# cmavro/GNN-RAG

Hardware: AMD Instinct MI355X
Metric: kg_edges_aggregated_per_sec (higher is better)
Workload: dtype f32

## Files before the change

### gnn-rag_amd/_lib.py

```python
from __future__ import annotations

import ctypes as C
import os

PKG = os.path.dirname(os.path.abspath(__file__))
LIB_PATH = os.path.join(PKG, "lib", "libgnnrag_hip.so")

c_i32p = C.POINTER(C.c_int32)
c_f32p = C.POINTER(C.c_float)


class CsrStruct(C.Structure):
    _fields_ = [
        ("B", C.c_int32), ("N", C.c_int32), ("R1", C.c_int32), ("heavy_deg", C.c_int32),
        ("F", C.c_int64),
        ("row_ptr", C.c_void_p * 2), ("edge", C.c_void_p * 2), ("perm", C.c_void_p * 2),
        ("w_gnn", C.c_void_p * 2), ("w_rel", C.c_void_p * 2),
        ("heavy", C.c_void_p * 2), ("chunk_off", C.c_void_p * 2),
        ("n_heavy", C.c_void_p), ("n_chunks", C.c_void_p),
        ("heavy_cap", C.c_int32), ("max_chunks", C.c_int32),
        ("big_cnt", C.c_void_p), ("big_nodes", C.c_void_p),
        ("big_deg", C.c_int32), ("hub_sorted", C.c_int32),
        ("edge_l", C.c_void_p * 2), ("rel_off", C.c_void_p), ("rel_rows", C.c_void_p),
        ("rel_total", C.c_int32), ("rel_max", C.c_int32),
        ("edge_m", C.c_void_p), ("m_from", C.c_void_p), ("m_dst", C.c_void_p),
        ("hub_q_off", C.c_void_p * 2), ("hub_wbase", C.c_void_p * 2),
    ]


class RelorderStruct(C.Structure):
    _fields_ = [("F", C.c_int64), ("rel_total", C.c_int32), ("n_chunks", C.c_int32),
                ("ht", C.c_void_p), ("perm", C.c_void_p), ("w", C.c_void_p), ("row_ptr", C.c_void_p),
                ("chunk_ptr", C.c_void_p)]


class UGraphStruct(C.Structure):
    _fields_ = [("B", C.c_int32), ("N", C.c_int32), ("F", C.c_int64), ("cap", C.c_int64),
                ("u_ptr", C.c_void_p), ("u_adj", C.c_void_p)]


class DenseFormStruct(C.Structure):
    _fields_ = [(n, C.c_int32) for n in ("family", "block_family", "launches", "epi", "nt", "mt", "v4", "math", "nw",
                                          "v4out", "n0", "nc", "has_add", "kguard")]


class LayerParams(C.Structure):
    _fields_ = [("W_rel", C.c_void_p), ("b_rel", C.c_void_p), ("pos_fwd", C.c_void_p), ("pos_inv", C.c_void_p),
                ("W_e2e", C.c_void_p), ("b_e2e", C.c_void_p)]


class BertLayer(C.Structure):
    _fields_ = [(n, C.c_void_p) for n in ("W_qkv", "b_qkv", "W_o", "b_o", "ln1_g", "ln1_b", "W_i", "b_i", "W_f", "b_f",
                                          "ln2_g", "ln2_b")]


_VP = C.c_void_p
SIGNATURES = {
    "gnnrag_csr_bytes": (C.c_size_t, [C.c_int64, C.c_int32, C.c_int32, C.c_int32, C.c_int, C.c_int]),
    "gnnrag_csr_scratch_bytes": (C.c_size_t, [C.c_int64, C.c_int32, C.c_int32, C.c_int32]),
    "gnnrag_csr_build": (C.c_int, [_VP, _VP, _VP, _VP, _VP, C.c_int64, C.c_int32, C.c_int32, C.c_int32,
                                   _VP, C.c_size_t, _VP, C.c_size_t, C.POINTER(CsrStruct), _VP]),
    "gnnrag_csr_build_counts": (C.c_int, [_VP, _VP, _VP, _VP, _VP, C.c_int64, C.c_int32, C.c_int32, C.c_int32, C.c_int32,
                                          C.c_int32, _VP, C.c_size_t, _VP, C.c_size_t, C.POINTER(CsrStruct), _VP]),
    "gnnrag_csr_status": (C.c_int, [C.POINTER(CsrStruct), _VP]),
    "gnnrag_csr_concat": (C.c_int, [C.POINTER(C.POINTER(CsrStruct)), C.c_int32, C.c_int32, C.c_int32, _VP, C.c_size_t,
                                    C.POINTER(CsrStruct), _VP]),
    "gnnrag_narrow_tuple": (C.c_int, [_VP, _VP, _VP, C.c_int64, _VP, C.c_int32]),
    "gnnrag_csr_permute_weight": (C.c_int, [C.POINTER(CsrStruct), _VP, C.c_int, _VP, _VP, _VP]),
    "gnnrag_linear": (C.c_int, [_VP, C.c_int64, C.c_int32, _VP, _VP, _VP, C.c_int64, C.c_int, _VP,
                                C.c_int32, C.c_int32, _VP]),
    "gnnrag_linear_pair": (C.c_int, [_VP, _VP, C.c_int64, C.c_int32, _VP, _VP, _VP, _VP, C.c_int64, _VP, _VP,
                                     C.c_int32, C.c_int32, _VP]),
    "gnnrag_aggregate_workspace_bytes": (C.c_size_t, [C.POINTER(CsrStruct), C.c_int32, C.c_int32]),
    "gnnrag_aggregate": (C.c_int, [C.POINTER(CsrStruct), _VP, _VP, _VP, _VP, _VP, C.c_int32, C.c_int32,
                                   _VP, C.c_size_t, _VP]),
    "gnnrag_aggregate_fused": (C.c_int, [C.POINTER(CsrStruct), _VP, _VP, _VP, C.c_int32, _VP, C.c_size_t, _VP]),
    "gnnrag_aggregate_fused_variant": (C.c_int, [C.POINTER(CsrStruct), C.c_int32]),
    "gnnrag_aggregate_fused_hub_form": (C.c_int, [C.POINTER(CsrStruct), C.c_int32, _VP, C.c_size_t, _VP, _VP]),
    "gnnrag_relorder_bytes": (C.c_size_t, [C.POINTER(CsrStruct), C.c_int]),
    "gnnrag_relorder_scratch_bytes": (C.c_size_t, [C.POINTER(CsrStruct)]),
    "gnnrag_relorder_build": (C.c_int, [C.POINTER(CsrStruct), _VP, _VP, _VP, _VP, _VP, C.c_size_t, _VP, C.c_size_t,
                                        C.POINTER(RelorderStruct), _VP]),
    "gnnrag_backward_workspace_bytes": (C.c_size_t, [C.POINTER(CsrStruct), C.POINTER(RelorderStruct), C.c_int32,
                                                     C.c_int32]),
    "gnnrag_aggregate_fused_backward": (C.c_int, [C.POINTER(CsrStruct), C.POINTER(RelorderStruct), _VP, _VP, _VP, _VP, _VP,
                                                 C.c_int32, _VP, C.c_size_t, _VP]),
    "gnnrag_aggregate_backward": (C.c_int, [C.POINTER(CsrStruct), C.POINTER(RelorderStruct), _VP, _VP, _VP, _VP, _VP,
                                            _VP, _VP, _VP, _VP, C.c_int32, C.c_int32, _VP, C.c_size_t, _VP]),
    "gnnrag_typelayer_backward": (C.c_int, [C.POINTER(CsrStruct), C.POINTER(RelorderStruct), _VP, _VP, C.c_int, _VP,
                                            C.c_int32, _VP, C.c_size_t, _VP]),
    "gnnrag_lstm_workspace_bytes": (C.c_size_t, [C.c_int32, C.c_int32]),
    "gnnrag_lstm_forward": (C.c_int, [_VP] * 10 + [C.c_int32] * 4 + [_VP, C.c_size_t, _VP]),
    "gnnrag_lstm_reserve_bytes": (C.c_size_t, [C.c_int32] * 3),
    "gnnrag_lstm_forward_train": (C.c_int, [_VP] * 10 + [C.c_int32] * 4 + [_VP, C.c_size_t, _VP, C.c_size_t, _VP]),
    "gnnrag_lstm_backward_workspace_bytes": (C.c_size_t, [C.c_int32] * 4),
    "gnnrag_lstm_backward": (C.c_int, [_VP] * 7 + [C.c_size_t] + [_VP] * 9 + [C.c_int32] * 4 + [_VP, C.c_size_t, _VP]),
    "gnnrag_seed_retrieve": (C.c_int, [_VP, _VP, _VP, C.c_int32, C.c_int32, C.c_int32, _VP]),
    "gnnrag_query_reform": (C.c_int, [_VP, _VP, _VP, C.c_int64, _VP, _VP, _VP, C.c_int32, C.c_int32, C.c_int32, _VP]),
    "gnnrag_topp_candidates": (C.c_int, [_VP, _VP, C.c_int32, C.c_int32, C.c_double, C.c_double, _VP, _VP, _VP]),
    "gnnrag_topp_workspace_bytes": (C.c_size_t, [C.c_int32, C.c_int32]),
    "gnnrag_topp_candidates_ws": (C.c_int, [_VP, _VP, C.c_int32, C.c_int32, C.c_double, C.c_double, _VP, _VP, _VP,
                                            C.c_size_t, _VP]),
    "gnnrag_relation_tables": (C.c_int, [C.POINTER(CsrStruct), _VP, _VP, _VP, _VP, _VP, C.c_int32, C.c_int32,
                                         C.c_int32, _VP]),
    "gnnrag_update_score_fused": (C.c_int, [_VP, _VP, _VP, _VP, _VP, _VP, _VP, _VP, _VP, C.c_int64, C.c_int32,
                                            C.c_int32, C.c_int32, _VP]),
    "gnnrag_update_score": (C.c_int, [_VP, _VP, _VP, _VP, _VP, _VP, _VP, _VP, _VP, C.c_int64, C.c_int32,
                                      C.c_int32, C.c_int32, _VP]),
    "gnnrag_dense_form": (C.c_int, [C.c_int32, C.c_int64, C.c_int32, C.c_int32, C.c_int32, C.c_int32, C.c_int64,
                                    C.c_int32, C.c_int32, C.POINTER(DenseFormStruct)]),
    "gnnrag_masked_softmax": (C.c_int, [_VP, _VP, C.c_int32, C.c_int32, _VP]),
    "gnnrag_typelayer": (C.c_int, [C.POINTER(CsrStruct), _VP, C.c_int, _VP, C.c_int32, _VP, C.c_size_t, _VP]),
    "gnnrag_layer_workspace_bytes": (C.c_size_t, [C.POINTER(CsrStruct), C.c_int32, C.c_int32]),
    "gnnrag_stack_workspace_bytes": (C.c_size_t, [C.POINTER(CsrStruct), C.c_int32, C.c_int32, C.c_int32]),
    "gnnrag_rel_transform": (C.c_int, [_VP, _VP, C.c_int64, C.c_int32, C.c_int32, C.POINTER(LayerParams), C.c_int32, _VP,
                                      _VP, _VP]),
    "gnnrag_gemm_tn_workspace_bytes": (C.c_size_t, [C.c_int64, C.c_int32, C.c_int32]),
    "gnnrag_gemm_tn": (C.c_int, [_VP, _VP, C.c_int64, C.c_int32, C.c_int32, _VP, _VP, C.c_size_t, _VP]),
    "gnnrag_rel_planes_bytes": (C.c_size_t, [C.c_int64, C.c_int32, C.c_int32]),
    "gnnrag_relation_tables_planes": (C.c_int, [C.POINTER(CsrStruct), _VP, _VP, _VP, _VP, C.c_int32, C.c_int32, _VP]),
    "gnnrag_rel_packed_bytes": (C.c_size_t, [C.c_int64, C.c_int32, C.c_int32]),
    "gnnrag_rel_transform_packed": (C.c_int, [_VP, _VP, C.c_int64, C.c_int32, C.c_int32, C.POINTER(LayerParams), C.c_int32,
                                             _VP, _VP, _VP]),
    "gnnrag_relation_tables_packed": (C.c_int, [C.POINTER(CsrStruct), _VP, _VP, _VP, _VP, C.c_int32, C.c_int32, C.c_int32,
                                               _VP]),
    "gnnrag_reason_layer": (C.c_int, [C.POINTER(CsrStruct)] + [_VP] * 9 + [C.c_int32] + [_VP] * 8 +
                            [_VP, C.c_size_t, C.c_int32, C.c_int32, C.c_int32, C.c_int32, _VP]),
    "gnnrag_reason_stack": (C.c_int, [C.POINTER(CsrStruct), C.c_int32, C.POINTER(LayerParams)] + [_VP] * 5 +
                            [C.c_int32] + [_VP] * 6 + [_VP, C.c_size_t, C.c_int32, C.c_int32, C.c_int32, C.c_int32, _VP]),
    "gnnrag_reason_stack_capture": (C.c_int, [C.POINTER(CsrStruct), C.c_int32, C.POINTER(LayerParams)] + [_VP] * 5 +
                                    [C.c_int32] + [_VP] * 6 + [_VP, C.c_size_t, C.c_int32, C.c_int32, C.c_int32,
                                                               C.c_int32, _VP, C.POINTER(C.c_void_p)]),
    "gnnrag_graph_launch": (C.c_int, [_VP, _VP]),
    "gnnrag_graph_destroy": (C.c_int, [_VP]),
    "gnnrag_frontier_workspace_bytes": (C.c_size_t, [C.POINTER(CsrStruct)]),
    "gnnrag_frontier_supported": (C.c_int, [C.POINTER(CsrStruct), C.c_int32]),
    "gnnrag_frontier_build": (C.c_int, [C.POINTER(CsrStruct), _VP, _VP, C.c_size_t, _VP]),
    "gnnrag_relation_tables_frontier": (C.c_int, [C.POINTER(CsrStruct), _VP, _VP, _VP, _VP, _VP, _VP, C.c_int32,
                                                  C.c_int32, _VP]),
    "gnnrag_aggregate_fused_frontier": (C.c_int, [C.POINTER(CsrStruct), _VP, _VP, _VP, _VP, C.c_int32, _VP]),
    "gnnrag_frontier_read": (C.c_int, [C.POINTER(CsrStruct), _VP, _VP, _VP, _VP]),
    "gnnrag_instructions": (C.c_int, [_VP] * 4 + [C.POINTER(C.c_void_p)] * 2 + [_VP] * 4 + [C.c_int32] * 4 + [_VP] * 3),
    "gnnrag_instructions_reserve_bytes": (C.c_size_t, [C.c_int32] * 4),
    "gnnrag_instructions_train": (C.c_int, [_VP] * 4 + [C.POINTER(C.c_void_p)] * 2 + [_VP] * 7 + [C.c_int32] * 4 +
                                  [_VP] * 3 + [C.c_size_t, _VP]),
    "gnnrag_instructions_backward_workspace_bytes": (C.c_size_t, [C.c_int32] * 4),
    "gnnrag_instructions_backward": (C.c_int, [_VP] * 3 + [C.POINTER(C.c_void_p)] + [_VP] * 8 + [C.c_size_t] + [_VP] * 5 +
                                     [C.POINTER(C.c_void_p)] * 2 + [_VP] * 4 + [C.c_int32] * 4 + [_VP, C.c_size_t, _VP]),
    "gnnrag_query_reform_reserve_bytes": (C.c_size_t, [C.c_int32] * 3),
    "gnnrag_query_reform_train": (C.c_int, [C.POINTER(C.c_void_p), _VP, _VP, C.c_int64] + [C.POINTER(C.c_void_p)] * 2 +
                                  [_VP, _VP, C.c_size_t] + [C.c_int32] * 4 + [_VP]),
    "gnnrag_query_reform_backward_workspace_bytes": (C.c_size_t, [C.c_int32] * 4),
    "gnnrag_query_reform_backward": (C.c_int, [C.POINTER(C.c_void_p), _VP] + [C.POINTER(C.c_void_p)] * 2 +
                                     [_VP, C.c_size_t] + [C.POINTER(C.c_void_p)] * 4 + [_VP] + [C.c_int32] * 4 +
                                     [_VP, C.c_size_t, _VP]),
    "gnnrag_layer_tail_train": (C.c_int, [_VP] * 3 + [C.c_float] + [_VP] * 3 + [C.c_int32] * 3 + [_VP] * 4),
    "gnnrag_layer_tail_backward_workspace_bytes": (C.c_size_t, [C.c_int32] * 3),
    "gnnrag_layer_tail_backward": (C.c_int, [_VP] * 3 + [C.c_float] + [_VP] * 3 + [C.c_int32] * 3 + [_VP] * 4 +
                                   [C.c_size_t, _VP]),
    "gnnrag_kl_loss_workspace_bytes": (C.c_size_t, [C.c_int32]),
    "gnnrag_kl_loss_train": (C.c_int, [_VP] * 3 + [C.c_int32] * 2 + [_VP] * 3 + [C.c_size_t, _VP]),
    "gnnrag_kl_loss_backward": (C.c_int, [_VP] * 5 + [C.c_int32] * 2 + [_VP] * 2),
    "gnnrag_train_metrics": (C.c_int, [_VP] * 4 + [C.c_int64, C.c_double] + [C.c_int32] * 2 + [_VP] * 5),
    "gnnrag_bert_workspace_bytes": (C.c_size_t, [C.c_int32] * 4),
    "gnnrag_bert_attention": (C.c_int, [_VP] + [C.c_int32] * 4 + [_VP, _VP]),
    "gnnrag_bert_encode": (C.c_int, [_VP, _VP, C.c_int32, _VP, C.c_int32, _VP, _VP, _VP, C.c_float, C.c_int32,
                                     C.POINTER(BertLayer)] + [C.c_int32] * 5 + [_VP, _VP, C.c_size_t, C.c_int32, _VP]),
    "gnnrag_bert_attention_bias": (C.c_int, [_VP] + [C.c_int32] * 4 + [_VP, _VP, _VP]),
    "gnnrag_bert_encode_ex": (C.c_int, [_VP, _VP, C.c_int32, _VP, C.c_int32, _VP, C.c_int32, _VP, _VP, _VP, C.c_float,
                                        C.c_int32, C.POINTER(BertLayer)] + [C.c_int32] * 5 +
                              [_VP, _VP, C.c_size_t, C.c_int32, _VP]),
    "gnnrag_bert_keep_hidden_bytes": (C.c_size_t, [C.c_int32] * 4),
    "gnnrag_bert_keep_att_bytes": (C.c_size_t, [C.c_int32] * 4),
    "gnnrag_bert_attention_drop": (C.c_int, [_VP] + [C.c_int32] * 4 + [_VP, _VP, C.c_float, _VP, _VP]),
    "gnnrag_bert_encode_train": (C.c_int, [_VP, _VP, C.c_int32, _VP, C.c_int32, _VP, C.c_int32, _VP, _VP, _VP, C.c_float,
                                           C.c_int32, C.POINTER(BertLayer)] + [C.c_int32] * 5 +
                                 [_VP, C.c_float, _VP, C.c_float, _VP, _VP, C.c_size_t, C.c_int32, _VP]),
    "gnnrag_rel_text_workspace_bytes": (C.c_size_t, [C.c_int64] + [C.c_int32] * 4),
    "gnnrag_rel_text_pool": (C.c_int, [_VP] * 6 + [C.c_int64] + [C.c_int32] * 3 + [_VP] * 5 + [C.c_size_t, _VP]),
    "gnnrag_rel_text_backward_workspace_bytes": (C.c_size_t, [C.c_int64] + [C.c_int32] * 4),
    "gnnrag_rel_text_pool_backward": (C.c_int, [_VP] * 8 + [C.c_int64] + [C.c_int32] * 3 + [_VP] * 4 + [C.c_size_t, _VP]),
    "gnnrag_ugraph_bytes": (C.c_size_t, [C.c_int64, C.c_int32, C.c_int32]),
    "gnnrag_ugraph_scratch_bytes": (C.c_size_t, [C.c_int64, C.c_int32, C.c_int32]),
    "gnnrag_ugraph_build": (C.c_int, [C.POINTER(CsrStruct), _VP, C.c_size_t, _VP, C.c_size_t, C.POINTER(UGraphStruct),
                                      _VP]),
    "gnnrag_paths_workspace_bytes": (C.c_size_t, [C.c_int32, C.c_int32, C.c_int32, C.c_int32]),
    "gnnrag_paths_out_bytes": (C.c_size_t, [C.c_int32] * 5),
    "gnnrag_shortest_paths": (C.c_int, [C.POINTER(UGraphStruct), _VP, _VP, _VP, C.c_int32, C.c_int32, C.c_int32, C.c_int32,
                                        _VP, _VP, _VP, _VP, _VP, _VP, C.c_size_t, _VP]),
    "gnnrag_rule_paths_workspace_bytes": (C.c_size_t, [C.c_int64] + [C.c_int32] * 4),
    "gnnrag_rule_paths_out_bytes": (C.c_size_t, [C.c_int32] * 5),
    "gnnrag_rule_paths": (C.c_int, [C.POINTER(UGraphStruct), _VP, _VP, _VP, _VP, C.c_int32, C.c_int32, C.c_int32, C.c_int32,
                                    _VP, _VP, _VP, _VP, _VP, _VP, C.c_size_t, _VP]),
    "gnnrag_stream_copy": (C.c_int, [_VP, _VP, C.c_int64, _VP]),
    "gnnrag_abi_version": (C.c_int, []),
    "gnnrag_error_string": (C.c_char_p, [C.c_int]),
}

ABI_VERSION = 16
PATH_AUTO, PATH_UNFUSED, PATH_FUSED = 0, 1, 2
PATH_ONLY_FWD, PATH_ONLY_INV = 0x10, 0x20
PATH_SEED_PRIOR = 0x40
PATH_REUSE_PROJ = 0x80
E_TUPLE = -4
_lib = None


class GnnragError(RuntimeError):
    pass


def load():
    global _lib
    if _lib is not None:
        return _lib
    path = os.environ.get("GNNRAG_LIB", LIB_PATH)
    if not os.path.exists(path):
        raise GnnragError(
            "HIP extension %s is not built. Run `python -c 'import __graft_entry__ as g; g.build()'` "
            "(hipcc --offload-arch=gfx950). There is no CPU fallback." % path)
    lib = C.CDLL(path)
    for name, (res, args) in SIGNATURES.items():
        fn = getattr(lib, name)
        fn.restype = res
        fn.argtypes = args
    if lib.gnnrag_abi_version() != ABI_VERSION:
        raise GnnragError("ABI mismatch: library %d, binding %d" % (lib.gnnrag_abi_version(), ABI_VERSION))
    _lib = lib
    return lib


def check(code: int, what: str = ""):
    if code != 0:
        msg = load().gnnrag_error_string(code)
        err = GnnragError("%s failed (%d): %s" % (what or "gnnrag call", code,
                                                  msg.decode() if msg else "?"))
        err.code = code
        raise err
```

### gnn-rag_amd/csrc/dense_internal.h

```cpp
#pragma once
#include "gnnrag_common.h"

namespace gnnrag {

int tables_vq_launch_z(const gnnrag_csr* csr, const void* planes, const float* ins, const float* W, float* P, int32_t D,
                       int32_t I, int32_t only_dir, float* zero, int64_t zero_n, hipStream_t stream, bool packed);
size_t tables_vq_packed_bytes(int64_t R1);

int update_score_fused_rows(const float* h, const float* nbr, const uint8_t* add_flag, const float* W, const float* b,
                            const float* w_s, const float* b_s, const float* mask, float* h_out, float* score,
                            int64_t BN, int32_t D, int32_t I, int32_t math, hipStream_t stream, bool score_zeroed);
int update_b3_launch_f(const float* h, const float* nbr, const uint8_t* add_flag, const float* W, const float* b,
                       const float* w_s, const float* b_s, const float* mask, float* h_out, float* score, int64_t BN,
                       int32_t D, int32_t ldw, hipStream_t stream, bool score_zeroed);

bool update_rows_supported(const float* h, const float* nbr, const float* W, const float* h_out, int64_t BN, int32_t D,
                           int32_t I, int32_t math);
bool update_b3_shape_ok(int64_t BN, int32_t D, int32_t ldw);
int tables_small_launch(const gnnrag_csr* csr, const float* T_fwd, const float* T_inv, const float* ins, const float* W,
                        float* P, int32_t D, int32_t I, hipStream_t stream);

int frontier_build_z(const gnnrag_csr* csr, const float* dist, void* fws, size_t fws_bytes, float* zero_a,
                     int64_t zero_na, float* zero_b, int64_t zero_nb, hipStream_t stream);
const uint8_t* frontier_row_flags(const gnnrag_csr* csr, const void* fws);

int update_score_fused_z(const float* h, const float* nbr, const float* W, const float* b, const float* w_s,
                         const float* b_s, const float* mask, float* h_out, float* score, int64_t BN, int32_t D,
                         int32_t I, int32_t math, hipStream_t stream, bool score_zeroed);

bool rel_transform_accepts(const float* relfeat_fwd, const float* relfeat_inv, int64_t R1, int32_t D, int32_t L,
                           const gnnrag_layer_params* layers, int32_t pos_rows, const float* T_out, const void* planes_out);
int rel_transform_launch(const float* relfeat_fwd, const float* relfeat_inv, int64_t R1, int32_t D, int32_t L,
                         const gnnrag_layer_params* layers, int32_t pos_rows, float* T_out, void* planes_out,
                         void* packed_out, gnnrag_stream_t stream);

}
```

### gnn-rag_amd/csrc/frontier.hip

```cpp
#include "dense_internal.h"

namespace gnnrag {

constexpr int kFrThreads = 1024;
constexpr int kFrSeedCap = 2048;
constexpr int kFrAltSeeds = 32;

struct FrontierWs {
  size_t counts, row_flag, rows, tflag, trows, seeds, seedinfo, total;
};

static FrontierWs frontier_ws(const gnnrag_csr* csr) {
  FrontierWs w;
  Carve cv;
  const size_t BN = (size_t)csr->B * csr->N;
  const size_t RT = (size_t)(csr->rel_total > 0 ? csr->rel_total : 1);
  w.counts = cv.take((size_t)2 * csr->B * sizeof(int32_t));
  w.row_flag = cv.take(BN + 64);
  w.rows = cv.take(BN * sizeof(int32_t));
  w.tflag = cv.take(RT + 64);
  w.trows = cv.take(RT * sizeof(int32_t));
  w.seeds = cv.take((size_t)csr->B * kFrAltSeeds * sizeof(int32_t));
  w.seedinfo = cv.take((size_t)2 * csr->B * sizeof(int32_t));
  w.total = cv.off;
  return w;
}

__global__ __launch_bounds__(kFrThreads) void k_frontier_build(
    const float* __restrict__ dist, const int32_t* __restrict__ rp0, const int32_t* __restrict__ rp1,
    const int2* __restrict__ el0, const int2* __restrict__ el1, const int32_t* __restrict__ rel_off, int N,
    uint8_t* __restrict__ row_flag, int32_t* __restrict__ rows, uint8_t* __restrict__ tflag,
    int32_t* __restrict__ trows, int32_t* __restrict__ counts, int32_t* __restrict__ seeds,
    int32_t* __restrict__ seedinfo, float* __restrict__ zero_a, long long zero_na, float* __restrict__ zero_b,
    long long zero_nb) {
  __shared__ int s_seed[kFrSeedCap];
  __shared__ int s_ns, s_wsum[kFrThreads / 64];
  const int g = blockIdx.x, tid = threadIdx.x, lane = tid & 63, wave = tid >> 6;
  const int roff = rel_off[g], Rg = rel_off[g + 1] - roff;
  const size_t n0 = (size_t)g * N;
  for (long long i = (long long)blockIdx.x * kFrThreads + tid; i < zero_na; i += (long long)gridDim.x * kFrThreads) zero_a[i] = 0.f;
  for (long long i = (long long)blockIdx.x * kFrThreads + tid; i < zero_nb; i += (long long)gridDim.x * kFrThreads) zero_b[i] = 0.f;
  if (tid == 0) s_ns = 0;
  if (g == (int)gridDim.x - 1 && tid < 64) row_flag[(size_t)gridDim.x * N + tid] = 0;
  for (int i = tid; i < N; i += kFrThreads) row_flag[n0 + i] = 0;
  for (int i = tid; i < Rg; i += kFrThreads) tflag[roff + i] = 0;
  __syncthreads();
  for (int i = tid; i < N; i += kFrThreads) {
    if (dist[n0 + i] != 0.f) {
      const int k = atomicAdd(&s_ns, 1);
      if (k < kFrSeedCap) s_seed[k] = (int)n0 + i;
    }
  }
  __syncthreads();
  const int ns = s_ns;
  if (tid == 0) {
    int cnt = -1, facts = 0;
    if (ns <= kFrAltSeeds) {
      cnt = ns;
      for (int i = 1; i < ns; ++i) {
        const int v = s_seed[i];
        int j = i - 1;
        for (; j >= 0 && s_seed[j] > v; --j) s_seed[j + 1] = s_seed[j];
        s_seed[j + 1] = v;
      }
      for (int i = 0; i < ns; ++i) {
        const int sn = s_seed[i];
        seeds[g * kFrAltSeeds + i] = sn;
        facts += (rp0[sn + 1] - rp0[sn]) + (rp1[sn + 1] - rp1[sn]);
      }
    }
    seedinfo[2 * g] = cnt;
    seedinfo[2 * g + 1] = facts;
  }
  __syncthreads();
  if (ns > kFrSeedCap) {
    for (int i = tid; i < N; i += kFrThreads) row_flag[n0 + i] = 1;
    for (int i = tid; i < Rg; i += kFrThreads) tflag[roff + i] = 1;
  } else {
    for (int k = 0; k < ns; ++k) {
      const int s = s_seed[k];
#pragma unroll
      for (int dd = 0; dd < 2; ++dd) {
        const int32_t* rp = dd ? rp1 : rp0;
        const int2* el = dd ? el1 : el0;
        const int beg = rp[s], end = rp[s + 1];
        for (int j = beg + tid; j < end; j += kFrThreads) {
          const int2 e = el[j];
          row_flag[e.x] = 1;
          tflag[roff + e.y] = 1;
        }
      }
    }
  }
  __syncthreads();
  auto compact = [&](const uint8_t* flag, int n, int first, int32_t* list, int32_t* count_out) {
    int base = 0;
    for (int c0 = 0; c0 < n; c0 += kFrThreads) {
      const int i = c0 + tid;
      const bool on = i < n && flag[i] != 0;
      const unsigned long long m = __ballot(on);
      if (lane == 0) s_wsum[wave] = __popcll(m);
      __syncthreads();
      int off = base, tot = 0;
      for (int w = 0; w < kFrThreads / 64; ++w) {
        const int c = s_wsum[w];
        if (w < wave) off += c;
        tot += c;
      }
      if (on) list[off + __popcll(m & ((1ull << lane) - 1))] = first + i;
      base += tot;
      __syncthreads();
    }
    if (tid == 0) *count_out = base;
  };
  compact(row_flag + n0, N, (int)n0, rows + n0, counts + 2 * g);
  compact(tflag + roff, Rg, roff, trows + roff, counts + 2 * g + 1);
}

struct TabFrArgs {
  const float* T[2];
  const float* ins;
  const float* W;
  const int2* rel_rows;
  const int32_t* rel_off;
  const int32_t* list;
  const int32_t* counts;
  float* P;
  int32_t D, I, rel_total, B;
  int32_t dense;
};

__global__ __launch_bounds__(256) void k_tables_frontier(TabFrArgs a, int tiles_per_q) {
  __shared__ __attribute__((aligned(16))) float s_part[3][4][64][4];
  const int lane = threadIdx.x & 63, wave = threadIdx.x >> 6;
  const int fr = lane & 15, fg = lane >> 4;
  const int D = a.D, K = a.I * D, ldw = (2 * a.I + 1) * D;
  const int ncg = (D + 63) >> 6;
  const f32x4 zero4 = {0.f, 0.f, 0.f, 0.f};
  const int nitem = a.dense ? ((a.rel_total + 15) >> 4) * 2 * ncg : a.B * 2 * ncg;
  for (int item = blockIdx.x; item < nitem; item += gridDim.x)
  for (int tile = a.dense ? item / (2 * ncg) : 0; tile < (a.dense ? item / (2 * ncg) + 1 : tiles_per_q); ++tile) {
    int r = a.dense ? item % (2 * ncg) : item;
    const int cg = r % ncg; r /= ncg;
    const int d = r & 1; r >>= 1;
    const int g = a.dense ? 0 : r;
    const int cnt = a.dense ? a.rel_total : a.counts[2 * g + 1];
    if (tile * 16 >= cnt) break;
    const int32_t* list = a.dense ? nullptr : a.list + a.rel_off[g];
    const int c0 = cg * 64;
    const int m = tile * 16 + fr;
    const int prow = a.dense ? (m < cnt ? m : cnt - 1) : list[m < cnt ? m : cnt - 1];
    const int2 br = a.rel_rows[prow];
    const float* trow = a.T[d] + (size_t)br.y * D;
    const float* qrow = a.ins + (size_t)br.x * a.I * D;
    const float* wrow[4];
#pragma unroll
    for (int nt = 0; nt < 4; ++nt) wrow[nt] = a.W + (size_t)min(c0 + nt * 16 + fr, D - 1) * ldw + (size_t)(1 + d) * D;
    f32x4 acc[4] = {zero4, zero4, zero4, zero4};
    const int nkg = (K + 15) >> 4;
    for (int kg0 = wave; kg0 < nkg; kg0 += 16) {
      f32x4 av[4], bv[4][4];
#pragma unroll
      for (int u = 0; u < 4; ++u) {
        const int k = (kg0 + 4 * u) * 16 + fg * 4;
        av[u] = zero4;
#pragma unroll
        for (int nt = 0; nt < 4; ++nt) bv[u][nt] = zero4;
        if (k < K) {
          const int i = k / D, kk = k - i * D;
          const f32x4 t = *reinterpret_cast<const f32x4*>(trow + kk);
          const f32x4 q = *reinterpret_cast<const f32x4*>(qrow + (size_t)i * D + kk);
          av[u] = __builtin_elementwise_max(t * q, zero4);
#pragma unroll
          for (int nt = 0; nt < 4; ++nt) bv[u][nt] = *reinterpret_cast<const f32x4*>(wrow[nt] + (size_t)2 * i * D + kk);
        }
      }
#pragma unroll
      for (int u = 0; u < 4; ++u)
#pragma unroll
        for (int nt = 0; nt < 4; ++nt)
#pragma unroll
          for (int e = 0; e < 4; ++e) acc[nt] = __builtin_amdgcn_mfma_f32_16x16x4f32(av[u][e], bv[u][nt][e], acc[nt], 0, 0, 0);
    }
    if (wave > 0) {
#pragma unroll
      for (int nt = 0; nt < 4; ++nt) *reinterpret_cast<f32x4*>(&s_part[wave - 1][nt][lane][0]) = acc[nt];
    }
    __syncthreads();
    if (wave == 0) {
#pragma unroll
      for (int nt = 0; nt < 4; ++nt) {
        const f32x4 v = ((acc[nt] + *reinterpret_cast<const f32x4*>(&s_part[0][nt][lane][0])) +
                         *reinterpret_cast<const f32x4*>(&s_part[1][nt][lane][0])) +
                        *reinterpret_cast<const f32x4*>(&s_part[2][nt][lane][0]);
        const int col = c0 + nt * 16 + fr;
#pragma unroll
        for (int rr = 0; rr < 4; ++rr) {
          const int mm = tile * 16 + fg * 4 + rr;
          if (mm < cnt && col < D) a.P[((size_t)d * a.rel_total + (a.dense ? mm : list[mm])) * D + col] = v[rr];
        }
      }
    }
    __syncthreads();
  }
}

struct WalkFrArgs {
  const int32_t* rp0;
  const int32_t* rp1;
  const int2* edge_m;
  const int32_t* m_from;
  const float* w0;
  const float* w1;
  const float* dist;
  const float* P;
  const int32_t* rel_off;
  const int32_t* rows;
  const int32_t* counts;
  float* out;
  const int32_t* seeds;
  const int32_t* seedinfo;
  int64_t F;
  int32_t N, D, rel_total, B;
};

constexpr int kWfThreads = 256;
constexpr int kWfPer = 8;
constexpr int kWfCap = kWfThreads * kWfPer;
constexpr int kWfAltMin = 4096;

__global__ __launch_bounds__(kWfThreads) void k_walk_frontier(WalkFrArgs a, int per_q) {
  __shared__ int2 s_live[kWfCap];
  __shared__ int s_wsum[kWfPer * 4];
  __shared__ __attribute__((aligned(16))) float s_red[3][256];
  const int tid = threadIdx.x, lane = tid & 63, wave = tid >> 6;
  const int D = a.D;
  const int g = blockIdx.x / per_q;
  const int cnt = a.counts[2 * g];
  const int roff = a.rel_off[g], Rg = a.rel_off[g + 1] - roff;
  const int col = 4 * lane;
  const bool cok = col < D;
  const f32x4 zero4 = {0.f, 0.f, 0.f, 0.f};
  for (int it = blockIdx.x % per_q; it < cnt; it += per_q) {
    const int n = a.rows[(size_t)g * a.N + it];
    const int beg = a.rp0[n] + a.rp1[n], end = a.rp0[n + 1] + a.rp1[n + 1];
    f32x4 acc = zero4;
    bool split = false;
    const int nseed = a.seedinfo[2 * g];
    const bool alt = nseed > 0 && end - beg > kWfAltMin && a.seedinfo[2 * g + 1] <= ((end - beg) >> 2);
    if (alt && wave == 0) {
      for (int si = 0; si < nseed; ++si) {
        const int sn = a.seeds[g * kFrAltSeeds + si];
        const float ps = a.dist[sn];
        const int sb = a.rp0[sn] + a.rp1[sn], se = a.rp0[sn + 1] + a.rp1[sn + 1];
        for (int c0 = sb; c0 < se; c0 += 64) {
          const int j = c0 + lane;
          const int2 e = j < se ? a.edge_m[j] : make_int2(-1, 0);
          float p = 0.f;
          if (e.x == n) {
            p = ps;
            if (a.w0) {
              const int f = a.m_from[j];
              p *= f < a.F ? a.w0[f] : a.w1[f - a.F];
            }
          }
          unsigned long long m = __ballot(p != 0.f);
          while (m) {
            const int l = __builtin_ctzll(m);
            m &= m - 1;
            const float pl = __int_as_float(__builtin_amdgcn_readlane(__float_as_int(p), l));
            const int rm = __builtin_amdgcn_readlane(e.y, l);
            const int dq = rm > Rg ? 1 : 0;
            const int rl = dq ? rm - (Rg + 1) : rm;
            if (cok) acc += pl * *reinterpret_cast<const f32x4*>(a.P + ((size_t)(1 - dq) * a.rel_total + roff + rl) * D + col);
          }
        }
      }
    }
    for (int c0 = beg; c0 < (alt ? beg : end); c0 += kWfCap) {
      int2 e[kWfPer];
      float p[kWfPer];
#pragma unroll
      for (int u = 0; u < kWfPer; ++u) {
        const int j = c0 + u * kWfThreads + tid;
        e[u] = j < end ? a.edge_m[j] : make_int2(0, 0);
      }
#pragma unroll
      for (int u = 0; u < kWfPer; ++u) {
        const int j = c0 + u * kWfThreads + tid;
        p[u] = 0.f;
        if (j < end) {
          p[u] = a.dist[e[u].x];
          if (a.w0) {
            const int f = a.m_from[j];
            p[u] *= f < a.F ? a.w0[f] : a.w1[f - a.F];
          }
        }
      }
      unsigned long long mk[kWfPer];
#pragma unroll
      for (int u = 0; u < kWfPer; ++u) {
        mk[u] = __ballot(p[u] != 0.f);
        if (lane == 0) s_wsum[u * 4 + wave] = __popcll(mk[u]);
      }
      __syncthreads();
      int nl = 0;
#pragma unroll
      for (int u = 0; u < kWfPer; ++u) {
        int off = nl;
#pragma unroll
        for (int w = 0; w < 4; ++w) {
          const int t = s_wsum[u * 4 + w];
          if (w < wave) off += t;
          nl += t;
        }
        if (p[u] != 0.f) {
          const int rm = e[u].y;
          const int d = rm > Rg ? 1 : 0;
          const int rl = d ? rm - (Rg + 1) : rm;
          s_live[off + __popcll(mk[u] & ((1ull << lane) - 1))] = make_int2(__float_as_int(p[u]), d * a.rel_total + roff + rl);
        }
      }
      __syncthreads();
      if (nl <= 32 && !split) {
        if (wave == 0 && cok) {
          for (int k = 0; k < nl; ++k) {
            const int2 lv = s_live[k];
            const f32x4 t = *reinterpret_cast<const f32x4*>(a.P + (size_t)lv.y * D + col);
            acc += __int_as_float(lv.x) * t;
          }
        }
      } else {
        split = true;
        if (cok) {
          for (int k = wave; k < nl; k += 4) {
            const int2 lv = s_live[k];
            const f32x4 t = *reinterpret_cast<const f32x4*>(a.P + (size_t)lv.y * D + col);
            acc += __int_as_float(lv.x) * t;
          }
        }
      }
      __syncthreads();
    }
    if (split) {
      if (wave > 0) *reinterpret_cast<f32x4*>(&s_red[wave - 1][col]) = acc;
      __syncthreads();
      if (wave == 0)
        acc = ((acc + *reinterpret_cast<const f32x4*>(&s_red[0][col])) + *reinterpret_cast<const f32x4*>(&s_red[1][col])) +
              *reinterpret_cast<const f32x4*>(&s_red[2][col]);
      __syncthreads();
    }
    if (wave == 0 && cok) *reinterpret_cast<f32x4*>(a.out + (size_t)n * D + col) = acc;
  }
}

}

using namespace gnnrag;

extern "C" size_t gnnrag_frontier_workspace_bytes(const gnnrag_csr* csr) {
  if (!csr) return 0;
  return frontier_ws(csr).total;
}

extern "C" int gnnrag_frontier_supported(const gnnrag_csr* csr, int32_t D) {
  return csr && csr->edge_m && csr->m_from && D > 0 && D % 4 == 0 && D <= 256 ? 1 : 0;
}

int gnnrag::frontier_build_z(const gnnrag_csr* csr, const float* dist, void* fws, size_t fws_bytes, float* zero_a,
                             int64_t zero_na, float* zero_b, int64_t zero_nb, hipStream_t stream) {
  if (!csr || !dist || !fws) return GNNRAG_E_BADARG;
  const FrontierWs w = frontier_ws(csr);
  if (fws_bytes < w.total) return GNNRAG_E_WORKSPACE;
  char* base = (char*)fws;
  hipLaunchKernelGGL(k_frontier_build, dim3(csr->B), dim3(kFrThreads), 0, stream, dist, csr->row_ptr[0], csr->row_ptr[1],
                     (const int2*)csr->edge_l[0], (const int2*)csr->edge_l[1], csr->rel_off, csr->N,
                     (uint8_t*)(base + w.row_flag), (int32_t*)(base + w.rows), (uint8_t*)(base + w.tflag),
                     (int32_t*)(base + w.trows), (int32_t*)(base + w.counts), (int32_t*)(base + w.seeds),
                     (int32_t*)(base + w.seedinfo), zero_a, (long long)zero_na, zero_b,
                     (long long)zero_nb);
  GNNRAG_LAUNCH_CHECK();
  return 0;
}

extern "C" int gnnrag_frontier_build(const gnnrag_csr* csr, const float* dist, void* fws, size_t fws_bytes,
                                     gnnrag_stream_t stream) {
  return frontier_build_z(csr, dist, fws, fws_bytes, nullptr, 0, nullptr, 0, (hipStream_t)stream);
}

const uint8_t* gnnrag::frontier_row_flags(const gnnrag_csr* csr, const void* fws) {
  return (const uint8_t*)fws + frontier_ws(csr).row_flag;
}

extern "C" int gnnrag_relation_tables_frontier(const gnnrag_csr* csr, const void* fws, const float* T_fwd,
                                               const float* T_inv, const float* ins, const float* W, float* P,
                                               int32_t D, int32_t I, gnnrag_stream_t stream) {
  if (!csr || !fws || !T_fwd || !T_inv || !ins || !W || !P || I <= 0) return GNNRAG_E_BADARG;
  if (!gnnrag_frontier_supported(csr, D) || !aligned16(T_fwd, T_inv, ins, W, P)) return GNNRAG_E_UNSUPPORTED;
  if (csr->rel_total == 0) return 0;
  const FrontierWs w = frontier_ws(csr);
  const char* base = (const char*)fws;
  TabFrArgs a;
  a.T[0] = T_fwd; a.T[1] = T_inv; a.ins = ins; a.W = W;
  a.rel_rows = (const int2*)csr->rel_rows;
  a.rel_off = csr->rel_off;
  a.list = (const int32_t*)(base + w.trows);
  a.counts = (const int32_t*)(base + w.counts);
  a.P = P; a.D = D; a.I = I; a.rel_total = csr->rel_total; a.B = csr->B; a.dense = 0;
  const int tiles_per_q = (csr->rel_max + 15) / 16;
  const int64_t nitem = (int64_t)csr->B * 2 * ((D + 63) / 64);
  hipLaunchKernelGGL(k_tables_frontier, dim3((unsigned)(nitem < 4096 ? nitem : 4096)), dim3(256), 0, (hipStream_t)stream, a,
                     tiles_per_q);
  GNNRAG_LAUNCH_CHECK();
  return 0;
}

extern "C" int gnnrag_aggregate_fused_frontier(const gnnrag_csr* csr, const void* fws, const float* dist,
                                               const float* P, float* out, int32_t D, gnnrag_stream_t stream) {
  if (!csr || !fws || !dist || !P || !out) return GNNRAG_E_BADARG;
  if (!gnnrag_frontier_supported(csr, D) || !aligned16(P, out) || csr->N <= 0) return GNNRAG_E_UNSUPPORTED;
  const FrontierWs w = frontier_ws(csr);
  const char* base = (const char*)fws;
  WalkFrArgs a;
  a.rp0 = csr->row_ptr[0]; a.rp1 = csr->row_ptr[1];
  a.edge_m = (const int2*)csr->edge_m; a.m_from = csr->m_from;
  a.w0 = csr->w_gnn[0]; a.w1 = csr->w_gnn[1];
  a.dist = dist; a.P = P; a.rel_off = csr->rel_off;
  a.rows = (const int32_t*)(base + w.rows);
  a.counts = (const int32_t*)(base + w.counts);
  a.seeds = (const int32_t*)(base + w.seeds);
  a.seedinfo = (const int32_t*)(base + w.seedinfo);
  a.out = out; a.F = csr->F; a.N = csr->N; a.D = D; a.rel_total = csr->rel_total; a.B = csr->B;
  int per_q = 1024 / csr->B;
  if (per_q < 4) per_q = 4;
  if (per_q > 256) per_q = 256;
  if (per_q > csr->N) per_q = csr->N;
  hipLaunchKernelGGL(k_walk_frontier, dim3((unsigned)(csr->B * per_q)), dim3(kWfThreads), 0, (hipStream_t)stream, a, per_q);
  GNNRAG_LAUNCH_CHECK();
  return 0;
}

extern "C" int gnnrag_frontier_read(const gnnrag_csr* csr, const void* fws, int32_t* counts2, uint8_t* row_flag_host,
                                    gnnrag_stream_t stream) {
  if (!csr || !fws || !counts2) return GNNRAG_E_BADARG;
  const FrontierWs w = frontier_ws(csr);
  const char* base = (const char*)fws;
  int32_t* per_q = new int32_t[(size_t)2 * csr->B];
  hipError_t e = hipMemcpyAsync(per_q, base + w.counts, (size_t)2 * csr->B * sizeof(int32_t), hipMemcpyDeviceToHost,
                                (hipStream_t)stream);
  if (e == hipSuccess && row_flag_host)
    e = hipMemcpyAsync(row_flag_host, base + w.row_flag, (size_t)csr->B * csr->N, hipMemcpyDeviceToHost, (hipStream_t)stream);
  if (e == hipSuccess) e = hipStreamSynchronize((hipStream_t)stream);
  counts2[0] = counts2[1] = 0;
  for (int g = 0; g < csr->B; ++g) {
    counts2[0] += per_q[2 * g];
    counts2[1] += per_q[2 * g + 1];
  }
  delete[] per_q;
  return e == hipSuccess ? 0 : (int)e;
}

int gnnrag::tables_small_launch(const gnnrag_csr* csr, const float* T_fwd, const float* T_inv, const float* ins,
                                const float* W, float* P, int32_t D, int32_t I, hipStream_t stream) {
  if (D % 4 || D > 256 || csr->rel_total <= 0) return GNNRAG_E_UNSUPPORTED;
  if (2.0 * 2 * csr->rel_total * (double)I * D * D > 1.5e8) return GNNRAG_E_UNSUPPORTED;
  if (!aligned16(T_fwd, T_inv, ins, W)) return GNNRAG_E_UNSUPPORTED;
  TabFrArgs a;
  a.T[0] = T_fwd; a.T[1] = T_inv; a.ins = ins; a.W = W;
  a.rel_rows = (const int2*)csr->rel_rows;
  a.rel_off = csr->rel_off;
  a.list = nullptr; a.counts = nullptr;
  a.P = P; a.D = D; a.I = I; a.rel_total = csr->rel_total; a.B = csr->B; a.dense = 1;
  const int nitem = ((csr->rel_total + 15) / 16) * 2 * ((D + 63) / 64);
  hipLaunchKernelGGL(k_tables_frontier, dim3(nitem), dim3(256), 0, stream, a, 0);
  GNNRAG_LAUNCH_CHECK();
  return 0;
}
```

### gnn-rag_amd/csrc/rel_transform.hip

```cpp
#include "gnnrag_common.h"
#include "dense_internal.h"

namespace gnnrag {

constexpr int kRtMaxL = 8;
constexpr int kRtUnroll = 7;

struct RelTArgs {
  const float* A[2];
  const float* W[kRtMaxL];
  const float* b[kRtMaxL];
  const float* add[kRtMaxL][2];
  float* C;
  unsigned short* planes;
  unsigned char* packed;
  int M, K, N, add_rows;
};

constexpr int kPlaneHalf = 224;
constexpr int kPlaneRow = 2 * kPlaneHalf;
constexpr int kPackPlaneB = kPlaneHalf * 2;
constexpr int kPackIdxB = 3 * kPackPlaneB;
constexpr int kPackRowB = kPackIdxB + 64;

template <int TPW>
__global__ __launch_bounds__(256) void k_rel_transform(RelTArgs g) {
  extern __shared__ __attribute__((aligned(16))) float Wf[];
  const int tid = threadIdx.x, lane = tid & 63, wave = tid >> 6;
  const int fr = lane & 15, fg = lane >> 4;
  const int j = blockIdx.z >> 1, d = blockIdx.z & 1;
  const int colg = blockIdx.y * 64;
  const int K = g.K;
  const int nch = (K + 15) >> 4;
  const f32x4 zero4 = {0.f, 0.f, 0.f, 0.f};
  const bool compute = colg < g.N;
  if (compute) {
    const int total = 64 * nch * 4;
    for (int x = tid; x < total; x += 256) {
      const int col = x / (nch * 4), kq = x - col * (nch * 4);
      f32x4 v = zero4;
      if (colg + col < g.N && 4 * kq < K) v = *reinterpret_cast<const f32x4*>(g.W[j] + (size_t)(colg + col) * K + 4 * kq);
      const int c = kq >> 2, fgq = kq & 3, a = col & 3, frq = col >> 2;
      *reinterpret_cast<f32x4*>(Wf + ((size_t)((c * 4 + a) * 64 + fgq * 16 + frq)) * 4) = v;
    }
  }
  __syncthreads();
  const int c4 = colg + 4 * fr;
  const bool in_T = c4 < g.N;
  const bool in_pad = !in_T && c4 < kPlaneHalf;
  f32x4 bias = zero4;
  if (in_T && g.b[j]) bias = *reinterpret_cast<const f32x4*>(g.b[j] + c4);
  const float* __restrict__ addp = g.add[j][d];
  float* __restrict__ cp = g.C + ((size_t)(2 * j + d) * g.M) * g.N;
  unsigned short* pp = g.planes ? g.planes + ((size_t)(2 * j + d) * 3 * g.M) * kPlaneRow : nullptr;
  unsigned char* pk = g.packed ? g.packed + ((size_t)(2 * j + d) * g.M) * kPackRowB : nullptr;

#pragma unroll 1
  for (int t = 0; t < TPW; ++t) {
    const int row0 = (blockIdx.x * TPW + t) * 64 + wave * 16;
    if (row0 >= g.M) break;
    f32x4 acc[4][2];
#pragma unroll
    for (int a = 0; a < 4; ++a) acc[a][0] = acc[a][1] = zero4;
    if (compute) {
      const float* __restrict__ ap = g.A[d] + (size_t)min(row0 + fr, g.M - 1) * K;
      for (int c0 = 0; c0 < nch; c0 += kRtUnroll) {
        f32x4 av[kRtUnroll];
#pragma unroll
        for (int u = 0; u < kRtUnroll; ++u)
          av[u] = *reinterpret_cast<const f32x4*>(ap + min(16 * (c0 + u) + 4 * fg, K - 4));
#pragma unroll
        for (int u = 0; u < kRtUnroll; ++u) {
          const int c = min(c0 + u, nch - 1);
          const bool live = 16 * (c0 + u) + 4 * fg < K;
          const f32x4 x = live ? av[u] : zero4;
          f32x4 wv[4];
#pragma unroll
          for (int a = 0; a < 4; ++a) wv[a] = *reinterpret_cast<const f32x4*>(Wf + ((size_t)((c * 4 + a) * 64 + lane)) * 4);
#pragma unroll
          for (int e = 0; e < 4; ++e)
#pragma unroll
            for (int a = 0; a < 4; ++a)
              acc[a][e & 1] = __builtin_amdgcn_mfma_f32_16x16x4f32(x[e], wv[a][e], acc[a][e & 1], 0, 0, 0);
        }
      }
    }
    if (!in_T && !(pp && in_pad) && !pk) continue;
#pragma unroll
    for (int r = 0; r < 4; ++r) {
      const int row = row0 + 4 * fg + r;
      if (row >= g.M) continue;
      f32x4 v = zero4;
      if (in_T) {
#pragma unroll
        for (int a = 0; a < 4; ++a) v[a] = acc[a][0][r] + acc[a][1][r];
        v += bias;
        if (addp && row < g.add_rows) v += *reinterpret_cast<const f32x4*>(addp + (size_t)row * g.N + c4);
        *reinterpret_cast<f32x4*>(cp + (size_t)row * g.N + c4) = v;
      }
      if (pp) {
#pragma unroll
        for (int half = 0; half < 2; ++half) {
          const Split3 sp = split3(__builtin_elementwise_max(half ? -v : v, zero4));
          const size_t e = (size_t)row * kPlaneRow + half * kPlaneHalf + c4;
          *reinterpret_cast<uint2*>(pp + e) = sp.hi;
          *reinterpret_cast<uint2*>(pp + (size_t)g.M * kPlaneRow + e) = sp.mid;
          *reinterpret_cast<uint2*>(pp + (size_t)2 * g.M * kPlaneRow + e) = sp.lo;
        }
      }
      if (pk) {
        unsigned char* rowp = pk + (size_t)row * kPackRowB;
        if (c4 < kPlaneHalf) {
          const Split3 sp = split3(__builtin_elementwise_abs(v));
          *reinterpret_cast<uint2*>(rowp + 2 * c4) = sp.hi;
          *reinterpret_cast<uint2*>(rowp + kPackPlaneB + 2 * c4) = sp.mid;
          *reinterpret_cast<uint2*>(rowp + 2 * kPackPlaneB + 2 * c4) = sp.lo;
        }
        const int q = c4 >> 2;
        const unsigned ix = 0x88u | (unsigned)(v[0] < 0.f) | (unsigned)(v[1] < 0.f) << 2 | (unsigned)(v[2] < 0.f) << 4 |
                            (unsigned)(v[3] < 0.f) << 6;
        rowp[kPackIdxB + ((q & 7) >> 1) * 16 + (q >> 3) * 2 + (q & 1)] = (unsigned char)(c4 < kPlaneHalf ? ix : 0u);
      }
    }
  }
}

}

using namespace gnnrag;

extern "C" size_t gnnrag_rel_planes_bytes(int64_t R1, int32_t D, int32_t L) {
  if (R1 <= 0 || D <= 0 || D > kPlaneHalf || L <= 0) return 0;
  return (size_t)L * 2 * 3 * R1 * kPlaneRow * sizeof(unsigned short);
}

bool gnnrag::rel_transform_accepts(const float* relfeat_fwd, const float* relfeat_inv, int64_t R1, int32_t D, int32_t L,
                                   const gnnrag_layer_params* layers, int32_t pos_rows, const float* T_out,
                                   const void* planes_out) {
  if (D <= 0 || (D & 3)) return false;
  if (planes_out && D > kPlaneHalf) return false;
  if (R1 >= ((int64_t)1 << 31) / D) return false;
  uintptr_t align = (uintptr_t)relfeat_fwd | (uintptr_t)relfeat_inv | (uintptr_t)T_out | (uintptr_t)planes_out;
  for (int j = 0; j < L; ++j) {
    align |= (uintptr_t)layers[j].W_rel | (uintptr_t)layers[j].b_rel;
    if (pos_rows > 0) align |= (uintptr_t)layers[j].pos_fwd | (uintptr_t)layers[j].pos_inv;
  }
  if (align & 15) return false;
  return (size_t)64 * ((D + 15) / 16) * 16 * sizeof(float) <= 160 * 1024;
}

extern "C" size_t gnnrag_rel_packed_bytes(int64_t R1, int32_t D, int32_t L) {
  if (R1 <= 0 || D <= 0 || D > kPlaneHalf || L <= 0) return 0;
  return (size_t)L * 2 * R1 * kPackRowB;
}

int gnnrag::rel_transform_launch(const float* relfeat_fwd, const float* relfeat_inv, int64_t R1, int32_t D, int32_t L,
                                 const gnnrag_layer_params* layers, int32_t pos_rows, float* T_out, void* planes_out,
                                 void* packed_out, gnnrag_stream_t stream) {
  if (planes_out && packed_out) return GNNRAG_E_BADARG;
  void* const side_out = planes_out ? planes_out : packed_out;
  if (!relfeat_fwd || !relfeat_inv || !layers || !T_out || R1 < 0 || D <= 0 || L <= 0 || pos_rows < 0)
    return GNNRAG_E_BADARG;
  for (int j = 0; j < L; ++j) {
    if (!layers[j].W_rel) return GNNRAG_E_BADARG;
    if ((layers[j].pos_fwd == nullptr) != (layers[j].pos_inv == nullptr)) return GNNRAG_E_BADARG;
  }
  if (!gnnrag::rel_transform_accepts(relfeat_fwd, relfeat_inv, R1, D, L, layers, pos_rows, T_out, side_out))
    return GNNRAG_E_UNSUPPORTED;
  if (R1 == 0) return 0;
  for (int j0 = 0; j0 < L; j0 += kRtMaxL) {
    const int n = L - j0 < kRtMaxL ? L - j0 : kRtMaxL;
    RelTArgs g;
    memset(&g, 0, sizeof(g));
    g.A[0] = relfeat_fwd;
    g.A[1] = relfeat_inv;
    for (int j = 0; j < n; ++j) {
      const gnnrag_layer_params& p = layers[j0 + j];
      g.W[j] = p.W_rel;
      g.b[j] = p.b_rel;
      g.add[j][0] = pos_rows > 0 ? p.pos_fwd : nullptr;
      g.add[j][1] = pos_rows > 0 ? p.pos_inv : nullptr;
    }
    g.C = T_out + (size_t)j0 * 2 * R1 * D;
    g.planes = planes_out ? (unsigned short*)planes_out + (size_t)j0 * 2 * 3 * R1 * kPlaneRow : nullptr;
    g.packed = packed_out ? (unsigned char*)packed_out + (size_t)j0 * 2 * R1 * kPackRowB : nullptr;
    g.M = (int)R1; g.K = D; g.N = D;
    g.add_rows = (int)(pos_rows < R1 ? pos_rows : R1);
    const unsigned gy = (unsigned)(((side_out ? kPlaneHalf : D) + 63) / 64), gz = (unsigned)(2 * n);
    const size_t lds = (size_t)64 * ((D + 15) / 16) * 16 * sizeof(float);
    static DeviceMask cap1, cap4;
    if (R1 > 2048) {
      if (lds > 64 * 1024) { const int rc = raise_lds_cap(k_rel_transform<4>, cap4); if (rc) return rc; }
      hipLaunchKernelGGL(k_rel_transform<4>, dim3((unsigned)((R1 + 255) / 256), gy, gz), dim3(256), lds,
                         (hipStream_t)stream, g);
    } else {
      if (lds > 64 * 1024) { const int rc = raise_lds_cap(k_rel_transform<1>, cap1); if (rc) return rc; }
      hipLaunchKernelGGL(k_rel_transform<1>, dim3((unsigned)((R1 + 63) / 64), gy, gz), dim3(256), lds,
                         (hipStream_t)stream, g);
    }
    GNNRAG_LAUNCH_CHECK();
  }
  return 0;
}

extern "C" int gnnrag_rel_transform(const float* relfeat_fwd, const float* relfeat_inv, int64_t R1, int32_t D,
                                    int32_t L, const gnnrag_layer_params* layers, int32_t pos_rows, float* T_out,
                                    void* planes_out, gnnrag_stream_t stream) {
  return gnnrag::rel_transform_launch(relfeat_fwd, relfeat_inv, R1, D, L, layers, pos_rows, T_out, planes_out, nullptr, stream);
}

extern "C" int gnnrag_rel_transform_packed(const float* relfeat_fwd, const float* relfeat_inv, int64_t R1, int32_t D,
                                           int32_t L, const gnnrag_layer_params* layers, int32_t pos_rows, float* T_out,
                                           void* packed_out, gnnrag_stream_t stream) {
  if (!packed_out) return GNNRAG_E_BADARG;
  return gnnrag::rel_transform_launch(relfeat_fwd, relfeat_inv, R1, D, L, layers, pos_rows, T_out, nullptr, packed_out, stream);
}
```

### gnn-rag_amd/csrc/softmax_layer.hip

```cpp
#include "gnnrag_common.h"
#include "dense_internal.h"

namespace gnnrag {

template <int ITEMS>
__global__ __launch_bounds__(1024) void k_masked_softmax(const float* __restrict__ score,
                                                         float* __restrict__ dist, int N) {
  __shared__ float red[16];
  __shared__ float bcast;
  const float* s = score + (size_t)blockIdx.x * N;
  float* o = dist + (size_t)blockIdx.x * N;
  const int lane = threadIdx.x & 63, wave = threadIdx.x >> 6;
  float v[ITEMS > 0 ? ITEMS : 1];

  float m = -INFINITY;
  if constexpr (ITEMS > 0) {
#pragma unroll
    for (int k = 0; k < ITEMS; ++k) {
      const int i = threadIdx.x + k * 1024;
      v[k] = i < N ? s[i] : -INFINITY;
      m = fmaxf(m, v[k]);
    }
  } else {
    for (int i = threadIdx.x; i < N; i += 1024) m = fmaxf(m, s[i]);
  }
#pragma unroll
  for (int off = 32; off > 0; off >>= 1) m = fmaxf(m, __shfl_xor(m, off, 64));
  if (lane == 0) red[wave] = m;
  __syncthreads();
  if (threadIdx.x == 0) {
    float mm = red[0];
    for (int w = 1; w < 16; ++w) mm = fmaxf(mm, red[w]);
    bcast = mm;
  }
  __syncthreads();
  m = bcast;
  __syncthreads();

  float sum = 0.f;
  if constexpr (ITEMS > 0) {
#pragma unroll
    for (int k = 0; k < ITEMS; ++k) {
      v[k] = expf(v[k] - m);
      sum += v[k];
    }
  } else {
    for (int i = threadIdx.x; i < N; i += 1024) sum += expf(s[i] - m);
  }
  sum = wave_sum(sum);
  if (lane == 0) red[wave] = sum;
  __syncthreads();
  if (threadIdx.x == 0) {
    float t = 0.f;
    for (int w = 0; w < 16; ++w) t += red[w];
    bcast = t;
  }
  __syncthreads();
  const float total = bcast;
  if constexpr (ITEMS > 0) {
#pragma unroll
    for (int k = 0; k < ITEMS; ++k) {
      const int i = threadIdx.x + k * 1024;
      if (i < N) o[i] = v[k] / total;
    }
  } else {
    for (int i = threadIdx.x; i < N; i += 1024) o[i] = expf(s[i] - m) / total;
  }
}

template <int ITEMS>
__global__ __launch_bounds__(1024) void k_softmax_pairs(const float* __restrict__ score, float* __restrict__ dist, int N,
                                                        const int32_t* __restrict__ rp0, const int32_t* __restrict__ rp1,
                                                        const int2* __restrict__ em, const int32_t* __restrict__ from,
                                                        const float* __restrict__ w0, const float* __restrict__ w1,
                                                        int64_t F, int2* __restrict__ pr) {
  extern __shared__ float s_dist[];
  __shared__ float red[16];
  __shared__ float bcast;
  const int g = blockIdx.x, part = blockIdx.y, nparts = gridDim.y;
  const float* s = score + (size_t)g * N;
  float* o = dist + (size_t)g * N;
  const int lane = threadIdx.x & 63, wave = threadIdx.x >> 6;
  float v[ITEMS];
  float m = -INFINITY;
#pragma unroll
  for (int k = 0; k < ITEMS; ++k) {
    const int i = threadIdx.x + k * 1024;
    v[k] = i < N ? s[i] : -INFINITY;
    m = fmaxf(m, v[k]);
  }
  m = wave_max(m);
  if (lane == 0) red[wave] = m;
  __syncthreads();
  if (threadIdx.x == 0) {
    float mm = red[0];
    for (int w = 1; w < 16; ++w) mm = fmaxf(mm, red[w]);
    bcast = mm;
  }
  __syncthreads();
  m = bcast;
  __syncthreads();
  float sum = 0.f;
#pragma unroll
  for (int k = 0; k < ITEMS; ++k) {
    v[k] = expf(v[k] - m);
    sum += v[k];
  }
  sum = wave_sum(sum);
  if (lane == 0) red[wave] = sum;
  __syncthreads();
  if (threadIdx.x == 0) {
    float t = 0.f;
    for (int w = 0; w < 16; ++w) t += red[w];
    bcast = t;
  }
  __syncthreads();
  const float total = bcast;
#pragma unroll
  for (int k = 0; k < ITEMS; ++k) {
    const int i = threadIdx.x + k * 1024;
    if (i < N) {
      const float d = v[k] / total;
      s_dist[i] = d;
      if (part == 0) o[i] = d;
    }
  }
  __syncthreads();
  const int64_t n0 = (int64_t)g * N;
  const int64_t beg = (int64_t)rp0[n0] + rp1[n0], end = (int64_t)rp0[n0 + N] + rp1[n0 + N];
  const int64_t lo = beg + (end - beg) * part / nparts, hi = beg + (end - beg) * (part + 1) / nparts;
  typedef int i32x2 __attribute__((ext_vector_type(2)));
  for (int64_t j = lo + threadIdx.x; j < hi; j += 1024) {
    const i32x2 e = __builtin_nontemporal_load(reinterpret_cast<const i32x2*>(em) + j);
    const unsigned s = (unsigned)(e.x - (int)n0);
    float p = s < (unsigned)N ? s_dist[s] : 0.f;
    if (w0) {
      const int f = from[j];
      p *= f < F ? w0[f] : w1[f - F];
    }
    pr[j] = make_int2(__float_as_int(p), e.y);
  }
}

__global__ __launch_bounds__(256) void k_stream_copy(const f32x4* __restrict__ src, f32x4* __restrict__ dst,
                                                     int64_t n4) {
  const int64_t stride = (int64_t)gridDim.x * 1024;
  for (int64_t base = (int64_t)blockIdx.x * 1024; base < n4; base += stride) {
    f32x4 v[4];
#pragma unroll
    for (int u = 0; u < 4; ++u) {
      const int64_t i = base + u * 256 + threadIdx.x;
      if (i < n4) v[u] = __builtin_nontemporal_load(src + i);
    }
#pragma unroll
    for (int u = 0; u < 4; ++u) {
      const int64_t i = base + u * 256 + threadIdx.x;
      if (i < n4) __builtin_nontemporal_store(v[u], dst + i);
    }
  }
}

struct LayerWs { size_t T_fwd, T_inv, planes, agg, P, nbr, partial, partial_bytes, fws, fws_bytes, total; };

static bool fused_is_cheaper(int64_t B, int64_t N, int64_t rel_total, int64_t D, int64_t I) {
  const double unfused = (double)B * N * (2 * I + 1) * D * D;
  const double fused = 2.0 * rel_total * I * D * D + (double)B * N * D * D;
  return fused < 0.8 * unfused;
}

static bool path_ok(int32_t path) {
  const int base = path & 0xf, flags = path & ~0xf & ~GNNRAG_PATH_SEED_PRIOR & ~GNNRAG_PATH_REUSE_PROJ;
  if (base < GNNRAG_PATH_AUTO || base > GNNRAG_PATH_FUSED) return false;
  return flags == 0 || flags == GNNRAG_PATH_ONLY_FWD || flags == GNNRAG_PATH_ONLY_INV;
}

static LayerWs layer_ws(const gnnrag_csr* csr, int32_t D, int32_t I) {
  LayerWs w;
  Carve cv;
  const size_t BN = (size_t)csr->B * csr->N;
  w.T_fwd = cv.take((size_t)2 * csr->R1 * D * sizeof(float));
  w.T_inv = w.T_fwd + (size_t)csr->R1 * D * sizeof(float);
  w.planes = cv.take(tables_vq_shape_ok(D, I) ? tables_vq_planes_bytes(csr->R1) : 0);
  const size_t a_bytes = BN * 2 * I * D * sizeof(float);
  const size_t p_bytes = align_up((size_t)2 * (csr->rel_total > 0 ? csr->rel_total : 1) * D * sizeof(float), 256);
  const size_t n_bytes = (BN + 1) * D * sizeof(float);
  const size_t big = cv.take(a_bytes > p_bytes + n_bytes ? a_bytes : p_bytes + n_bytes);
  w.agg = big;
  w.P = big;
  w.nbr = big + p_bytes;
  w.partial_bytes = gnnrag_aggregate_workspace_bytes(csr, D, I);
  w.partial = cv.take(w.partial_bytes);
  w.fws_bytes = gnnrag_frontier_workspace_bytes(csr);
  w.fws = cv.take(w.fws_bytes);
  w.total = cv.off;
  return w;
}

static bool planes_wanted(const gnnrag_csr* csr, int32_t D, int32_t I, int32_t path, int32_t math) {
  const bool fused = (path & 0xf) == GNNRAG_PATH_FUSED ||
                     ((path & 0xf) == GNNRAG_PATH_AUTO && fused_is_cheaper(csr->B, csr->N, csr->rel_total, D, I));
  return fused && math != GNNRAG_MATH_FP32 && tables_vq_shape_ok(D, I) && csr->rel_total >= 1024;
}

}

using namespace gnnrag;

extern "C" int gnnrag_masked_softmax(const float* score, float* dist, int32_t B, int32_t N,
                                     gnnrag_stream_t stream) {
  if (!score || !dist || B <= 0 || N <= 0) return GNNRAG_E_BADARG;
  if (N <= 2048) hipLaunchKernelGGL(k_masked_softmax<2>, dim3(B), dim3(1024), 0, (hipStream_t)stream, score, dist, N);
  else if (N <= 8192) hipLaunchKernelGGL(k_masked_softmax<8>, dim3(B), dim3(1024), 0, (hipStream_t)stream, score, dist, N);
  else hipLaunchKernelGGL(k_masked_softmax<0>, dim3(B), dim3(1024), 0, (hipStream_t)stream, score, dist, N);
  GNNRAG_LAUNCH_CHECK();
  return 0;
}

extern "C" int gnnrag_stream_copy(const float* src, float* dst, int64_t n, gnnrag_stream_t stream) {
  if (!src || !dst || n < 0 || (n & 3)) return GNNRAG_E_BADARG;
  if (n == 0) return 0;
  hipLaunchKernelGGL(k_stream_copy, dim3(256 * 16), dim3(256), 0, (hipStream_t)stream, (const f32x4*)src,
                     (f32x4*)dst, n / 4);
  GNNRAG_LAUNCH_CHECK();
  return 0;
}

extern "C" size_t gnnrag_layer_workspace_bytes(const gnnrag_csr* csr, int32_t D, int32_t I) {
  if (!csr || D <= 0 || I <= 0) return 0;
  return layer_ws(csr, D, I).total;
}

static int finish_softmax(const gnnrag_csr* csr, const LayerWs& w, char* base, const float* score, float* dist_out, int32_t D,
                          bool want_pairs, bool* pairs_done, gnnrag_stream_t stream) {
  if (pairs_done) *pairs_done = false;
  const char* env = getenv("GNNRAG_SOFTMAX_PAIRS");
  const bool enabled = !(env && env[0] == '0');
  if (want_pairs && pairs_done && enabled && csr->N <= 8192 && csr->edge_m) {
    PriorPairsTarget t;
    const int rc = prior_pairs_target(csr, D, base + w.partial, w.partial_bytes, &t);
    if (rc) return rc;
    if (t.ok) {
      int parts = (512 + csr->B - 1) / csr->B;
      parts = parts < 1 ? 1 : parts > 8 ? 8 : parts;
      const size_t lds = (size_t)csr->N * sizeof(float);
      if (csr->N <= 2048)
        hipLaunchKernelGGL(k_softmax_pairs<2>, dim3(csr->B, parts), dim3(1024), lds, (hipStream_t)stream, score, dist_out,
                           csr->N, csr->row_ptr[0], csr->row_ptr[1], t.edge_m, t.m_from, t.w0, t.w1, t.F, t.pairs);
      else
        hipLaunchKernelGGL(k_softmax_pairs<8>, dim3(csr->B, parts), dim3(1024), lds, (hipStream_t)stream, score, dist_out,
                           csr->N, csr->row_ptr[0], csr->row_ptr[1], t.edge_m, t.m_from, t.w0, t.w1, t.F, t.pairs);
      GNNRAG_LAUNCH_CHECK();
      *pairs_done = true;
      return 0;
    }
  }
  return gnnrag_masked_softmax(score, dist_out, csr->B, csr->N, stream);
}

static int layer_body(const gnnrag_csr* csr, const LayerWs& w, char* base, const float* h, const float* dist,
                      const float* ins, const float* T_fwd, const float* T_inv, const void* planes, const float* W_e2e,
                      const float* b_e2e, const float* w_score, const float* b_score, const float* mask,
                      float* h_out, float* score_out, float* dist_out, int32_t D, int32_t I, int32_t path,
                      int32_t math, gnnrag_stream_t stream, bool pairs_ready = false, bool* pairs_for_next = nullptr) {
  if (pairs_for_next) *pairs_for_next = false;
  const int64_t BN = (int64_t)csr->B * csr->N;
  int rc;
  const int only = (path & GNNRAG_PATH_ONLY_FWD) ? 0 : (path & GNNRAG_PATH_ONLY_INV) ? 1 : -1;
  const bool seed_prior = (path & GNNRAG_PATH_SEED_PRIOR) != 0;
  path &= 0xf;
  if (path == GNNRAG_PATH_AUTO)
    path = fused_is_cheaper(csr->B, csr->N, csr->rel_total, D, I) ? GNNRAG_PATH_FUSED : GNNRAG_PATH_UNFUSED;
  if (path == GNNRAG_PATH_FUSED) {
    float* P = (float*)(base + w.P);
    float* nbr = (float*)(base + w.nbr);
    const bool one_dir = only >= 0 && gnnrag_aggregate_fused_variant(csr, D) != GNNRAG_WALK_L2_GATHER;
    const bool fr_aligned = aligned16(ins, W_e2e, T_fwd, T_inv, P, nbr, dist) && csr->N > 0;
    const bool frontier_form = seed_prior && only < 0 && fr_aligned && gnnrag_frontier_supported(csr, D) && csr->rel_total > 0;
    if (frontier_form) {
      void* fws = base + w.fws;
      const bool gated = update_rows_supported(h, nbr, W_e2e, h_out, BN, D, I, math);
      if (!gated) GNNRAG_HIP(hipMemsetAsync(nbr, 0, (size_t)BN * D * sizeof(float), (hipStream_t)stream));
      rc = frontier_build_z(csr, dist, fws, w.fws_bytes, score_out, BN, nbr + (size_t)BN * D, D, (hipStream_t)stream);
      if (rc) return rc;
      rc = gnnrag_relation_tables_frontier(csr, fws, T_fwd, T_inv, ins, W_e2e, P, D, I, stream);
      if (rc) return rc;
      rc = gnnrag_aggregate_fused_frontier(csr, fws, dist, P, nbr, D, stream);
      if (rc) return rc;
      rc = update_score_fused_rows(h, nbr, gated ? frontier_row_flags(csr, fws) : nullptr, W_e2e, b_e2e, w_score, b_score,
                                   mask, h_out, score_out, BN, D, I, math, (hipStream_t)stream, true);
      if (rc) return rc;
      return finish_softmax(csr, w, base, score_out, dist_out, D, only < 0, pairs_for_next, stream);
    }
    rc = GNNRAG_E_UNSUPPORTED;
    bool score_zeroed = false;
    if (planes && math != GNNRAG_MATH_FP32 && csr->rel_total > 0) {
      rc = tables_vq_launch_z(csr, planes, ins, W_e2e, P, D, I, one_dir ? only : -1, score_out, BN, (hipStream_t)stream, true);
      score_zeroed = rc == 0;
    }
    if (rc == GNNRAG_E_UNSUPPORTED) rc = gnnrag_relation_tables(csr, T_fwd, T_inv, ins, W_e2e, P, D, I, math, stream);
    if (rc) return rc;
    rc = aggregate_fused_dirs(csr, dist, P, nbr, D, one_dir ? 2 - only : 0, base + w.partial, w.partial_bytes,
                              (hipStream_t)stream, pairs_ready && !one_dir);
    if (rc) return rc;
    rc = update_score_fused_z(h, nbr, W_e2e, b_e2e, w_score, b_score, mask, h_out, score_out, BN, D, I, math,
                              (hipStream_t)stream, score_zeroed);
    if (rc) return rc;
    return finish_softmax(csr, w, base, score_out, dist_out, D, only < 0, pairs_for_next, stream);
  } else {
    float* agg = (float*)(base + w.agg);
    rc = gnnrag_aggregate(csr, dist, ins, T_fwd, T_inv, agg, D, I, base + w.partial, w.partial_bytes, stream);
    if (rc) return rc;
    rc = gnnrag_update_score(h, agg, W_e2e, b_e2e, w_score, b_score, mask, h_out, score_out, BN, D, I, math,
                             stream);
    if (rc) return rc;
  }
  return gnnrag_masked_softmax(score_out, dist_out, csr->B, csr->N, stream);
}

static int rel_projections(const gnnrag_csr* csr, int32_t n, const gnnrag_layer_params* layers,
                           const float* relfeat_fwd, const float* relfeat_inv, int32_t pos_rows, float* T,
                           void* planes, bool* planes_written, int32_t D, int32_t math, gnnrag_stream_t stream) {
  *planes_written = false;
  if ((D & 3) == 0) {
    const int rc = rel_transform_launch(relfeat_fwd, relfeat_inv, csr->R1, D, n, layers, pos_rows, T, nullptr, planes, stream);
    if (rc == 0) *planes_written = planes != nullptr;
    if (rc != GNNRAG_E_UNSUPPORTED) return rc;
  }
  const size_t RD = (size_t)csr->R1 * D;
  for (int j = 0; j < n; ++j) {
    const gnnrag_layer_params& p = layers[j];
    const int rc = gnnrag_linear_pair(relfeat_fwd, relfeat_inv, csr->R1, D, p.W_rel, p.b_rel, p.pos_fwd, p.pos_inv,
                                      p.pos_fwd ? pos_rows : 0, T + 2 * j * RD, T + (2 * j + 1) * RD, D, math, stream);
    if (rc) return rc;
  }
  return 0;
}

extern "C" size_t gnnrag_stack_workspace_bytes(const gnnrag_csr* csr, int32_t L, int32_t D, int32_t I) {
  if (!csr || L <= 0 || D <= 0 || I <= 0) return 0;
  return layer_ws(csr, D, I).total + align_up((size_t)L * 2 * csr->R1 * D * sizeof(float), 256) +
         align_up(tables_vq_shape_ok(D, I) ? (size_t)L * tables_vq_planes_bytes(csr->R1) : 0, 256);
}

extern "C" int gnnrag_reason_layer(const gnnrag_csr* csr, const float* h, const float* dist, const float* ins,
                                   const float* relfeat_fwd, const float* relfeat_inv, const float* W_rel,
                                   const float* b_rel, const float* pos_fwd, const float* pos_inv,
                                   int32_t pos_rows, const float* W_e2e, const float* b_e2e,
                                   const float* w_score, const float* b_score, const float* mask,
                                   float* h_out, float* score_out, float* dist_out, void* workspace,
                                   size_t workspace_bytes, int32_t D, int32_t I, int32_t path, int32_t math,
                                   gnnrag_stream_t stream) {
  if (!csr || !h || !dist || !ins || !relfeat_fwd || !relfeat_inv || !W_rel || !b_rel || !W_e2e || !b_e2e ||
      !w_score || !b_score || !mask || !h_out || !score_out || !dist_out || !workspace || D <= 0 || I <= 0)
    return GNNRAG_E_BADARG;
  if (!path_ok(path)) return GNNRAG_E_BADARG;
  const LayerWs w = layer_ws(csr, D, I);
  if (workspace_bytes < w.total) return GNNRAG_E_WORKSPACE;
  char* base = (char*)workspace;
  float* T_fwd = (float*)(base + w.T_fwd);
  float* T_inv = (float*)(base + w.T_inv);
  const gnnrag_layer_params p = {W_rel, b_rel, pos_fwd, pos_inv, W_e2e, b_e2e};
  void* planes = planes_wanted(csr, D, I, path, math) ? (void*)(base + w.planes) : nullptr;
  bool planes_written = false;
  const int rc = rel_projections(csr, 1, &p, relfeat_fwd, relfeat_inv, pos_rows, T_fwd, planes, &planes_written, D, math,
                                 stream);
  if (rc) return rc;
  if (!planes_written) planes = nullptr;
  return layer_body(csr, w, base, h, dist, ins, T_fwd, T_inv, planes, W_e2e, b_e2e, w_score, b_score, mask, h_out, score_out,
                    dist_out, D, I, path, math, stream);
}

extern "C" int gnnrag_reason_stack(const gnnrag_csr* csr, int32_t L, const gnnrag_layer_params* layers,
                                   const float* h0, const float* dist0, const float* ins,
                                   const float* relfeat_fwd, const float* relfeat_inv, int32_t pos_rows,
                                   const float* w_score, const float* b_score, const float* mask, float* h_out,
                                   float* score_out, float* dist_out, void* workspace, size_t workspace_bytes,
                                   int32_t D, int32_t I, int32_t path, int32_t math, gnnrag_stream_t stream) {
  if (!csr || L <= 0 || !layers || !h0 || !dist0 || !ins || !relfeat_fwd || !relfeat_inv || !w_score || !b_score ||
      !mask || !h_out || !score_out || !dist_out || !workspace || D <= 0 || I <= 0)
    return GNNRAG_E_BADARG;
  if (!path_ok(path)) return GNNRAG_E_BADARG;
  for (int j = 0; j < L; ++j)
    if (!layers[j].W_rel || !layers[j].b_rel || !layers[j].W_e2e || !layers[j].b_e2e) return GNNRAG_E_BADARG;
  const LayerWs w = layer_ws(csr, D, I);
  if (workspace_bytes < w.total) return GNNRAG_E_WORKSPACE;
  char* base = (char*)workspace;
  const size_t BN = (size_t)csr->B * csr->N;
  const size_t RD = (size_t)csr->R1 * D;
  const bool upfront = L > 1 && workspace_bytes >= gnnrag_stack_workspace_bytes(csr, L, D, I);
  float* T0 = (float*)(base + w.T_fwd);
  float* Tall = (float*)(base + w.total);
  const bool want_planes = planes_wanted(csr, D, I, path, math);
  const size_t plane_bytes = tables_vq_packed_bytes(csr->R1);
  char* planes_all = base + w.total + align_up((size_t)L * 2 * RD * sizeof(float), 256);
  bool planes_written = false;
  const bool reuse = upfront && (path & GNNRAG_PATH_REUSE_PROJ) != 0;
  path &= ~GNNRAG_PATH_REUSE_PROJ;
  if (reuse) {
    planes_written = want_planes && rel_transform_accepts(relfeat_fwd, relfeat_inv, csr->R1, D, L, layers, pos_rows, Tall,
                                                          planes_all);
  } else if (upfront) {
    const int rc = rel_projections(csr, L, layers, relfeat_fwd, relfeat_inv, pos_rows, Tall,
                                   want_planes ? planes_all : nullptr, &planes_written, D, math, stream);
    if (rc) return rc;
  }
  const float* h = h0;
  const float* dist = dist0;
  bool pairs_ready = false;
  for (int j = 0; j < L; ++j) {
    const gnnrag_layer_params& p = layers[j];
    float* hj = h_out + (size_t)j * BN * D;
    float* sj = score_out + (size_t)j * BN;
    float* dj = dist_out + (size_t)j * BN;
    float* T = upfront ? Tall + (size_t)j * 2 * RD : T0;
    void* planes = !want_planes ? nullptr : upfront ? (void*)(planes_all + (size_t)j * plane_bytes) : (void*)(base + w.planes);
    if (!upfront) {
      const int rc = rel_projections(csr, 1, &p, relfeat_fwd, relfeat_inv, pos_rows, T, planes, &planes_written, D, math,
                                     stream);
      if (rc) return rc;
    }
    if (!planes_written) planes = nullptr;
    bool pairs_next = false;
    const int rc = layer_body(csr, w, base, h, dist, ins, T, T + RD, planes, p.W_e2e, p.b_e2e, w_score, b_score, mask, hj, sj,
                              dj, D, I, j == 0 ? path : (path & ~GNNRAG_PATH_SEED_PRIOR), math, stream, pairs_ready,
                              j + 1 < L ? &pairs_next : nullptr);
    if (rc) return rc;
    pairs_ready = pairs_next;
    h = hj;
    dist = dj;
  }
  return 0;
}

struct gnnrag_graph {
  hipGraph_t graph;
  hipGraphExec_t exec;
};

extern "C" int gnnrag_reason_stack_capture(const gnnrag_csr* csr, int32_t L, const gnnrag_layer_params* layers,
                                           const float* h0, const float* dist0, const float* ins,
                                           const float* relfeat_fwd, const float* relfeat_inv, int32_t pos_rows,
                                           const float* w_score, const float* b_score, const float* mask,
                                           float* h_out, float* score_out, float* dist_out, void* workspace,
                                           size_t workspace_bytes, int32_t D, int32_t I, int32_t path, int32_t math,
                                           gnnrag_stream_t stream_, gnnrag_graph** out) {
  if (!out) return GNNRAG_E_BADARG;
  *out = nullptr;
  hipStream_t stream = (hipStream_t)stream_;
  GNNRAG_HIP(hipStreamBeginCapture(stream, hipStreamCaptureModeThreadLocal));
  const int rc = gnnrag_reason_stack(csr, L, layers, h0, dist0, ins, relfeat_fwd, relfeat_inv, pos_rows, w_score,
                                     b_score, mask, h_out, score_out, dist_out, workspace, workspace_bytes, D, I, path,
                                     math, stream);
  hipGraph_t graph = nullptr;
  const hipError_t e = hipStreamEndCapture(stream, &graph);
  if (rc) {
    if (graph) (void)hipGraphDestroy(graph);
    return rc;
  }
  if (e != hipSuccess) return (int)e;
  hipGraphExec_t exec = nullptr;
  const hipError_t e2 = hipGraphInstantiate(&exec, graph, nullptr, nullptr, 0);
  if (e2 != hipSuccess) {
    (void)hipGraphDestroy(graph);
    return (int)e2;
  }
  gnnrag_graph* g = new gnnrag_graph{graph, exec};
  *out = g;
  return 0;
}

extern "C" int gnnrag_graph_launch(gnnrag_graph* graph, gnnrag_stream_t stream) {
  if (!graph) return GNNRAG_E_BADARG;
  GNNRAG_HIP(hipGraphLaunch(graph->exec, (hipStream_t)stream));
  return 0;
}

extern "C" int gnnrag_graph_destroy(gnnrag_graph* graph) {
  if (!graph) return 0;
  (void)hipGraphExecDestroy(graph->exec);
  (void)hipGraphDestroy(graph->graph);
  delete graph;
  return 0;
}

extern "C" int gnnrag_abi_version(void) { return GNNRAG_ABI_VERSION; }

extern "C" const char* gnnrag_error_string(int code) {
  switch (code) {
    case 0: return "success";
    case GNNRAG_E_BADARG: return "gnnrag: bad argument (null pointer, negative or inconsistent size)";
    case GNNRAG_E_UNSUPPORTED: return "gnnrag: shape outside the compiled kernel set";
    case GNNRAG_E_WORKSPACE: return "gnnrag: caller-provided buffer too small";
    case GNNRAG_E_TUPLE:
      return "gnnrag: edge tuple out of range: node ids must lie in [0, B*N), relation ids in [0, R1), and a fact "
             "may not connect two questions";
  }
  if (code > 0) return hipGetErrorString((hipError_t)code);
  return "gnnrag: unknown error";
}
```

### gnn-rag_amd/ops.py

```python
from __future__ import annotations

import collections
import ctypes as C
import os
from typing import Optional

import numpy as np
import torch

from . import _lib


MATH_FP32, MATH_BF16X3, MATH_MIXED = 0, 1, 2
MATH_NAMES = {MATH_FP32: "fp32 (v_mfma_f32_16x16x4_f32, bit-exact fmaf chains)",
              MATH_BF16X3: "bf16x3 (exact 3-way bf16 split, 6 plane products on v_mfma_f32_16x16x32_bf16, fp32 accumulate)",
              MATH_MIXED: "mixed (per kernel the faster fp32-class form: bf16x3 - exact 3-way bf16 split, 6 plane products, "
                          "fp32 accumulate - for the relation tables and the self-block update, exact fp32 MFMA for the "
                          "small products)"}
_default_math = {"fp32": MATH_FP32, "bf16x3": MATH_BF16X3, "mixed": MATH_MIXED}[os.environ.get("GNNRAG_MATH", "mixed")]


def set_dense_math(mode: int) -> int:
    global _default_math
    if mode not in (MATH_FP32, MATH_BF16X3, MATH_MIXED):
# ... 274 lines not shown
            out["edge%d" % d] = self._view(self.c.edge[d], 2 * self.F, torch.int32).numpy().reshape(-1, 2)
            out["perm%d" % d] = self._view(self.c.perm[d], self.F, torch.int32).numpy()
        nh = self._view(self.c.n_heavy, 2, torch.int32).numpy()
        out["n_heavy"] = nh
        for d in (0, 1):
            out["heavy%d" % d] = self._view(self.c.heavy[d], int(min(nh[d], self.c.heavy_cap)), torch.int32).numpy()
            out["hub_q_off%d" % d] = self._view(self.c.hub_q_off[d], self.B + 1, torch.int32).numpy()
            out["hub_wbase%d" % d] = self._view(self.c.hub_wbase[d], self.B + 1, torch.int32).numpy()
        for key, t in self._w.items():
            if isinstance(key, str):
                out[key] = t.cpu().numpy()
        nc = self._view(self.c.n_chunks, 2, torch.int32).numpy()
        out["n_chunks"] = nc
        bc = self._view(self.c.big_cnt, self.B, torch.int32).numpy()
        bn = self._view(self.c.big_nodes, BN, torch.int32).numpy().reshape(self.B, self.N)
        out["big"] = [np.sort(bn[b, : bc[b]]) for b in range(self.B)]
        for d in (0, 1):
            out["edge_l%d" % d] = self._view(self.c.edge_l[d], 2 * self.F, torch.int32).numpy().reshape(-1, 2)
        out["rel_off"] = self._view(self.c.rel_off, self.B + 1, torch.int32).numpy()
        out["rel_rows"] = self._view(self.c.rel_rows, 2 * self.rel_total, torch.int32).numpy().reshape(-1, 2)
        out["edge_m"] = self._view(self.c.edge_m, 4 * self.F, torch.int32).numpy().reshape(-1, 2)
        out["m_from"] = self._view(self.c.m_from, 2 * self.F, torch.int32).numpy()
        out["m_dst"] = self._view(self.c.m_dst, 2 * self.F, torch.int32).numpy()
        return out

    def rel_rows(self) -> np.ndarray:
        return self._view(self.c.rel_rows, 2 * self.rel_total, torch.int32).numpy().reshape(-1, 2)


def linear(A: torch.Tensor, W: torch.Tensor, bias: Optional[torch.Tensor] = None,
           add: Optional[torch.Tensor] = None, relu: bool = False, math: Optional[int] = None) -> torch.Tensor:
    lib = _lib.load()
    A = _chk(A, "A")
    W = _chk(W, "W")
    M, K = A.shape
    Nout = W.shape[0]
    if W.shape[1] != K:
        raise ValueError("W is %s, A is %s" % (tuple(W.shape), tuple(A.shape)))
    bias = None if bias is None else _chk(bias, "bias", shape=(Nout,))
    add_rows = 0
    if add is not None:
        add = _chk(add, "add")
        if add.shape[1] != Nout:
            raise ValueError("add must have %d columns" % Nout)
        add_rows = add.shape[0]
    out = _buf((M, Nout), torch.float32, A.device, "linear: out")
    with torch.cuda.device(A.device):
        _lib.check(lib.gnnrag_linear(A.data_ptr(), M, K, W.data_ptr(), _ptr(bias), _ptr(add), add_rows,
                                     int(relu), out.data_ptr(), Nout, _math(math), _stream()), "gnnrag_linear")
    return out


def rel_transform(relfeat: torch.Tensor, relfeat_inv: torch.Tensor, layers, planes: bool = False, packed: bool = False):
    if planes and packed:
        raise ValueError("planes and packed are two forms of the same operand: ask for one")
    lib = _lib.load()
    relfeat = _chk(relfeat, "rel_features")
    R1, D = relfeat.shape
    relfeat_inv = _chk(relfeat_inv, "rel_features_inv", shape=(R1, D))
    L = len(layers)
    params = (_lib.LayerParams * max(L, 1))()
    keep, pos_rows = [], 0
    for j, (W, b, pos, pos_inv) in enumerate(layers):
        W = _chk(W, "rel_linear.weight", shape=(D, D))
        b = _chk(b, "rel_linear.bias", shape=(D,))
        keep += [W, b]
        params[j].W_rel, params[j].b_rel = W.data_ptr(), b.data_ptr()
        if pos is not None:
            pos = _chk(pos, "pos_emb.weight")
            pos_inv = _chk(pos_inv, "pos_emb_inv.weight", shape=tuple(pos.shape))
            if pos.shape[1] != D or (pos_rows and pos.shape[0] != pos_rows):
                raise ValueError("pos_emb must be [rows, D], the same size in every layer")
            pos_rows = pos.shape[0]
            keep += [pos, pos_inv]
            params[j].pos_fwd, params[j].pos_inv = pos.data_ptr(), pos_inv.data_ptr()
    out = _buf((L, 2, R1, D), torch.float32, relfeat.device, "rel_transform: out")
    pl = None
    if planes:
        nbytes = lib.gnnrag_rel_planes_bytes(R1, D, L)
        if nbytes == 0:
            raise _lib.GnnragError("relation planes need a hidden size <= 224")
        pl = _buf((L, 2, 3, R1, nbytes // (L * 6 * R1 * 2)), torch.int16, relfeat.device, "rel_transform: planes")
    if packed:
        nbytes = lib.gnnrag_rel_packed_bytes(R1, D, L)
        if nbytes == 0:
            raise _lib.GnnragError("the packed relation operand needs a hidden size <= 224")
        pl = _buf((L, 2, R1, nbytes // (L * 2 * R1)), torch.uint8, relfeat.device, "rel_transform: packed")
    with torch.cuda.device(relfeat.device):
        if packed:
            _lib.check(lib.gnnrag_rel_transform_packed(relfeat.data_ptr(), relfeat_inv.data_ptr(), R1, D, L, params,
                                                       pos_rows, out.data_ptr(), _ptr(pl), _stream()),
                       "gnnrag_rel_transform_packed")
        else:
            _lib.check(lib.gnnrag_rel_transform(relfeat.data_ptr(), relfeat_inv.data_ptr(), R1, D, L, params, pos_rows,
                                                out.data_ptr(), _ptr(pl), _stream()), "gnnrag_rel_transform")
    return (out, pl) if planes or packed else out


def relation_tables_planes(plan: "CsrPlan", planes: torch.Tensor, ins: torch.Tensor, W_e2e: torch.Tensor) -> torch.Tensor:
    lib = _lib.load()
    ins = _chk(ins, "relational_ins")
    B, I, D = ins.shape
    if (planes.dtype != torch.int16 or tuple(planes.shape[:3]) != (2, 3, plan.R1) or not planes.is_contiguous()
            or B != plan.B):
        raise ValueError("planes must be a contiguous [2, 3, R1, 448] int16 tensor of this plan's relation count")
    W_e2e = _chk(W_e2e, "e2e_linear.weight", shape=(D, (2 * I + 1) * D))
    _on_plan_device(plan, ins, "relational_ins")
    P = _buf((2, max(plan.rel_total, 1), D), torch.float32, ins.device, "relation_tables_planes: P")
    with torch.cuda.device(ins.device):
        _lib.check(lib.gnnrag_relation_tables_planes(C.byref(plan.c), planes.data_ptr(), ins.data_ptr(), W_e2e.data_ptr(),
                                                     P.data_ptr(), D, I, _stream()), "gnnrag_relation_tables_planes")
    return P[:, :plan.rel_total]


def relation_tables_packed(plan: "CsrPlan", packed: torch.Tensor, ins: torch.Tensor, W_e2e: torch.Tensor,
                           only_dir: int = -1) -> torch.Tensor:
    lib = _lib.load()
    ins = _chk(ins, "relational_ins")
    B, I, D = ins.shape
    if (packed.dtype != torch.uint8 or packed.dim() != 3 or tuple(packed.shape[:2]) != (2, plan.R1)
            or not packed.is_contiguous() or B != plan.B):
        raise ValueError("packed must be a contiguous [2, R1, 1408] uint8 tensor of this plan's relation count")
    if only_dir not in (-1, 0, 1):
        raise ValueError("only_dir is -1, 0 or 1")
    W_e2e = _chk(W_e2e, "e2e_linear.weight", shape=(D, (2 * I + 1) * D))
    _on_plan_device(plan, ins, "relational_ins")
    P = _buf((2, max(plan.rel_total, 1), D), torch.float32, ins.device, "relation_tables_packed: P")
    if only_dir >= 0:
        P.zero_()
    with torch.cuda.device(ins.device):
        _lib.check(lib.gnnrag_relation_tables_packed(C.byref(plan.c), packed.data_ptr(), ins.data_ptr(), W_e2e.data_ptr(),
                                                     P.data_ptr(), D, I, only_dir, _stream()), "gnnrag_relation_tables_packed")
    return P[:, :plan.rel_total]


def gemm_tn(A: torch.Tensor, B: torch.Tensor) -> torch.Tensor:
    lib = _lib.load()
    A = _chk(A, "A")
    B = _chk(B, "B")
    if A.dim() != 2 or B.dim() != 2 or A.shape[0] != B.shape[0]:
        raise ValueError("A is %s, B is %s" % (tuple(A.shape), tuple(B.shape)))
    M, N1 = A.shape
    N2 = B.shape[1]
    out = _buf((N1, N2), torch.float32, A.device, "gemm_tn: C")
    with torch.cuda.device(A.device):
        ws = _buf(max(lib.gnnrag_gemm_tn_workspace_bytes(M, N1, N2), 16), torch.uint8, A.device, "gemm_tn: workspace")
        _lib.check(lib.gnnrag_gemm_tn(A.data_ptr(), B.data_ptr(), M, N1, N2, out.data_ptr(), ws.data_ptr(), ws.numel(),
                                      _stream()), "gnnrag_gemm_tn")
    return out


def aggregate(plan: CsrPlan, dist: torch.Tensor, ins: torch.Tensor, T_fwd: torch.Tensor,
              T_inv: torch.Tensor) -> torch.Tensor:
    lib = _lib.load()
    B, N = plan.B, plan.N
    ins = _chk(ins, "ins")
    _, I, D = ins.shape
    dist = _chk(dist, "dist").reshape(-1)
    _on_plan_device(plan, dist, "dist")
    if dist.numel() != B * N or ins.shape[0] != B:
        raise ValueError("dist/ins do not match the plan (B=%d, N=%d)" % (B, N))
    T_fwd = _chk(T_fwd, "T_fwd", shape=(plan.R1, D))
    T_inv = _chk(T_inv, "T_inv", shape=(plan.R1, D))
    agg = _buf((B * N, 2 * I * D), torch.float32, dist.device, "aggregate: agg")
    ws = plan.walk_workspace(D, I)
    with torch.cuda.device(dist.device):
        _lib.check(lib.gnnrag_aggregate(C.byref(plan.c), dist.data_ptr(), ins.data_ptr(), T_fwd.data_ptr(),
                                        T_inv.data_ptr(), agg.data_ptr(), D, I, ws.data_ptr(), ws.numel(),
                                        _stream()), "gnnrag_aggregate")
    return agg


def relation_tables(plan: CsrPlan, T_fwd: torch.Tensor, T_inv: torch.Tensor, ins: torch.Tensor,
                    W_e2e: torch.Tensor, math: Optional[int] = None) -> torch.Tensor:
    lib = _lib.load()
    ins = _chk(ins, "ins")
    B, I, D = ins.shape
    if B != plan.B:
        raise ValueError("ins has %d questions, the plan %d" % (B, plan.B))
    T_fwd = _chk(T_fwd, "T_fwd", shape=(plan.R1, D))
    T_inv = _chk(T_inv, "T_inv", shape=(plan.R1, D))
    W_e2e = _chk(W_e2e, "e2e_linear.weight", shape=(D, (2 * I + 1) * D))
    P = _buf((2, plan.rel_total, D), torch.float32, ins.device, "relation_tables: P")
    with torch.cuda.device(ins.device):
        _lib.check(lib.gnnrag_relation_tables(C.byref(plan.c), T_fwd.data_ptr(), T_inv.data_ptr(), ins.data_ptr(),
                                              W_e2e.data_ptr(), P.data_ptr(), D, I, _math(math), _stream()),
                   "gnnrag_relation_tables")
    return P


WALK_L2_GATHER, WALK_LDS_16, WALK_LDS_32 = 0, 1, 2
WALK_KERNEL_NAMES = {WALK_L2_GATHER: "k_walk_light_q / k_walk_light<FUSED> + hub kernels (table rows gathered from L2)",
                     WALK_LDS_16: "k_fact_prior_merged + k_walk_slice<FUSED,1> (16-column table slices in LDS, merged rows)",
                     WALK_LDS_32: "k_fact_prior_merged + k_walk_slice<FUSED,2> (32-column table slices in LDS, merged rows)"}


def aggregate_fused_variant(plan: CsrPlan, D: int) -> int:
    v = _lib.load().gnnrag_aggregate_fused_variant(C.byref(plan.c), int(D))
    if v < 0:
        _lib.check(v, "gnnrag_aggregate_fused_variant")
    return v


DENSE_ENTRIES = {"linear": 0, "linear_pair": 1, "update_score": 2, "update_score_fused": 3}
DENSE_MISALIGNED_A, DENSE_MISALIGNED_W, DENSE_MISALIGNED_C, DENSE_MISALIGNED_ADD, DENSE_MISALIGNED_A1 = 1, 2, 4, 8, 16
(DENSE_NONE, DENSE_SKINNY, DENSE_KTILED, DENSE_WRES, DENSE_UPDATE_SKINNY, DENSE_UPDATE_B3,
 DENSE_WIDE) = range(7)
DENSE_KERNEL_NAMES = {DENSE_NONE: "nothing launched", DENSE_SKINNY: "k_gemm_skinny", DENSE_KTILED: "k_gemm_f32",
                      DENSE_WRES: "k_gemm_wres", DENSE_UPDATE_SKINNY: "k_update_skinny", DENSE_UPDATE_B3: "k_update_b3",
                      DENSE_WIDE: "EPI_LINEAR column blocks + k_score_rows"}
DenseForm = collections.namedtuple("DenseForm", [n for n, _ in _lib.DenseFormStruct._fields_])


def dense_form(entry: str, M: int, K: int, Nout: int, math: Optional[int] = None, add_rows: Optional[int] = None,
               misaligned: int = 0, block: int = 0) -> DenseForm:
    out = _lib.DenseFormStruct()
    _lib.check(_lib.load().gnnrag_dense_form(DENSE_ENTRIES[entry], int(M), int(K), int(Nout), _math(math),
                                             int(add_rows is not None), int(add_rows or 0), int(misaligned), int(block),
                                             C.byref(out)), "gnnrag_dense_form")
    return DenseForm(*(getattr(out, n) for n in DenseForm._fields))


HUB_FORM_NONE, HUB_FORM_DENSE, HUB_FORM_CHUNKED = 0, 1, 2


def aggregate_fused_hub_form(plan: CsrPlan, D: int, I: int = 1) -> dict:
    lib = _lib.load()
    ws = plan.walk_workspace(D, I)
    form = _buf(4, torch.int32, ws.device, "aggregate_fused_hub_form: form", 0)
    with torch.cuda.device(ws.device):
        _lib.check(lib.gnnrag_aggregate_fused_hub_form(C.byref(plan.c), int(D), ws.data_ptr(), ws.numel(), form.data_ptr(),
                                                       _stream()), "gnnrag_aggregate_fused_hub_form")
    f = form.cpu().tolist()
    return {"form": f[0], "hubs": (f[1], f[2]), "relation_ranges": f[3]}


def aggregate_fused(plan: CsrPlan, dist: torch.Tensor, P: torch.Tensor) -> torch.Tensor:
    lib = _lib.load()
    B, N = plan.B, plan.N
    P = _chk(P, "P")
    D = P.shape[-1]
    if tuple(P.shape) != (2, plan.rel_total, D):
        raise ValueError("P must be [2, plan.rel_total, D]")
    dist = _chk(dist, "dist").reshape(-1)
    _on_plan_device(plan, dist, "dist")
    out = _buf((B * N, D), torch.float32, dist.device, "aggregate_fused: out")
    ws = plan.walk_workspace(D, 1)
    with torch.cuda.device(dist.device):
        _lib.check(lib.gnnrag_aggregate_fused(C.byref(plan.c), dist.data_ptr(), P.data_ptr(), out.data_ptr(), D,
                                              ws.data_ptr(), ws.numel(), _stream()), "gnnrag_aggregate_fused")
    return out


class Frontier:

    def __init__(self, plan: CsrPlan, dist: torch.Tensor):
        lib = _lib.load()
        self.plan = plan
        dist = _chk(dist, "dist").reshape(-1)
        _on_plan_device(plan, dist, "dist")
        if dist.numel() != plan.B * plan.N:
            raise ValueError("dist does not match the plan")
        self.dist = dist
        nbytes = max(lib.gnnrag_frontier_workspace_bytes(C.byref(plan.c)), 256)
        self.ws = _buf(nbytes, torch.uint8, dist.device, "frontier_build: fws")
        with torch.cuda.device(dist.device):
            _lib.check(lib.gnnrag_frontier_build(C.byref(plan.c), dist.data_ptr(), self.ws.data_ptr(), self.ws.numel(),
                                                 _stream()), "gnnrag_frontier_build")

    def read(self):
        counts = (C.c_int32 * 2)()
        flags = np.zeros(self.plan.B * self.plan.N, dtype=np.uint8)
        with torch.cuda.device(self.dist.device):
            _lib.check(_lib.load().gnnrag_frontier_read(C.byref(self.plan.c), self.ws.data_ptr(), counts,
                                                        flags.ctypes.data, _stream()), "gnnrag_frontier_read")
        return int(counts[0]), int(counts[1]), flags

    def relation_tables(self, T_fwd, T_inv, ins, W_e2e, P: Optional[torch.Tensor] = None) -> torch.Tensor:
        ins = _chk(ins, "ins")
        B, I, D = ins.shape
        T_fwd = _chk(T_fwd, "T_fwd", shape=(self.plan.R1, D))
        T_inv = _chk(T_inv, "T_inv", shape=(self.plan.R1, D))
        W_e2e = _chk(W_e2e, "e2e_linear.weight", shape=(D, (2 * I + 1) * D))
        if P is None:
            P = _buf((2, max(self.plan.rel_total, 1), D), torch.float32, ins.device, "relation_tables_frontier: P", float("nan"))
        with torch.cuda.device(ins.device):
            _lib.check(_lib.load().gnnrag_relation_tables_frontier(
                C.byref(self.plan.c), self.ws.data_ptr(), T_fwd.data_ptr(), T_inv.data_ptr(), ins.data_ptr(),
                W_e2e.data_ptr(), P.data_ptr(), D, I, _stream()), "gnnrag_relation_tables_frontier")
        return P

    def aggregate(self, P: torch.Tensor, out: Optional[torch.Tensor] = None) -> torch.Tensor:
        P = _chk(P, "P")
        D = P.shape[-1]
        if out is None:
            out = _buf((self.plan.B * self.plan.N, D), torch.float32, P.device, "aggregate_fused_frontier: out", 0)
        with torch.cuda.device(P.device):
            _lib.check(_lib.load().gnnrag_aggregate_fused_frontier(
                C.byref(self.plan.c), self.ws.data_ptr(), self.dist.data_ptr(), P.data_ptr(), out.data_ptr(), D,
                _stream()), "gnnrag_aggregate_fused_frontier")
        return out


def update_score_fused(h, nbr, W, b, w_s, b_s, mask, I: int, math: Optional[int] = None):
    lib = _lib.load()
    h = _chk(h, "h")
    BN, D = h.shape
    nbr = _chk(nbr, "nbr", shape=(BN, D))
    W = _chk(W, "W", shape=(D, (2 * I + 1) * D))
    b = _chk(b, "b", shape=(D,))
    w_s = _chk(w_s, "w_s").reshape(-1)
    b_s = _chk(b_s, "b_s").reshape(-1)
    mask = _chk(mask, "mask").reshape(-1)
    h_out = _buf(h.shape, torch.float32, h.device, "update_score_fused: h_out")
    score = _buf(BN, torch.float32, h.device, "update_score_fused: score")
    with torch.cuda.device(h.device):
        _lib.check(lib.gnnrag_update_score_fused(h.data_ptr(), nbr.data_ptr(), W.data_ptr(), b.data_ptr(),
                                                 w_s.data_ptr(), b_s.data_ptr(), mask.data_ptr(), h_out.data_ptr(),
                                                 score.data_ptr(), BN, D, I, _math(math), _stream()),
                   "gnnrag_update_score_fused")
    return h_out, score


def update_score(h, agg, W, b, w_s, b_s, mask, I: int, math: Optional[int] = None):
    lib = _lib.load()
    h = _chk(h, "h")
    BN, D = h.shape
    agg = _chk(agg, "agg", shape=(BN, 2 * I * D))
    W = _chk(W, "W", shape=(D, (2 * I + 1) * D))
    b = _chk(b, "b", shape=(D,))
    w_s = _chk(w_s, "w_s").reshape(-1)
    b_s = _chk(b_s, "b_s").reshape(-1)
    mask = _chk(mask, "mask").reshape(-1)
    if w_s.numel() != D or b_s.numel() != 1 or mask.numel() != BN:
        raise ValueError("score_func / mask shapes do not match")
    h_out = _buf(h.shape, torch.float32, h.device, "update_score: h_out")
    score = _buf(BN, torch.float32, h.device, "update_score: score")
    with torch.cuda.device(h.device):
        _lib.check(lib.gnnrag_update_score(h.data_ptr(), agg.data_ptr(), W.data_ptr(), b.data_ptr(),
                                           w_s.data_ptr(), b_s.data_ptr(), mask.data_ptr(), h_out.data_ptr(),
                                           score.data_ptr(), BN, D, I, _math(math), _stream()), "gnnrag_update_score")
    return h_out, score


def masked_softmax(score: torch.Tensor, B: int, N: int) -> torch.Tensor:
    lib = _lib.load()
    score = _chk(score, "score")
    if score.numel() != B * N:
        raise ValueError("score has %d entries, expected %d" % (score.numel(), B * N))
    dist = _buf((B, N), torch.float32, score.device, "masked_softmax: dist")
    with torch.cuda.device(score.device):
        _lib.check(lib.gnnrag_masked_softmax(score.data_ptr(), dist.data_ptr(), B, N, _stream()),
                   "gnnrag_masked_softmax")
    return dist


def typelayer(plan: CsrPlan, T: torch.Tensor, use_w_rel: bool) -> torch.Tensor:
    lib = _lib.load()
    T = _chk(T, "T")
    _on_plan_device(plan, T, "T")
    D = T.shape[1]
    if T.shape[0] != plan.R1:
        raise ValueError("T has %d rows, plan has R1=%d" % (T.shape[0], plan.R1))
    h0 = _buf((plan.B * plan.N, D), torch.float32, T.device, "typelayer: h0")
    ws = plan.walk_workspace(D, 1)
    with torch.cuda.device(T.device):
        _lib.check(lib.gnnrag_typelayer(C.byref(plan.c), T.data_ptr(), int(use_w_rel), h0.data_ptr(), D,
                                        ws.data_ptr(), ws.numel(), _stream()), "gnnrag_typelayer")
    return h0


def aggregate_backward(plan: CsrPlan, dist, ins, T_fwd, T_inv, g_agg, gather: bool = True):
    lib = _lib.load()
    B, N = plan.B, plan.N
    ins = _chk(ins, "ins")
    _, I, D = ins.shape
    dist = _chk(dist, "dist").reshape(-1)
    T_fwd = _chk(T_fwd, "T_fwd", shape=(plan.R1, D))
    T_inv = _chk(T_inv, "T_inv", shape=(plan.R1, D))
    g_agg = _chk(g_agg, "g_agg", shape=(B * N, 2 * I * D))
    g_dist = _buf(B * N, torch.float32, dist.device, "aggregate_backward: g_dist")
    g_ins = _buf(ins.shape, torch.float32, ins.device, "aggregate_backward: g_ins")
    g_Tf = _buf(T_fwd.shape, torch.float32, T_fwd.device, "aggregate_backward: g_T_fwd")
    g_Ti = _buf(T_inv.shape, torch.float32, T_inv.device, "aggregate_backward: g_T_inv")
    ro = plan.relorder() if (gather and D % 4 == 0 and I <= 4) else None
    ws = plan.backward_workspace(D, I, ro)
    with torch.cuda.device(dist.device):
        _lib.check(lib.gnnrag_aggregate_backward(
            C.byref(plan.c), None if ro is None else C.byref(ro), dist.data_ptr(), ins.data_ptr(), T_fwd.data_ptr(),
            T_inv.data_ptr(), g_agg.data_ptr(),
            g_dist.data_ptr(), g_ins.data_ptr(), g_Tf.data_ptr(), g_Ti.data_ptr(), D, I, ws.data_ptr(), ws.numel(),
            _stream()), "gnnrag_aggregate_backward")
    return g_dist, g_ins, g_Tf, g_Ti


def aggregate_fused_backward(plan: CsrPlan, dist, P, g_nbr):
    lib = _lib.load()
    P = _chk(P, "P")
    D = P.shape[-1]
    if tuple(P.shape) != (2, plan.rel_total, D) or D % 4:
        raise ValueError("P must be [2, plan.rel_total, D] with D % 4 == 0")
    dist = _chk(dist, "dist").reshape(-1)
    g_nbr = _chk(g_nbr, "g_nbr", shape=(plan.B * plan.N, D))
    g_dist = _buf(plan.B * plan.N, torch.float32, dist.device, "aggregate_fused_backward: g_dist")
    g_P = _buf(P.shape, torch.float32, P.device, "aggregate_fused_backward: g_P", 0 if plan.rel_total == 0 else None)
    ro = plan.relorder()
    ws = plan.backward_workspace(D, 1, ro)
    with torch.cuda.device(dist.device):
        _lib.check(lib.gnnrag_aggregate_fused_backward(
            C.byref(plan.c), C.byref(ro), dist.data_ptr(), P.data_ptr(), g_nbr.data_ptr(), g_dist.data_ptr(),
            g_P.data_ptr(), D, ws.data_ptr(), ws.numel(), _stream()), "gnnrag_aggregate_fused_backward")
    return g_dist, g_P


def typelayer_backward(plan: CsrPlan, g_pre: torch.Tensor, use_w_rel: bool, gather: bool = True) -> torch.Tensor:
    lib = _lib.load()
    g_pre = _chk(g_pre, "g_pre")
    D = g_pre.shape[1]
    if g_pre.shape[0] != plan.B * plan.N:
        raise ValueError("g_pre has %d rows, the plan %d nodes" % (g_pre.shape[0], plan.B * plan.N))
    g_T = _buf((plan.R1, D), torch.float32, g_pre.device, "typelayer_backward: g_T")
    ro = plan.relorder() if (gather and D % 4 == 0) else None
    w_src = plan._w.get(("w_rel_src",)) if use_w_rel else None
    if use_w_rel and w_src is None:
        raise ValueError("use_w_rel needs attach_w_rel first")
    ws = plan.backward_workspace(D, 1, ro)
    with torch.cuda.device(g_pre.device):
        _lib.check(lib.gnnrag_typelayer_backward(C.byref(plan.c), None if ro is None else C.byref(ro), g_pre.data_ptr(),
                                                 _ptr(w_src), int(use_w_rel), g_T.data_ptr(), D, ws.data_ptr(),
                                                 ws.numel(), _stream()), "gnnrag_typelayer_backward")
    return g_T


class LayerWorkspace:

    def __init__(self):
        self.key = None
        self.buf = None

    def get(self, plan: "CsrPlan", D, I, device) -> torch.Tensor:
        nbytes = max(_lib.load().gnnrag_layer_workspace_bytes(C.byref(plan.c), D, I), 256)
        if self.key != str(device) or self.buf is None or self.buf.numel() < nbytes:
            self.buf = None
            self.buf = _buf(nbytes, torch.uint8, device, "reason_layer: workspace")
            self.key = str(device)
        return self.buf


def reason_layer(plan: CsrPlan, h, dist, ins, relfeat, relfeat_inv, W_rel, b_rel, W_e2e, b_e2e, w_score,
                 b_score, mask, pos=None, pos_inv=None, ws: Optional[LayerWorkspace] = None,
                 path: int = _lib.PATH_AUTO, math: Optional[int] = None):
    lib = _lib.load()
    B, N, R1 = plan.B, plan.N, plan.R1
    ins = _chk(ins, "ins")
    _, I, D = ins.shape
    h = _chk(h, "h").reshape(B * N, D)
    _on_plan_device(plan, h, "local_entity_emb")
    dist = _chk(dist, "dist").reshape(-1)
    mask = _chk(mask, "mask").reshape(-1)
    relfeat = _chk(relfeat, "rel_features", shape=(R1, D))
    relfeat_inv = _chk(relfeat_inv, "rel_features_inv", shape=(R1, D))
    W_rel = _chk(W_rel, "rel_linear.weight", shape=(D, D))
    b_rel = _chk(b_rel, "rel_linear.bias", shape=(D,))
    W_e2e = _chk(W_e2e, "e2e_linear.weight", shape=(D, (2 * I + 1) * D))
    b_e2e = _chk(b_e2e, "e2e_linear.bias", shape=(D,))
    w_score = _chk(w_score, "score_func.weight").reshape(-1)
    b_score = _chk(b_score, "score_func.bias").reshape(-1)
    if dist.numel() != B * N or mask.numel() != B * N or ins.shape[0] != B or w_score.numel() != D:
        raise ValueError("layer inputs do not match the plan (B=%d, N=%d, D=%d)" % (B, N, D))
    pos_rows = 0
    if pos is not None:
        pos = _chk(pos, "pos_emb.weight")
        pos_inv = _chk(pos_inv, "pos_emb_inv.weight", shape=tuple(pos.shape))
        pos_rows = pos.shape[0]
        if pos.shape[1] != D or pos_rows > R1:
            raise ValueError("pos_emb must be [<=R1, D]")
    ws = ws or LayerWorkspace()
    wbuf = ws.get(plan, D, I, h.device)
    h_out = _buf((B, N, D), torch.float32, h.device, "reason_layer: h_out")
    score = _buf((B, N), torch.float32, h.device, "reason_layer: score")
    dist_out = _buf((B, N), torch.float32, h.device, "reason_layer: dist_out")
    with torch.cuda.device(h.device):
        _lib.check(lib.gnnrag_reason_layer(
            C.byref(plan.c), h.data_ptr(), dist.data_ptr(), ins.data_ptr(), relfeat.data_ptr(),
            relfeat_inv.data_ptr(), W_rel.data_ptr(), b_rel.data_ptr(), _ptr(pos), _ptr(pos_inv), pos_rows,
            W_e2e.data_ptr(), b_e2e.data_ptr(), w_score.data_ptr(), b_score.data_ptr(), mask.data_ptr(),
            h_out.data_ptr(), score.data_ptr(), dist_out.data_ptr(), wbuf.data_ptr(), wbuf.numel(), D, I,
            int(path), _math(math), _stream()), "gnnrag_reason_layer")
    return h_out, score, dist_out


class LayerStack:

    def __init__(self, plan: CsrPlan, relfeat, relfeat_inv, layers, w_score, b_score, mask, I: int,
                 path: int = _lib.PATH_AUTO, math: Optional[int] = None):
        lib = _lib.load()
        B, N, R1 = plan.B, plan.N, plan.R1
        relfeat = _chk(relfeat, "rel_features")
        D = relfeat.shape[1]
        _on_plan_device(plan, relfeat, "rel_features")
        self.plan, self.B, self.N, self.D, self.I, self.L = plan, B, N, D, int(I), len(layers)
        self.path, self.math = int(path), _math(math)
        keep = [relfeat, _chk(relfeat_inv, "rel_features_inv", shape=(R1, D)),
                _chk(w_score, "score_func.weight").reshape(-1), _chk(b_score, "score_func.bias").reshape(-1),
                _chk(mask, "mask").reshape(-1)]
        if tuple(relfeat.shape) != (R1, D) or keep[2].numel() != D or keep[4].numel() != B * N:
            raise ValueError("layer stack inputs do not match the plan (B=%d, N=%d, R1=%d, D=%d)" % (B, N, R1, D))
        self._relfeat, self._relfeat_inv, self._ws, self._bs, self._mask = keep
        self._params = (_lib.LayerParams * self.L)()
        self.pos_rows = 0
        for j, (W_rel, b_rel, W_e2e, b_e2e, pos, pos_inv) in enumerate(layers):
            t = [_chk(W_rel, "rel_linear.weight", shape=(D, D)), _chk(b_rel, "rel_linear.bias", shape=(D,)),
                 _chk(W_e2e, "e2e_linear.weight", shape=(D, (2 * self.I + 1) * D)),
                 _chk(b_e2e, "e2e_linear.bias", shape=(D,))]
            if pos is not None:
                pos = _chk(pos, "pos_emb.weight")
                pos_inv = _chk(pos_inv, "pos_emb_inv.weight", shape=tuple(pos.shape))
                if pos.shape[1] != D or pos.shape[0] > R1 or (self.pos_rows and pos.shape[0] != self.pos_rows):
                    raise ValueError("pos_emb must be [<=R1, D], the same size in every layer")
                self.pos_rows = pos.shape[0]
                t += [pos, pos_inv]
            keep += t
            pr = self._params[j]
            pr.W_rel, pr.b_rel, pr.W_e2e, pr.b_e2e = (x.data_ptr() for x in t[:4])
            pr.pos_fwd, pr.pos_inv = (t[4].data_ptr(), t[5].data_ptr()) if pos is not None else (None, None)
        self._keep = keep
        self.device = relfeat.device
        nbytes = max(lib.gnnrag_stack_workspace_bytes(C.byref(plan.c), self.L, D, self.I), 256)
        self._ws_buf = _buf(nbytes, torch.uint8, self.device, "reason_stack: workspace")
        self._graph = self._graph_rest = None
        self.h = self.score = self.dist = None
        self._proj_valid = False

    def new_forward(self):
        self._proj_valid = False

    def _new_outputs(self):
        f32, dev, L, B, N, D = torch.float32, self.device, self.L, self.B, self.N, self.D
        return (_buf((L, B, N, D), f32, dev, "reason_stack: h_out"), _buf((L, B, N), f32, dev, "reason_stack: score"),
                _buf((L, B, N), f32, dev, "reason_stack: dist_out"))

    def _args(self, h0, dist0, ins, out, reuse=False):
        h, score, dist = out
        return (C.byref(self.plan.c), self.L, self._params, h0.data_ptr(), dist0.data_ptr(), ins.data_ptr(),
                self._relfeat.data_ptr(), self._relfeat_inv.data_ptr(), self.pos_rows, self._ws.data_ptr(),
                self._bs.data_ptr(), self._mask.data_ptr(), h.data_ptr(), score.data_ptr(),
                dist.data_ptr(), self._ws_buf.data_ptr(), self._ws_buf.numel(), self.D, self.I,
                self.path | (_lib.PATH_REUSE_PROJ if reuse else 0), self.math)

    def _inputs(self, h0, dist0, ins):
        h0 = _chk(h0, "local_entity_emb").reshape(self.B * self.N, self.D)
        dist0 = _chk(dist0, "dist").reshape(-1)
        ins = _chk(ins, "relational_ins", shape=(self.B, self.I, self.D))
        if dist0.numel() != self.B * self.N:
            raise ValueError("dist does not match the plan")
        _on_plan_device(self.plan, h0, "local_entity_emb")
        return h0, dist0, ins

    def run(self, h0, dist0, ins):
        h0, dist0, ins = self._inputs(h0, dist0, ins)
        out = self._new_outputs()
        reuse = self._proj_valid and self.L > 1
        with torch.cuda.device(h0.device):
            _lib.check(_lib.load().gnnrag_reason_stack(*self._args(h0, dist0, ins, out, reuse), _stream()),
                       "gnnrag_reason_stack")
        self._proj_valid = True
        return out

    def capture(self, h0, dist0, ins):
        if self.L < 2:
            raise ValueError("graph replay needs num_gnn >= 2 (layer 0 reads the buffer the last layer writes)")
        self.release_graph()
        self.h, self.score, self.dist = self._new_outputs()
        self.h[self.L - 1].copy_(h0.reshape(self.B, self.N, self.D))
        h0g, dist0, ins = self._inputs(self.h[self.L - 1], dist0, ins)
        g, g2 = C.c_void_p(), C.c_void_p()
        with torch.cuda.device(h0g.device):
            side = torch.cuda.Stream()
            side.wait_stream(torch.cuda.current_stream())
            with torch.cuda.stream(side):
                _lib.check(_lib.load().gnnrag_reason_stack_capture(
                    *self._args(h0g, dist0, ins, (self.h, self.score, self.dist)), _stream(), C.byref(g)),
                    "gnnrag_reason_stack_capture")
                _lib.check(_lib.load().gnnrag_reason_stack_capture(
                    *self._args(h0g, dist0, ins, (self.h, self.score, self.dist), reuse=True), _stream(), C.byref(g2)),
                    "gnnrag_reason_stack_capture")
            torch.cuda.current_stream().wait_stream(side)
        self._graph, self._graph_rest, self._graph_in = g, g2, (dist0, ins)

    def capture_rest(self, h_prev, dist0, ins):
        if self.L < 2:
            raise ValueError("graph replay needs num_gnn >= 2 (layer 0 reads the buffer the last layer writes)")
        if not self._proj_valid:
            raise RuntimeError("capture_rest() needs the projections of an eager run() in the workspace")
        self.release_graph()
        self.h, self.score, self.dist = self._new_outputs()
        self._ins_buf = _buf((self.B, self.I, self.D), torch.float32, self.device, "reason_stack_capture: ins")
        self.h[self.L - 1].copy_(h_prev.reshape(self.B, self.N, self.D))
        self._ins_buf.copy_(ins)
        h0g, dist0, insb = self._inputs(self.h[self.L - 1], dist0, self._ins_buf)
        g2 = C.c_void_p()
        with torch.cuda.device(h0g.device):
            side = torch.cuda.Stream()
            side.wait_stream(torch.cuda.current_stream())
            with torch.cuda.stream(side):
                _lib.check(_lib.load().gnnrag_reason_stack_capture(
# ... 894 lines not shown
```

### include/gnnrag.h

```cpp
#ifndef GNNRAG_H_
#define GNNRAG_H_

#include <stddef.h>
#include <stdint.h>

#ifdef __cplusplus
extern "C" {
#endif

#define GNNRAG_ABI_VERSION 16

#define GNNRAG_E_BADARG      (-1)
#define GNNRAG_E_UNSUPPORTED (-2)
#define GNNRAG_E_WORKSPACE   (-3)
#define GNNRAG_E_TUPLE       (-4)

typedef void* gnnrag_stream_t;

typedef struct gnnrag_csr {
  int32_t B;
  int32_t N;
  int32_t R1;
  int32_t heavy_deg;
  int64_t F;
  int32_t* row_ptr[2];
  int32_t* edge[2];
  int32_t* perm[2];
  float*   w_gnn[2];
  float*   w_rel[2];
  int32_t* heavy[2];
  int32_t* chunk_off[2];
  int32_t* n_heavy;
  int32_t* n_chunks;
  int32_t  heavy_cap;
  int32_t  max_chunks;
  int32_t* big_cnt;
  int32_t* big_nodes;
  int32_t  big_deg;
  int32_t  hub_sorted;
  int32_t* edge_l[2];
  int32_t* rel_off;
  int32_t* rel_rows;
  int32_t  rel_total;
  int32_t  rel_max;
  int32_t* edge_m;
  int32_t* m_from;
  int32_t* m_dst;
  int32_t* hub_q_off[2];
  int32_t* hub_wbase[2];
} gnnrag_csr;

size_t gnnrag_csr_bytes(int64_t F, int32_t B, int32_t N, int32_t R1, int has_w_gnn, int has_w_rel);
size_t gnnrag_csr_scratch_bytes(int64_t F, int32_t B, int32_t N, int32_t R1);

int gnnrag_csr_build(const int32_t* heads, const int32_t* rels, const int32_t* tails,
                     const float* w_gnn, const float* w_rel,
                     int64_t F, int32_t B, int32_t N, int32_t R1,
                     void* csr_mem, size_t csr_bytes, void* scratch, size_t scratch_bytes,
                     gnnrag_csr* out, gnnrag_stream_t stream);

int gnnrag_csr_build_counts(const int32_t* heads, const int32_t* rels, const int32_t* tails,
                            const float* w_gnn, const float* w_rel,
                            int64_t F, int32_t B, int32_t N, int32_t R1, int32_t rel_total, int32_t rel_max,
                            void* csr_mem, size_t csr_bytes, void* scratch, size_t scratch_bytes,
                            gnnrag_csr* out, gnnrag_stream_t stream);
int gnnrag_csr_status(const gnnrag_csr* csr, gnnrag_stream_t stream);

int gnnrag_csr_concat(const gnnrag_csr* const* parts, int32_t B, int32_t N, int32_t R1, void* csr_mem, size_t csr_bytes,
                      gnnrag_csr* out, gnnrag_stream_t stream);

int gnnrag_narrow_tuple(const int64_t* heads, const int64_t* rels, const int64_t* tails, int64_t F,
                        int32_t* out, int32_t nthreads);

int gnnrag_csr_permute_weight(const gnnrag_csr* csr, const float* w_per_fact, int square,
                              float* out_fwd, float* out_inv, gnnrag_stream_t stream);

#define GNNRAG_MATH_FP32   0
#define GNNRAG_MATH_BF16X3 1
#define GNNRAG_MATH_MIXED  2

int gnnrag_linear(const float* A, int64_t M, int32_t K, const float* W, const float* bias,
                  const float* add, int64_t add_rows, int relu,
                  float* C, int32_t Nout, int32_t math, gnnrag_stream_t stream);

int gnnrag_linear_pair(const float* A0, const float* A1, int64_t M, int32_t K, const float* W,
                       const float* bias, const float* add0, const float* add1, int64_t add_rows,
                       float* C0, float* C1, int32_t Nout, int32_t math, gnnrag_stream_t stream);

size_t gnnrag_aggregate_workspace_bytes(const gnnrag_csr* csr, int32_t D, int32_t I);
int gnnrag_aggregate(const gnnrag_csr* csr, const float* dist, const float* ins,
                     const float* T_fwd, const float* T_inv, float* agg,
                     int32_t D, int32_t I, void* workspace, size_t workspace_bytes,
                     gnnrag_stream_t stream);

int gnnrag_aggregate_fused(const gnnrag_csr* csr, const float* dist, const float* P, float* out,
                           int32_t D, void* workspace, size_t workspace_bytes,
                           gnnrag_stream_t stream);

#define GNNRAG_WALK_L2_GATHER 0
#define GNNRAG_WALK_LDS_16    1
#define GNNRAG_WALK_LDS_32    2
int gnnrag_aggregate_fused_variant(const gnnrag_csr* csr, int32_t D);

#define GNNRAG_HUB_FORM_NONE    0
#define GNNRAG_HUB_FORM_DENSE   1
#define GNNRAG_HUB_FORM_CHUNKED 2
int gnnrag_aggregate_fused_hub_form(const gnnrag_csr* csr, int32_t D, void* workspace, size_t workspace_bytes,
                                    int32_t* form_dev, gnnrag_stream_t stream);

int gnnrag_update_score(const float* h, const float* agg, const float* W, const float* b,
                        const float* w_s, const float* b_s, const float* mask,
                        float* h_out, float* score, int64_t BN, int32_t D, int32_t I, int32_t math,
                        gnnrag_stream_t stream);

int gnnrag_masked_softmax(const float* score, float* dist, int32_t B, int32_t N,
                          gnnrag_stream_t stream);

int gnnrag_typelayer(const gnnrag_csr* csr, const float* T, int use_w_rel, float* h0,
                     int32_t D, void* workspace, size_t workspace_bytes, gnnrag_stream_t stream);

typedef struct gnnrag_relorder {
  int64_t  F;
  int32_t  rel_total;
  int32_t  n_chunks;
  int32_t* ht;
  int32_t* perm;
  float*   w;
  int32_t* row_ptr;
  int32_t* chunk_ptr;
} gnnrag_relorder;
size_t gnnrag_relorder_bytes(const gnnrag_csr* csr, int has_w);
size_t gnnrag_relorder_scratch_bytes(const gnnrag_csr* csr);
int gnnrag_relorder_build(const gnnrag_csr* csr, const int32_t* heads, const int32_t* rels,
                          const int32_t* tails, const float* w_per_fact,
                          void* mem, size_t mem_bytes, void* scratch, size_t scratch_bytes,
                          gnnrag_relorder* out, gnnrag_stream_t stream);

size_t gnnrag_backward_workspace_bytes(const gnnrag_csr* csr, const gnnrag_relorder* relorder, int32_t D,
                                       int32_t I);
int gnnrag_aggregate_backward(const gnnrag_csr* csr, const gnnrag_relorder* relorder,
                              const float* dist, const float* ins,
                              const float* T_fwd, const float* T_inv, const float* g_agg,
                              float* g_dist, float* g_ins, float* g_T_fwd, float* g_T_inv,
                              int32_t D, int32_t I, void* workspace, size_t workspace_bytes,
                              gnnrag_stream_t stream);

int gnnrag_aggregate_fused_backward(const gnnrag_csr* csr, const gnnrag_relorder* relorder, const float* dist,
                                    const float* P, const float* g_nbr, float* g_dist, float* g_P, int32_t D,
                                    void* workspace, size_t workspace_bytes, gnnrag_stream_t stream);

int gnnrag_typelayer_backward(const gnnrag_csr* csr, const gnnrag_relorder* relorder, const float* g_pre,
                              const float* w_rel_per_fact, int use_w_rel, float* g_T,
                              int32_t D, void* workspace, size_t workspace_bytes, gnnrag_stream_t stream);

size_t gnnrag_gemm_tn_workspace_bytes(int64_t M, int32_t N1, int32_t N2);
int gnnrag_gemm_tn(const float* A, const float* B, int64_t M, int32_t N1, int32_t N2, float* C,
                   void* workspace, size_t workspace_bytes, gnnrag_stream_t stream);

int gnnrag_relation_tables(const gnnrag_csr* csr, const float* T_fwd, const float* T_inv, const float* ins,
                           const float* W_e2e, float* P, int32_t D, int32_t I, int32_t math,
                           gnnrag_stream_t stream);

int gnnrag_update_score_fused(const float* h, const float* nbr, const float* W_e2e, const float* b,
                              const float* w_s, const float* b_s, const float* mask,
                              float* h_out, float* score, int64_t BN, int32_t D, int32_t I, int32_t math,
                              gnnrag_stream_t stream);

#define GNNRAG_DENSE_ENTRY_LINEAR       0
#define GNNRAG_DENSE_ENTRY_LINEAR_PAIR  1
#define GNNRAG_DENSE_ENTRY_UPDATE       2
#define GNNRAG_DENSE_ENTRY_UPDATE_FUSED 3
#define GNNRAG_DENSE_MISALIGNED_A   1
#define GNNRAG_DENSE_MISALIGNED_W   2
#define GNNRAG_DENSE_MISALIGNED_C   4
#define GNNRAG_DENSE_MISALIGNED_ADD 8
#define GNNRAG_DENSE_MISALIGNED_A1  16
#define GNNRAG_DENSE_NONE          0
#define GNNRAG_DENSE_SKINNY        1
#define GNNRAG_DENSE_KTILED        2
#define GNNRAG_DENSE_WRES          3
#define GNNRAG_DENSE_UPDATE_SKINNY 4
#define GNNRAG_DENSE_UPDATE_B3     5
#define GNNRAG_DENSE_WIDE          6
typedef struct gnnrag_dense_form_t {
  int32_t family;
  int32_t block_family;
  int32_t launches;
  int32_t epi;
  int32_t nt, mt, v4, math, nw;
  int32_t v4out, n0;
  int32_t nc, has_add, kguard;
} gnnrag_dense_form_t;
int gnnrag_dense_form(int32_t entry, int64_t M, int32_t K, int32_t Nout, int32_t math, int32_t has_add, int64_t add_rows,
                      int32_t misaligned, int32_t block, gnnrag_dense_form_t* out);

#define GNNRAG_PATH_AUTO    0
#define GNNRAG_PATH_UNFUSED 1
#define GNNRAG_PATH_FUSED   2
#define GNNRAG_PATH_ONLY_FWD 0x10
#define GNNRAG_PATH_ONLY_INV 0x20
#define GNNRAG_PATH_SEED_PRIOR 0x40
#define GNNRAG_PATH_REUSE_PROJ 0x80
size_t gnnrag_layer_workspace_bytes(const gnnrag_csr* csr, int32_t D, int32_t I);
int gnnrag_reason_layer(const gnnrag_csr* csr,
                        const float* h, const float* dist, const float* ins,
                        const float* relfeat_fwd, const float* relfeat_inv,
                        const float* W_rel, const float* b_rel,
                        const float* pos_fwd, const float* pos_inv, int32_t pos_rows,
                        const float* W_e2e, const float* b_e2e,
                        const float* w_score, const float* b_score, const float* mask,
                        float* h_out, float* score_out, float* dist_out,
                        void* workspace, size_t workspace_bytes,
                        int32_t D, int32_t I, int32_t path, int32_t math, gnnrag_stream_t stream);

typedef struct gnnrag_layer_params {
  const float* W_rel;
  const float* b_rel;
  const float* pos_fwd;
  const float* pos_inv;
  const float* W_e2e;
  const float* b_e2e;
} gnnrag_layer_params;
size_t gnnrag_stack_workspace_bytes(const gnnrag_csr* csr, int32_t L, int32_t D, int32_t I);

size_t gnnrag_rel_planes_bytes(int64_t R1, int32_t D, int32_t L);
int gnnrag_rel_transform(const float* relfeat_fwd, const float* relfeat_inv, int64_t R1, int32_t D, int32_t L,
                         const gnnrag_layer_params* layers, int32_t pos_rows, float* T_out, void* planes_out,
                         gnnrag_stream_t stream);

int gnnrag_relation_tables_planes(const gnnrag_csr* csr, const void* planes, const float* ins, const float* W,
                                  float* P, int32_t D, int32_t I, gnnrag_stream_t stream);

size_t gnnrag_rel_packed_bytes(int64_t R1, int32_t D, int32_t L);
int gnnrag_rel_transform_packed(const float* relfeat_fwd, const float* relfeat_inv, int64_t R1, int32_t D, int32_t L,
                                const gnnrag_layer_params* layers, int32_t pos_rows, float* T_out, void* packed_out,
                                gnnrag_stream_t stream);
int gnnrag_relation_tables_packed(const gnnrag_csr* csr, const void* packed, const float* ins, const float* W,
                                  float* P, int32_t D, int32_t I, int32_t only_dir, gnnrag_stream_t stream);

int gnnrag_reason_stack(const gnnrag_csr* csr, int32_t L, const gnnrag_layer_params* layers,
                        const float* h0, const float* dist0, const float* ins,
                        const float* relfeat_fwd, const float* relfeat_inv, int32_t pos_rows,
                        const float* w_score, const float* b_score, const float* mask,
                        float* h_out, float* score_out, float* dist_out,
                        void* workspace, size_t workspace_bytes,
                        int32_t D, int32_t I, int32_t path, int32_t math, gnnrag_stream_t stream);

typedef struct gnnrag_graph gnnrag_graph;
int gnnrag_reason_stack_capture(const gnnrag_csr* csr, int32_t L, const gnnrag_layer_params* layers,
                                const float* h0, const float* dist0, const float* ins,
                                const float* relfeat_fwd, const float* relfeat_inv, int32_t pos_rows,
                                const float* w_score, const float* b_score, const float* mask,
                                float* h_out, float* score_out, float* dist_out,
                                void* workspace, size_t workspace_bytes,
                                int32_t D, int32_t I, int32_t path, int32_t math, gnnrag_stream_t stream,
                                gnnrag_graph** out);
int gnnrag_graph_launch(gnnrag_graph* graph, gnnrag_stream_t stream);
int gnnrag_graph_destroy(gnnrag_graph* graph);

size_t gnnrag_frontier_workspace_bytes(const gnnrag_csr* csr);
int gnnrag_frontier_supported(const gnnrag_csr* csr, int32_t D);
int gnnrag_frontier_build(const gnnrag_csr* csr, const float* dist, void* fws, size_t fws_bytes, gnnrag_stream_t stream);
int gnnrag_relation_tables_frontier(const gnnrag_csr* csr, const void* fws, const float* T_fwd, const float* T_inv,
                                    const float* ins, const float* W_e2e, float* P, int32_t D, int32_t I,
                                    gnnrag_stream_t stream);
int gnnrag_aggregate_fused_frontier(const gnnrag_csr* csr, const void* fws, const float* dist, const float* P,
                                    float* out, int32_t D, gnnrag_stream_t stream);
int gnnrag_frontier_read(const gnnrag_csr* csr, const void* fws, int32_t* counts2, uint8_t* row_flag_host,
                         gnnrag_stream_t stream);

int gnnrag_topp_candidates(const float* pred_dist, const uint8_t* eligible, int32_t B, int32_t N,
                           double ignore_prob, double eps, int32_t* out_slot, int32_t* out_cnt,
                           gnnrag_stream_t stream);
size_t gnnrag_topp_workspace_bytes(int32_t B, int32_t N);
int gnnrag_topp_candidates_ws(const float* pred_dist, const uint8_t* eligible, int32_t B, int32_t N,
                              double ignore_prob, double eps, int32_t* out_slot, int32_t* out_cnt,
                              void* workspace, size_t workspace_bytes, gnnrag_stream_t stream);

int gnnrag_seed_retrieve(const float* seed_info, const float* ent_emb, float* out, int32_t B, int32_t N,
                         int32_t D, gnnrag_stream_t stream);

int gnnrag_query_reform(const float* q_node, const float* seed_info, const float* ent_emb, int64_t ld_ent,
                        const float* W_r, const float* W_g, float* out, int32_t B, int32_t N, int32_t D,
                        gnnrag_stream_t stream);

#define GNNRAG_MAX_REFORMS 8
#define GNNRAG_QUERY_REFORM_MAX_D 4096
size_t gnnrag_query_reform_reserve_bytes(int32_t B, int32_t D, int32_t n);
int gnnrag_query_reform_train(const float* const* q, const float* seed_info, const float* ent_emb, int64_t ld_ent,
                              const float* const* W_r, const float* const* W_g, float* out, void* reserve,
                              size_t reserve_bytes, int32_t B, int32_t N, int32_t D, int32_t n, gnnrag_stream_t stream);

size_t gnnrag_query_reform_backward_workspace_bytes(int32_t B, int32_t N, int32_t D, int32_t n);
int gnnrag_query_reform_backward(const float* const* q, const float* seed_info, const float* const* W_r,
                                 const float* const* W_g, const void* reserve, size_t reserve_bytes,
                                 const float* const* g_out, float* const* dq, float* const* dW_r, float* const* dW_g,
                                 float* d_ent, int32_t B, int32_t N, int32_t D, int32_t n, void* workspace,
                                 size_t workspace_bytes, gnnrag_stream_t stream);

#define GNNRAG_LAYER_TAIL_MAX_D 4096
int gnnrag_layer_tail_train(const float* pre_a, const float* pre_b, const uint8_t* keep, float scale,
                            const float* w_score, const float* b_score, const float* mask, int32_t B, int32_t N, int32_t D,
                            float* h_out, float* score, float* dist, gnnrag_stream_t stream);

size_t gnnrag_layer_tail_backward_workspace_bytes(int32_t B, int32_t N, int32_t D);
int gnnrag_layer_tail_backward(const float* h, const float* dist, const uint8_t* keep, float scale, const float* w_score,
                               const float* g_h, const float* g_dist, int32_t B, int32_t N, int32_t D, float* g_pre,
                               float* dw_score, float* db_score, void* workspace, size_t workspace_bytes,
                               gnnrag_stream_t stream);

size_t gnnrag_kl_loss_workspace_bytes(int32_t B);
int gnnrag_kl_loss_train(const float* pred, const float* teacher, const float* label_valid, int32_t B, int32_t N,
                         float* loss, float* reserve, void* workspace, size_t workspace_bytes, gnnrag_stream_t stream);

int gnnrag_kl_loss_backward(const float* g_loss, const float* pred, const float* teacher, const float* label_valid,
                            const float* reserve, int32_t B, int32_t N, float* d_pred, gnnrag_stream_t stream);

#define GNNRAG_TRAIN_METRICS_MAX_N 16384
int gnnrag_train_metrics(const float* pred, const float* answer, const float* seed, const int64_t* local_entity,
                         int64_t pad_id, double eps, int32_t B, int32_t N, int32_t* out_pred, float* out_h1, float* out_f1,
                         int32_t* out_cnt, gnnrag_stream_t stream);

size_t gnnrag_lstm_workspace_bytes(int32_t E, int32_t H);
int gnnrag_lstm_forward(const float* x, const float* w_ih, const float* w_hh, const float* b_ih, const float* b_hh,
                        const float* h0, const float* c0, float* out, float* h_n, float* c_n, int32_t B, int32_t T,
                        int32_t E, int32_t H, void* workspace, size_t workspace_bytes, gnnrag_stream_t stream);

size_t gnnrag_lstm_reserve_bytes(int32_t B, int32_t T, int32_t H);
int gnnrag_lstm_forward_train(const float* x, const float* w_ih, const float* w_hh, const float* b_ih,
                              const float* b_hh, const float* h0, const float* c0, float* out, float* h_n, float* c_n,
                              int32_t B, int32_t T, int32_t E, int32_t H, void* reserve, size_t reserve_bytes,
                              void* workspace, size_t workspace_bytes, gnnrag_stream_t stream);

size_t gnnrag_lstm_backward_workspace_bytes(int32_t B, int32_t T, int32_t E, int32_t H);
int gnnrag_lstm_backward(const float* x, const float* w_ih, const float* w_hh, const float* h0, const float* c0,
                         const float* out, const void* reserve, size_t reserve_bytes, const float* g_out,
                         const float* g_hn, const float* g_cn, float* dx, float* dw_ih, float* dw_hh, float* db,
                         float* dh0, float* dc0, int32_t B, int32_t T, int32_t E, int32_t H, void* workspace,
                         size_t workspace_bytes, gnnrag_stream_t stream);

#define GNNRAG_MAX_INS 8
int gnnrag_instructions(const float* hidden, const float* node, const float* mask, const float* r_in,
                        const float* const* W_q, const float* const* b_q, const float* W_cq, const float* b_cq,
                        const float* w_ca, const float* b_ca, int32_t B, int32_t T, int32_t D, int32_t n_steps,
                        float* ins_out, float* attn_out, gnnrag_stream_t stream);

size_t gnnrag_instructions_reserve_bytes(int32_t B, int32_t T, int32_t D, int32_t n_steps);
int gnnrag_instructions_train(const float* hidden, const float* node, const float* mask, const float* r_in,
                              const float* const* W_q, const float* const* b_q, const float* W_cq, const float* b_cq,
                              const float* w_ca, const float* b_ca, const float* drop_node, const float* drop_cat,
                              const float* drop_tok, int32_t B, int32_t T, int32_t D, int32_t n_steps, float* ins_out,
                              float* attn_out, void* reserve, size_t reserve_bytes, gnnrag_stream_t stream);

size_t gnnrag_instructions_backward_workspace_bytes(int32_t B, int32_t T, int32_t D, int32_t n_steps);
int gnnrag_instructions_backward(const float* hidden, const float* node, const float* r_in, const float* const* W_q,
                                 const float* W_cq, const float* w_ca, const float* drop_node, const float* drop_cat,
                                 const float* drop_tok, const float* ins, const float* attn, const void* reserve,
                                 size_t reserve_bytes, const float* g_ins, const float* g_attn, float* dhidden,
                                 float* dnode, float* dr_in, float* const* dW_q, float* const* db_q, float* dW_cq,
                                 float* db_cq, float* dw_ca, float* db_ca, int32_t B, int32_t T, int32_t D,
                                 int32_t n_steps, void* workspace, size_t workspace_bytes, gnnrag_stream_t stream);

typedef struct gnnrag_bert_layer { const float *W_qkv, *b_qkv, *W_o, *b_o, *ln1_g, *ln1_b,
                                               *W_i, *b_i, *W_f, *b_f, *ln2_g, *ln2_b; } gnnrag_bert_layer;
size_t gnnrag_bert_workspace_bytes(int32_t B, int32_t T, int32_t H, int32_t I);
int gnnrag_bert_attention(const float* qkv, int32_t B, int32_t T, int32_t heads, int32_t dh, float* ctx,
                          gnnrag_stream_t stream);
int gnnrag_bert_encode(const int64_t* ids, const float* word_emb, int32_t vocab, const float* pos_emb, int32_t max_pos,
                       const float* type_emb, const float* ln_g, const float* ln_b, float ln_eps,
                       int32_t L, const gnnrag_bert_layer* layers, int32_t B, int32_t T, int32_t H, int32_t heads,
                       int32_t I, float* out , void* ws, size_t ws_bytes, int32_t math,
                       gnnrag_stream_t stream);
int gnnrag_bert_attention_bias(const float* qkv, int32_t B, int32_t T, int32_t heads, int32_t dh,
                               const float* rel_bias , float* ctx, gnnrag_stream_t stream);
int gnnrag_bert_encode_ex(const int64_t* ids, const float* word_emb, int32_t vocab, const float* pos_emb, int32_t max_pos,
                          const float* type_emb , int32_t pad_id ,
                          const float* rel_bias , const float* ln_g, const float* ln_b,
                          float ln_eps, int32_t L, const gnnrag_bert_layer* layers, int32_t B, int32_t T, int32_t H,
                          int32_t heads, int32_t I, float* out , void* ws, size_t ws_bytes, int32_t math,
                          gnnrag_stream_t stream);

size_t gnnrag_bert_keep_hidden_bytes(int32_t L, int32_t B, int32_t T, int32_t H);
size_t gnnrag_bert_keep_att_bytes(int32_t L, int32_t B, int32_t T, int32_t heads);
int gnnrag_bert_attention_drop(const float* qkv, int32_t B, int32_t T, int32_t heads, int32_t dh,
                               const float* rel_bias , const uint8_t* keep ,
                               float scale, float* ctx, gnnrag_stream_t stream);
int gnnrag_bert_encode_train(const int64_t* ids, const float* word_emb, int32_t vocab, const float* pos_emb,
                             int32_t max_pos, const float* type_emb , int32_t pad_id, const float* rel_bias,
                             const float* ln_g, const float* ln_b, float ln_eps, int32_t L,
                             const gnnrag_bert_layer* layers, int32_t B, int32_t T, int32_t H, int32_t heads, int32_t I,
                             const uint8_t* keep_hidden , float scale_hidden,
                             const uint8_t* keep_att , float scale_att, float* out , void* ws,
                             size_t ws_bytes, int32_t math, gnnrag_stream_t stream);

#define GNNRAG_REL_TEXT_MAX_T 256
#define GNNRAG_REL_TEXT_MAX_K 4096
#define GNNRAG_REL_TEXT_MAX_D 4096
size_t gnnrag_rel_text_workspace_bytes(int64_t R, int32_t T, int32_t K, int32_t D, int32_t n_dir);
int gnnrag_rel_text_pool(const float* X_fwd, const float* X_inv, const float* mask, const float* W, const float* b,
                         const float* a, int64_t R, int32_t T, int32_t K, int32_t D, float* out_fwd, float* out_inv,
                         float* xbar, float* alpha, void* workspace, size_t workspace_bytes, gnnrag_stream_t stream);

size_t gnnrag_rel_text_backward_workspace_bytes(int64_t R, int32_t T, int32_t K, int32_t D, int32_t n_dir);
int gnnrag_rel_text_pool_backward(const float* X_fwd, const float* X_inv, const float* W, const float* a,
                                  const float* xbar, const float* alpha, const float* g_fwd, const float* g_inv,
                                  int64_t R, int32_t T, int32_t K, int32_t D, float* dW, float* db, float* da,
                                  void* workspace, size_t workspace_bytes, gnnrag_stream_t stream);

typedef struct gnnrag_ugraph {
  int32_t B;
  int32_t N;
  int64_t F;
  int64_t cap;
  int32_t* u_ptr;
  int32_t* u_adj;
} gnnrag_ugraph;

size_t gnnrag_ugraph_bytes(int64_t F, int32_t B, int32_t N);
size_t gnnrag_ugraph_scratch_bytes(int64_t F, int32_t B, int32_t N);
int gnnrag_ugraph_build(const gnnrag_csr* csr, void* mem, size_t mem_bytes, void* scratch, size_t scratch_bytes,
                        gnnrag_ugraph* out, gnnrag_stream_t stream);

size_t gnnrag_paths_workspace_bytes(int32_t B, int32_t N, int32_t max_seeds, int32_t max_cands);
size_t gnnrag_paths_out_bytes(int32_t B, int32_t max_seeds, int32_t max_cands, int32_t max_paths, int32_t max_hops);
int gnnrag_shortest_paths(const gnnrag_ugraph* graph, const uint8_t* seed_flag, const int32_t* cand_slot,
                          const int32_t* cand_cnt, int32_t max_seeds, int32_t max_cands, int32_t max_paths,
                          int32_t max_hops, int32_t* q_info, int32_t* pair_info, int32_t* path_off, int32_t* path_nodes,
                          int32_t* path_facts, void* workspace, size_t workspace_bytes, gnnrag_stream_t stream);

size_t gnnrag_rule_paths_workspace_bytes(int64_t F, int32_t B, int32_t N, int32_t max_rules, int32_t max_hops);
size_t gnnrag_rule_paths_out_bytes(int32_t B, int32_t max_seeds, int32_t max_rules, int32_t max_paths, int32_t max_hops);
int gnnrag_rule_paths(const gnnrag_ugraph* graph, const int32_t* fact_rel, const uint8_t* seed_flag,
                      const int32_t* rule_rel, const int32_t* rule_len, int32_t max_seeds, int32_t max_rules,
                      int32_t max_paths, int32_t max_hops, int32_t* q_info, int32_t* pair_info, int32_t* path_off,
                      int32_t* path_nodes, int32_t* path_facts, void* workspace, size_t workspace_bytes,
                      gnnrag_stream_t stream);

int gnnrag_stream_copy(const float* src, float* dst, int64_t n, gnnrag_stream_t stream);

int gnnrag_abi_version(void);
const char* gnnrag_error_string(int code);

#ifdef __cplusplus
}
#endif
#endif
```

Measured before the change: 3.165 billion.

## Fuse frontier build and relation transform into one seed prologue kernel

Merges the frontier-build kernel and the relation-projection GEMM into a single launch, with the first B blocks building the per-batch frontier and the remaining blocks computing relation transforms. This removes a kernel launch and lets the two independent prologue stages run concurrently on the GPU. The shared bodies move to a common header. The frontier part now runs at 256 threads per block instead of 1024, and the relation transform is forced to one tile per block, which may slow either stage.

Result: faster. 3.205 billion, median of 6 (+1.3%).

```diff
diff --git a/gnn-rag_amd/_lib.py b/gnn-rag_amd/_lib.py
--- a/gnn-rag_amd/_lib.py
+++ b/gnn-rag_amd/_lib.py
@@ -140,6 +140,10 @@
                                                   C.c_int32, _VP]),
     "gnnrag_aggregate_fused_frontier": (C.c_int, [C.POINTER(CsrStruct), _VP, _VP, _VP, _VP, C.c_int32, _VP]),
     "gnnrag_frontier_read": (C.c_int, [C.POINTER(CsrStruct), _VP, _VP, _VP, _VP]),
+    "gnnrag_frontier_layout": (C.c_int, [C.POINTER(CsrStruct), C.POINTER(C.c_uint64)]),
+    "gnnrag_seed_prologue": (C.c_int, [C.POINTER(CsrStruct), _VP, _VP, C.c_size_t, _VP, C.c_int64, _VP, C.c_int64, _VP, _VP,
+                                      C.c_int32, C.c_int32, C.POINTER(LayerParams), C.c_int32, _VP, _VP,
+                                      C.POINTER(C.c_int32), _VP]),
     "gnnrag_instructions": (C.c_int, [_VP] * 4 + [C.POINTER(C.c_void_p)] * 2 + [_VP] * 4 + [C.c_int32] * 4 + [_VP] * 3),
     "gnnrag_instructions_reserve_bytes": (C.c_size_t, [C.c_int32] * 4),
     "gnnrag_instructions_train": (C.c_int, [_VP] * 4 + [C.POINTER(C.c_void_p)] * 2 + [_VP] * 7 + [C.c_int32] * 4 +
diff --git a/gnn-rag_amd/csrc/dense_internal.h b/gnn-rag_amd/csrc/dense_internal.h
--- a/gnn-rag_amd/csrc/dense_internal.h
+++ b/gnn-rag_amd/csrc/dense_internal.h
@@ -23,6 +23,9 @@
 int frontier_build_z(const gnnrag_csr* csr, const float* dist, void* fws, size_t fws_bytes, float* zero_a,
                      int64_t zero_na, float* zero_b, int64_t zero_nb, hipStream_t stream);
 const uint8_t* frontier_row_flags(const gnnrag_csr* csr, const void* fws);
+struct FrontierArgs;
+int frontier_args(const gnnrag_csr* csr, const float* dist, void* fws, size_t fws_bytes, float* zero_a, int64_t zero_na,
+                  float* zero_b, int64_t zero_nb, FrontierArgs* a);
 
 int update_score_fused_z(const float* h, const float* nbr, const float* W, const float* b, const float* w_s,
                          const float* b_s, const float* mask, float* h_out, float* score, int64_t BN, int32_t D,
@@ -33,5 +36,9 @@
 int rel_transform_launch(const float* relfeat_fwd, const float* relfeat_inv, int64_t R1, int32_t D, int32_t L,
                          const gnnrag_layer_params* layers, int32_t pos_rows, float* T_out, void* planes_out,
                          void* packed_out, gnnrag_stream_t stream);
+int seed_prologue_launch(const gnnrag_csr* csr, const float* dist, void* fws, size_t fws_bytes, float* zero_a,
+                         int64_t zero_na, float* zero_b, int64_t zero_nb, const float* relfeat_fwd,
+                         const float* relfeat_inv, int32_t D, int32_t L, const gnnrag_layer_params* layers,
+                         int32_t pos_rows, float* T_out, void* packed_out, gnnrag_stream_t stream);
 
 }
diff --git a/gnn-rag_amd/csrc/frontier.hip b/gnn-rag_amd/csrc/frontier.hip
--- a/gnn-rag_amd/csrc/frontier.hip
+++ b/gnn-rag_amd/csrc/frontier.hip
@@ -1,4 +1,5 @@
 #include "dense_internal.h"
+#include "seed_prologue.h"
 
 namespace gnnrag {
 
@@ -33,88 +34,11 @@
     int32_t* __restrict__ trows, int32_t* __restrict__ counts, int32_t* __restrict__ seeds,
     int32_t* __restrict__ seedinfo, float* __restrict__ zero_a, long long zero_na, float* __restrict__ zero_b,
     long long zero_nb) {
+  static_assert(kFrSeedCap == kSpSeedCap && kFrAltSeeds == kSpAltSeeds, "k_seed_prologue builds the same frontier");
   __shared__ int s_seed[kFrSeedCap];
-  __shared__ int s_ns, s_wsum[kFrThreads / 64];
-  const int g = blockIdx.x, tid = threadIdx.x, lane = tid & 63, wave = tid >> 6;
-  const int roff = rel_off[g], Rg = rel_off[g + 1] - roff;
-  const size_t n0 = (size_t)g * N;
-  for (long long i = (long long)blockIdx.x * kFrThreads + tid; i < zero_na; i += (long long)gridDim.x * kFrThreads) zero_a[i] = 0.f;
-  for (long long i = (long long)blockIdx.x * kFrThreads + tid; i < zero_nb; i += (long long)gridDim.x * kFrThreads) zero_b[i] = 0.f;
-  if (tid == 0) s_ns = 0;
-  if (g == (int)gridDim.x - 1 && tid < 64) row_flag[(size_t)gridDim.x * N + tid] = 0;
-  for (int i = tid; i < N; i += kFrThreads) row_flag[n0 + i] = 0;
-  for (int i = tid; i < Rg; i += kFrThreads) tflag[roff + i] = 0;
-  __syncthreads();
-  for (int i = tid; i < N; i += kFrThreads) {
-    if (dist[n0 + i] != 0.f) {
-      const int k = atomicAdd(&s_ns, 1);
-      if (k < kFrSeedCap) s_seed[k] = (int)n0 + i;
-    }
-  }
-  __syncthreads();
-  const int ns = s_ns;
-  if (tid == 0) {
-    int cnt = -1, facts = 0;
-    if (ns <= kFrAltSeeds) {
-      cnt = ns;
-      for (int i = 1; i < ns; ++i) {
-        const int v = s_seed[i];
-        int j = i - 1;
-        for (; j >= 0 && s_seed[j] > v; --j) s_seed[j + 1] = s_seed[j];
-        s_seed[j + 1] = v;
-      }
-      for (int i = 0; i < ns; ++i) {
-        const int sn = s_seed[i];
-        seeds[g * kFrAltSeeds + i] = sn;
-        facts += (rp0[sn + 1] - rp0[sn]) + (rp1[sn + 1] - rp1[sn]);
-      }
-    }
-    seedinfo[2 * g] = cnt;
-    seedinfo[2 * g + 1] = facts;
-  }
-  __syncthreads();
-  if (ns > kFrSeedCap) {
-    for (int i = tid; i < N; i += kFrThreads) row_flag[n0 + i] = 1;
-    for (int i = tid; i < Rg; i += kFrThreads) tflag[roff + i] = 1;
-  } else {
-    for (int k = 0; k < ns; ++k) {
-      const int s = s_seed[k];
-#pragma unroll
-      for (int dd = 0; dd < 2; ++dd) {
-        const int32_t* rp = dd ? rp1 : rp0;
-        const int2* el = dd ? el1 : el0;
-        const int beg = rp[s], end = rp[s + 1];
-        for (int j = beg + tid; j < end; j += kFrThreads) {
-          const int2 e = el[j];
-          row_flag[e.x] = 1;
-          tflag[roff + e.y] = 1;
-        }
-      }
-    }
-  }
-  __syncthreads();
-  auto compact = [&](const uint8_t* flag, int n, int first, int32_t* list, int32_t* count_out) {
-    int base = 0;
-    for (int c0 = 0; c0 < n; c0 += kFrThreads) {
-      const int i = c0 + tid;
-      const bool on = i < n && flag[i] != 0;
-      const unsigned long long m = __ballot(on);
-      if (lane == 0) s_wsum[wave] = __popcll(m);
-      __syncthreads();
-      int off = base, tot = 0;
-      for (int w = 0; w < kFrThreads / 64; ++w) {
-        const int c = s_wsum[w];
-        if (w < wave) off += c;
-        tot += c;
-      }
-      if (on) list[off + __popcll(m & ((1ull << lane) - 1))] = first + i;
-      base += tot;
-      __syncthreads();
-    }
-    if (tid == 0) *count_out = base;
-  };
-  compact(row_flag + n0, N, (int)n0, rows + n0, counts + 2 * g);
-  compact(tflag + roff, Rg, roff, trows + roff, counts + 2 * g + 1);
+  __shared__ int s_ns, s_wsum[kFrPass / 64];
+  frontier_body<kFrThreads, kFrSeedCap, kFrAltSeeds>(dist, rp0, rp1, el0, el1, rel_off, N, row_flag, rows, tflag, trows, counts, seeds, seedinfo,
+                            zero_a, zero_na, zero_b, zero_nb, (int)blockIdx.x, (int)gridDim.x, s_seed, s_ns, s_wsum);
 }
 
 struct TabFrArgs {
@@ -367,19 +291,43 @@
   return csr && csr->edge_m && csr->m_from && D > 0 && D % 4 == 0 && D <= 256 ? 1 : 0;
 }
 
+int gnnrag::frontier_args(const gnnrag_csr* csr, const float* dist, void* fws, size_t fws_bytes, float* zero_a,
+                          int64_t zero_na, float* zero_b, int64_t zero_nb, FrontierArgs* a) {
+  if (!csr || !dist || !fws || !a) return GNNRAG_E_BADARG;
+  const FrontierWs w = frontier_ws(csr);
+  if (fws_bytes < w.total) return GNNRAG_E_WORKSPACE;
+  char* base = (char*)fws;
+  a->dist = dist;
+  a->rp0 = csr->row_ptr[0]; a->rp1 = csr->row_ptr[1];
+  a->el0 = (const int2*)csr->edge_l[0]; a->el1 = (const int2*)csr->edge_l[1];
+  a->rel_off = csr->rel_off;
+  a->row_flag = (uint8_t*)(base + w.row_flag); a->rows = (int32_t*)(base + w.rows);
+  a->tflag = (uint8_t*)(base + w.tflag); a->trows = (int32_t*)(base + w.trows);
+  a->counts = (int32_t*)(base + w.counts); a->seeds = (int32_t*)(base + w.seeds);
+  a->seedinfo = (int32_t*)(base + w.seedinfo);
+  a->zero_a = zero_a; a->zero_na = (long long)zero_na; a->zero_b = zero_b; a->zero_nb = (long long)zero_nb;
+  a->N = csr->N; a->B = csr->B;
+  return 0;
+}
+
 int gnnrag::frontier_build_z(const gnnrag_csr* csr, const float* dist, void* fws, size_t fws_bytes, float* zero_a,
                              int64_t zero_na, float* zero_b, int64_t zero_nb, hipStream_t stream) {
   if (!csr || !dist || !fws) return GNNRAG_E_BADARG;
+  FrontierArgs a;
+  const int rc = frontier_args(csr, dist, fws, fws_bytes, zero_a, zero_na, zero_b, zero_nb, &a);
+  if (rc) return rc;
+  hipLaunchKernelGGL(k_frontier_build, dim3(csr->B), dim3(kFrThreads), 0, stream, a.dist, a.rp0, a.rp1, a.el0, a.el1,
+                     a.rel_off, a.N, a.row_flag, a.rows, a.tflag, a.trows, a.counts, a.seeds, a.seedinfo, a.zero_a,
+                     a.zero_na, a.zero_b, a.zero_nb);
+  GNNRAG_LAUNCH_CHECK();
+  return 0;
+}
+
+extern "C" int gnnrag_frontier_layout(const gnnrag_csr* csr, uint64_t* offsets8) {
+  if (!csr || !offsets8) return GNNRAG_E_BADARG;
   const FrontierWs w = frontier_ws(csr);
-  if (fws_bytes < w.total) return GNNRAG_E_WORKSPACE;
-  char* base = (char*)fws;
-  hipLaunchKernelGGL(k_frontier_build, dim3(csr->B), dim3(kFrThreads), 0, stream, dist, csr->row_ptr[0], csr->row_ptr[1],
-                     (const int2*)csr->edge_l[0], (const int2*)csr->edge_l[1], csr->rel_off, csr->N,
-                     (uint8_t*)(base + w.row_flag), (int32_t*)(base + w.rows), (uint8_t*)(base + w.tflag),
-                     (int32_t*)(base + w.trows), (int32_t*)(base + w.counts), (int32_t*)(base + w.seeds),
-                     (int32_t*)(base + w.seedinfo), zero_a, (long long)zero_na, zero_b,
-                     (long long)zero_nb);
-  GNNRAG_LAUNCH_CHECK();
+  const size_t o[8] = {w.counts, w.row_flag, w.rows, w.tflag, w.trows, w.seeds, w.seedinfo, w.total};
+  for (int i = 0; i < 8; ++i) offsets8[i] = (uint64_t)o[i];
   return 0;
 }
 
diff --git a/gnn-rag_amd/csrc/rel_transform.hip b/gnn-rag_amd/csrc/rel_transform.hip
--- a/gnn-rag_amd/csrc/rel_transform.hip
+++ b/gnn-rag_amd/csrc/rel_transform.hip
@@ -1,128 +1,27 @@
 #include "gnnrag_common.h"
 #include "dense_internal.h"
+#include "seed_prologue.h"
 
 namespace gnnrag {
-
-constexpr int kRtMaxL = 8;
-constexpr int kRtUnroll = 7;
-
-struct RelTArgs {
-  const float* A[2];
-  const float* W[kRtMaxL];
-  const float* b[kRtMaxL];
-  const float* add[kRtMaxL][2];
-  float* C;
-  unsigned short* planes;
-  unsigned char* packed;
-  int M, K, N, add_rows;
-};
-
-constexpr int kPlaneHalf = 224;
-constexpr int kPlaneRow = 2 * kPlaneHalf;
-constexpr int kPackPlaneB = kPlaneHalf * 2;
-constexpr int kPackIdxB = 3 * kPackPlaneB;
-constexpr int kPackRowB = kPackIdxB + 64;
 
 template <int TPW>
 __global__ __launch_bounds__(256) void k_rel_transform(RelTArgs g) {
   extern __shared__ __attribute__((aligned(16))) float Wf[];
-  const int tid = threadIdx.x, lane = tid & 63, wave = tid >> 6;
-  const int fr = lane & 15, fg = lane >> 4;
-  const int j = blockIdx.z >> 1, d = blockIdx.z & 1;
-  const int colg = blockIdx.y * 64;
-  const int K = g.K;
-  const int nch = (K + 15) >> 4;
-  const f32x4 zero4 = {0.f, 0.f, 0.f, 0.f};
-  const bool compute = colg < g.N;
-  if (compute) {
-    const int total = 64 * nch * 4;
-    for (int x = tid; x < total; x += 256) {
-      const int col = x / (nch * 4), kq = x - col * (nch * 4);
-      f32x4 v = zero4;
-      if (colg + col < g.N && 4 * kq < K) v = *reinterpret_cast<const f32x4*>(g.W[j] + (size_t)(colg + col) * K + 4 * kq);
-      const int c = kq >> 2, fgq = kq & 3, a = col & 3, frq = col >> 2;
-      *reinterpret_cast<f32x4*>(Wf + ((size_t)((c * 4 + a) * 64 + fgq * 16 + frq)) * 4) = v;
-    }
+  rel_transform_body<TPW>(g, (int)blockIdx.x, (int)blockIdx.y, (int)blockIdx.z, Wf);
+}
+
+constexpr int kSpThreads = 256;
+__global__ __launch_bounds__(kSpThreads) void k_seed_prologue(RelTArgs g, FrontierArgs f, int gx, int gy) {
+  extern __shared__ __attribute__((aligned(16))) float Wf[];
+  if ((int)blockIdx.x < f.B) {
+    int* s = reinterpret_cast<int*>(Wf);
+    frontier_body<kSpThreads>(f.dist, f.rp0, f.rp1, f.el0, f.el1, f.rel_off, f.N, f.row_flag, f.rows, f.tflag, f.trows,
+                              f.counts, f.seeds, f.seedinfo, f.zero_a, f.zero_na, f.zero_b, f.zero_nb, (int)blockIdx.x, f.B,
+                              s, s[kSpSeedCap], s + kSpSeedCap + 1);
+    return;
   }
-  __syncthreads();
-  const int c4 = colg + 4 * fr;
-  const bool in_T = c4 < g.N;
-  const bool in_pad = !in_T && c4 < kPlaneHalf;
-  f32x4 bias = zero4;
-  if (in_T && g.b[j]) bias = *reinterpret_cast<const f32x4*>(g.b[j] + c4);
-  const float* __restrict__ addp = g.add[j][d];
-  float* __restrict__ cp = g.C + ((size_t)(2 * j + d) * g.M) * g.N;
-  unsigned short* pp = g.planes ? g.planes + ((size_t)(2 * j + d) * 3 * g.M) * kPlaneRow : nullptr;
-  unsigned char* pk = g.packed ? g.packed + ((size_t)(2 * j + d) * g.M) * kPackRowB : nullptr;
-
-#pragma unroll 1
-  for (int t = 0; t < TPW; ++t) {
-    const int row0 = (blockIdx.x * TPW + t) * 64 + wave * 16;
-    if (row0 >= g.M) break;
-    f32x4 acc[4][2];
-#pragma unroll
-    for (int a = 0; a < 4; ++a) acc[a][0] = acc[a][1] = zero4;
-    if (compute) {
-      const float* __restrict__ ap = g.A[d] + (size_t)min(row0 + fr, g.M - 1) * K;
-      for (int c0 = 0; c0 < nch; c0 += kRtUnroll) {
-        f32x4 av[kRtUnroll];
-#pragma unroll
-        for (int u = 0; u < kRtUnroll; ++u)
-          av[u] = *reinterpret_cast<const f32x4*>(ap + min(16 * (c0 + u) + 4 * fg, K - 4));
-#pragma unroll
-        for (int u = 0; u < kRtUnroll; ++u) {
-          const int c = min(c0 + u, nch - 1);
-          const bool live = 16 * (c0 + u) + 4 * fg < K;
-          const f32x4 x = live ? av[u] : zero4;
-          f32x4 wv[4];
-#pragma unroll
-          for (int a = 0; a < 4; ++a) wv[a] = *reinterpret_cast<const f32x4*>(Wf + ((size_t)((c * 4 + a) * 64 + lane)) * 4);
-#pragma unroll
-          for (int e = 0; e < 4; ++e)
-#pragma unroll
-            for (int a = 0; a < 4; ++a)
-              acc[a][e & 1] = __builtin_amdgcn_mfma_f32_16x16x4f32(x[e], wv[a][e], acc[a][e & 1], 0, 0, 0);
-        }
-      }
-    }
-    if (!in_T && !(pp && in_pad) && !pk) continue;
-#pragma unroll
-    for (int r = 0; r < 4; ++r) {
-      const int row = row0 + 4 * fg + r;
-      if (row >= g.M) continue;
-      f32x4 v = zero4;
-      if (in_T) {
-#pragma unroll
-        for (int a = 0; a < 4; ++a) v[a] = acc[a][0][r] + acc[a][1][r];
-        v += bias;
-        if (addp && row < g.add_rows) v += *reinterpret_cast<const f32x4*>(addp + (size_t)row * g.N + c4);
-        *reinterpret_cast<f32x4*>(cp + (size_t)row * g.N + c4) = v;
-      }
-      if (pp) {
-#pragma unroll
-        for (int half = 0; half < 2; ++half) {
-          const Split3 sp = split3(__builtin_elementwise_max(half ? -v : v, zero4));
-          const size_t e = (size_t)row * kPlaneRow + half * kPlaneHalf + c4;
-          *reinterpret_cast<uint2*>(pp + e) = sp.hi;
-          *reinterpret_cast<uint2*>(pp + (size_t)g.M * kPlaneRow + e) = sp.mid;
-          *reinterpret_cast<uint2*>(pp + (size_t)2 * g.M * kPlaneRow + e) = sp.lo;
-        }
-      }
-      if (pk) {
-        unsigned char* rowp = pk + (size_t)row * kPackRowB;
-        if (c4 < kPlaneHalf) {
-          const Split3 sp = split3(__builtin_elementwise_abs(v));
-          *reinterpret_cast<uint2*>(rowp + 2 * c4) = sp.hi;
-          *reinterpret_cast<uint2*>(rowp + kPackPlaneB + 2 * c4) = sp.mid;
-          *reinterpret_cast<uint2*>(rowp + 2 * kPackPlaneB + 2 * c4) = sp.lo;
-        }
-        const int q = c4 >> 2;
-        const unsigned ix = 0x88u | (unsigned)(v[0] < 0.f) | (unsigned)(v[1] < 0.f) << 2 | (unsigned)(v[2] < 0.f) << 4 |
-                            (unsigned)(v[3] < 0.f) << 6;
-        rowp[kPackIdxB + ((q & 7) >> 1) * 16 + (q >> 3) * 2 + (q & 1)] = (unsigned char)(c4 < kPlaneHalf ? ix : 0u);
-      }
-    }
-  }
+  const int r = (int)blockIdx.x - f.B;
+  rel_transform_body<1>(g, r % gx, (r / gx) % gy, r / (gx * gy), Wf);
 }
 
 }
@@ -203,6 +102,64 @@
   return 0;
 }
 
+int gnnrag::seed_prologue_launch(const gnnrag_csr* csr, const float* dist, void* fws, size_t fws_bytes, float* zero_a,
+                                 int64_t zero_na, float* zero_b, int64_t zero_nb, const float* relfeat_fwd,
+                                 const float* relfeat_inv, int32_t D, int32_t L, const gnnrag_layer_params* layers,
+                                 int32_t pos_rows, float* T_out, void* packed_out, gnnrag_stream_t stream) {
+  if (!csr || !relfeat_fwd || !relfeat_inv || !layers || !T_out || D <= 0 || L <= 0 || pos_rows < 0) return GNNRAG_E_BADARG;
+  for (int j = 0; j < L; ++j) {
+    if (!layers[j].W_rel) return GNNRAG_E_BADARG;
+    if ((layers[j].pos_fwd == nullptr) != (layers[j].pos_inv == nullptr)) return GNNRAG_E_BADARG;
+  }
+  const int64_t R1 = csr->R1;
+  if (L > kRtMaxL || R1 <= 0 || R1 > 2048 || csr->B <= 0) return GNNRAG_E_UNSUPPORTED;
+  if (!gnnrag::rel_transform_accepts(relfeat_fwd, relfeat_inv, R1, D, L, layers, pos_rows, T_out, packed_out))
+    return GNNRAG_E_UNSUPPORTED;
+  FrontierArgs f;
+  int rc = frontier_args(csr, dist, fws, fws_bytes, zero_a, zero_na, zero_b, zero_nb, &f);
+  if (rc) return rc;
+  RelTArgs g;
+  memset(&g, 0, sizeof(g));
+  g.A[0] = relfeat_fwd;
+  g.A[1] = relfeat_inv;
+  for (int j = 0; j < L; ++j) {
+    g.W[j] = layers[j].W_rel;
+    g.b[j] = layers[j].b_rel;
+    g.add[j][0] = pos_rows > 0 ? layers[j].pos_fwd : nullptr;
+    g.add[j][1] = pos_rows > 0 ? layers[j].pos_inv : nullptr;
+  }
+  g.C = T_out;
+  g.packed = (unsigned char*)packed_out;
+  g.M = (int)R1; g.K = D; g.N = D;
+  g.add_rows = (int)(pos_rows < R1 ? pos_rows : R1);
+  const int gx = (int)((R1 + 63) / 64), gy = ((packed_out ? kPlaneHalf : D) + 63) / 64, gz = 2 * L;
+  size_t lds = (size_t)64 * ((D + 15) / 16) * 16 * sizeof(float);
+  const size_t fr_lds = align_up((size_t)kFrLdsInts * sizeof(int), 16);
+  if (lds < fr_lds) lds = fr_lds;
+  static DeviceMask cap;
+  if (lds > 64 * 1024) { rc = raise_lds_cap(k_seed_prologue, cap); if (rc) return rc; }
+  hipLaunchKernelGGL(k_seed_prologue, dim3((unsigned)(csr->B + gx * gy * gz)), dim3(kSpThreads), lds, (hipStream_t)stream,
+                     g, f, gx, gy);
+  GNNRAG_LAUNCH_CHECK();
+  return 0;
+}
+
+extern "C" int gnnrag_seed_prologue(const gnnrag_csr* csr, const float* dist, void* fws, size_t fws_bytes, float* zero_a,
+                                    int64_t zero_na, float* zero_b, int64_t zero_nb, const float* relfeat_fwd,
+                                    const float* relfeat_inv, int32_t D, int32_t L, const gnnrag_layer_params* layers,
+                                    int32_t pos_rows, float* T_out, void* packed_out, int32_t* combined,
+                                    gnnrag_stream_t stream) {
+  if (combined) *combined = 0;
+  if (!csr || !dist || !fws) return GNNRAG_E_BADARG;
+  int rc = gnnrag::seed_prologue_launch(csr, dist, fws, fws_bytes, zero_a, zero_na, zero_b, zero_nb, relfeat_fwd, relfeat_inv,
+                                        D, L, layers, pos_rows, T_out, packed_out, stream);
+  if (rc == 0 && combined) *combined = 1;
+  if (rc != GNNRAG_E_UNSUPPORTED) return rc;
+  rc = gnnrag::rel_transform_launch(relfeat_fwd, relfeat_inv, csr->R1, D, L, layers, pos_rows, T_out, nullptr, packed_out, stream);
+  if (rc) return rc;
+  return gnnrag::frontier_build_z(csr, dist, fws, fws_bytes, zero_a, zero_na, zero_b, zero_nb, (hipStream_t)stream);
+}
+
 extern "C" int gnnrag_rel_transform(const float* relfeat_fwd, const float* relfeat_inv, int64_t R1, int32_t D,
                                     int32_t L, const gnnrag_layer_params* layers, int32_t pos_rows, float* T_out,
                                     void* planes_out, gnnrag_stream_t stream) {
diff --git a/gnn-rag_amd/csrc/seed_prologue.h b/gnn-rag_amd/csrc/seed_prologue.h
--- /dev/null
+++ b/gnn-rag_amd/csrc/seed_prologue.h
@@ -0,0 +1,298 @@
+#pragma once
+#include "gnnrag_common.h"
+
+namespace gnnrag {
+
+constexpr int kRtMaxL = 8;
+constexpr int kRtUnroll = 7;
+constexpr int kRtStage = 16;
+
+struct RelTArgs {
+  const float* A[2];
+  const float* W[kRtMaxL];
+  const float* b[kRtMaxL];
+  const float* add[kRtMaxL][2];
+  float* C;
+  unsigned short* planes;
+  unsigned char* packed;
+  int M, K, N, add_rows;
+};
+
+constexpr int kPlaneHalf = 224;
+constexpr int kPlaneRow = 2 * kPlaneHalf;
+constexpr int kPackPlaneB = kPlaneHalf * 2;
+constexpr int kPackIdxB = 3 * kPackPlaneB;
+constexpr int kPackRowB = kPackIdxB + 64;
+
+__device__ __forceinline__ void load_a_round(const float* __restrict__ ap, int c0, int fg, int K, f32x4 (&av)[kRtUnroll]) {
+#pragma unroll
+  for (int u = 0; u < kRtUnroll; ++u) av[u] = *reinterpret_cast<const f32x4*>(ap + min(16 * (c0 + u) + 4 * fg, K - 4));
+}
+
+template <int TPW>
+__device__ __forceinline__ void rel_transform_body(const RelTArgs& g, int bx, int by, int bz, float* Wf) {
+  const int tid = threadIdx.x, lane = tid & 63, wave = tid >> 6;
+  const int fr = lane & 15, fg = lane >> 4;
+  const int j = bz >> 1, d = bz & 1;
+  const int colg = by * 64;
+  const int K = g.K;
+  const int nch = (K + 15) >> 4;
+  const f32x4 zero4 = {0.f, 0.f, 0.f, 0.f};
+  const bool compute = colg < g.N;
+  const float* __restrict__ ap0 = g.A[d] + (size_t)min(bx * TPW * 64 + wave * 16 + fr, g.M - 1) * K;
+  f32x4 av[kRtUnroll];
+  if (compute) {
+    const int a = wave, frq = lane >> 2, fgq = lane & 3;
+    const int col = colg + 4 * frq + a;
+    const float* __restrict__ wrow = g.W[j] + (size_t)min(col, g.N - 1) * K;
+    float* __restrict__ wdst = Wf + (size_t)(a * 64 + fgq * 16 + frq) * 4;
+    f32x4 wv[kRtStage];
+    auto request = [&](int i0) {
+#pragma unroll
+      for (int u = 0; u < kRtStage; ++u)
+        wv[u] = *reinterpret_cast<const f32x4*>(wrow + min(16 * min(i0 + u, nch - 1) + 4 * fgq, K - 4));
+    };
+    auto write = [&](int i0) {
+#pragma unroll
+      for (int u = 0; u < kRtStage; ++u) {
+        const int i = min(i0 + u, nch - 1);
+        const bool live = col < g.N && 16 * i + 4 * fgq < K;
+        *reinterpret_cast<f32x4*>(wdst + (size_t)i * 1024) = live ? wv[u] : zero4;
+      }
+    };
+    request(0);
+    load_a_round(ap0, 0, fg, K, av);
+    __builtin_amdgcn_sched_barrier(0);
+    write(0);
+    for (int i0 = kRtStage; i0 < nch; i0 += kRtStage) {
+      request(i0);
+      write(i0);
+    }
+  }
+  __syncthreads();
+  const int c4 = colg + 4 * fr;
+  const bool in_T = c4 < g.N;
+  const bool in_pad = !in_T && c4 < kPlaneHalf;
+  f32x4 bias = zero4;
+  const float* __restrict__ bp = g.b[j];
+  if (in_T && bp) bias = *reinterpret_cast<const f32x4*>(bp + c4);
+  const float* __restrict__ addp = g.add[j][d];
+  float* __restrict__ cp = g.C + ((size_t)(2 * j + d) * g.M) * g.N;
+  unsigned short* pp = g.planes ? g.planes + ((size_t)(2 * j + d) * 3 * g.M) * kPlaneRow : nullptr;
+  unsigned char* pk = g.packed ? g.packed + ((size_t)(2 * j + d) * g.M) * kPackRowB : nullptr;
+
+#pragma unroll 1
+  for (int t = 0; t < TPW; ++t) {
+    const int row0 = (bx * TPW + t) * 64 + wave * 16;
+    if (row0 >= g.M) break;
+    f32x4 acc[4][2];
+#pragma unroll
+    for (int a = 0; a < 4; ++a) acc[a][0] = acc[a][1] = zero4;
+    if (compute) {
+      const float* __restrict__ ap = g.A[d] + (size_t)min(row0 + fr, g.M - 1) * K;
+      if (t > 0) load_a_round(ap, 0, fg, K, av);
+      for (int c0 = 0; c0 < nch; c0 += kRtUnroll) {
+        f32x4 nx[kRtUnroll];
+        const bool more = c0 + kRtUnroll < nch;
+        if (more) load_a_round(ap, c0 + kRtUnroll, fg, K, nx);
+        __builtin_amdgcn_sched_barrier(0);
+#pragma unroll
+        for (int u = 0; u < kRtUnroll; ++u) {
+          const int c = min(c0 + u, nch - 1);
+          const bool live = 16 * (c0 + u) + 4 * fg < K;
+          const f32x4 x = live ? av[u] : zero4;
+          f32x4 wv[4];
+#pragma unroll
+          for (int a = 0; a < 4; ++a) wv[a] = *reinterpret_cast<const f32x4*>(Wf + ((size_t)((c * 4 + a) * 64 + lane)) * 4);
+#pragma unroll
+          for (int e = 0; e < 4; ++e)
+#pragma unroll
+            for (int a = 0; a < 4; ++a)
+              acc[a][e & 1] = __builtin_amdgcn_mfma_f32_16x16x4f32(x[e], wv[a][e], acc[a][e & 1], 0, 0, 0);
+        }
+        if (more) {
+#pragma unroll
+          for (int u = 0; u < kRtUnroll; ++u) av[u] = nx[u];
+        }
+      }
+    }
+    if (!in_T && !(pp && in_pad) && !pk) continue;
+    f32x4 addv[4] = {zero4, zero4, zero4, zero4};
+    if (in_T && addp && g.add_rows > 0) {
+#pragma unroll
+      for (int r = 0; r < 4; ++r)
+        addv[r] = *reinterpret_cast<const f32x4*>(addp + (size_t)min(row0 + 4 * fg + r, g.add_rows - 1) * g.N + c4);
+    }
+#pragma unroll
+    for (int r = 0; r < 4; ++r) {
+      const int row = row0 + 4 * fg + r;
+      if (row >= g.M) continue;
+      f32x4 v = zero4;
+      if (in_T) {
+#pragma unroll
+        for (int a = 0; a < 4; ++a) v[a] = acc[a][0][r] + acc[a][1][r];
+        v += bias;
+        if (addp && row < g.add_rows) v += addv[r];
+        *reinterpret_cast<f32x4*>(cp + (size_t)row * g.N + c4) = v;
+      }
+      if (pp) {
+#pragma unroll
+        for (int half = 0; half < 2; ++half) {
+          const Split3 sp = split3(__builtin_elementwise_max(half ? -v : v, zero4));
+          const size_t e = (size_t)row * kPlaneRow + half * kPlaneHalf + c4;
+          *reinterpret_cast<uint2*>(pp + e) = sp.hi;
+          *reinterpret_cast<uint2*>(pp + (size_t)g.M * kPlaneRow + e) = sp.mid;
+          *reinterpret_cast<uint2*>(pp + (size_t)2 * g.M * kPlaneRow + e) = sp.lo;
+        }
+      }
+      if (pk) {
+        unsigned char* rowp = pk + (size_t)row * kPackRowB;
+        if (c4 < kPlaneHalf) {
+          const Split3 sp = split3(__builtin_elementwise_abs(v));
+          *reinterpret_cast<uint2*>(rowp + 2 * c4) = sp.hi;
+          *reinterpret_cast<uint2*>(rowp + kPackPlaneB + 2 * c4) = sp.mid;
+          *reinterpret_cast<uint2*>(rowp + 2 * kPackPlaneB + 2 * c4) = sp.lo;
+        }
+        const int q = c4 >> 2;
+        const unsigned ix = 0x88u | (unsigned)(v[0] < 0.f) | (unsigned)(v[1] < 0.f) << 2 | (unsigned)(v[2] < 0.f) << 4 |
+                            (unsigned)(v[3] < 0.f) << 6;
+        rowp[kPackIdxB + ((q & 7) >> 1) * 16 + (q >> 3) * 2 + (q & 1)] = (unsigned char)(c4 < kPlaneHalf ? ix : 0u);
+      }
+    }
+  }
+}
+
+constexpr int kSpSeedCap = 2048, kSpAltSeeds = 32;
+constexpr int kFrPass = 2048;
+constexpr int kFrLdsInts = kSpSeedCap + 1 + kFrPass / 64;
+template <int NT, int kFrSeedCap = kSpSeedCap, int kFrAltSeeds = kSpAltSeeds>
+__device__ __forceinline__ void frontier_body(
+    const float* __restrict__ dist, const int32_t* __restrict__ rp0, const int32_t* __restrict__ rp1,
+    const int2* __restrict__ el0, const int2* __restrict__ el1, const int32_t* __restrict__ rel_off, int N,
+    uint8_t* __restrict__ row_flag, int32_t* __restrict__ rows, uint8_t* __restrict__ tflag,
+    int32_t* __restrict__ trows, int32_t* __restrict__ counts, int32_t* __restrict__ seeds,
+    int32_t* __restrict__ seedinfo, float* __restrict__ zero_a, long long zero_na, float* __restrict__ zero_b,
+    long long zero_nb, int g, int nq, int* s_seed, int& s_ns, int* s_wsum) {
+  const int tid = threadIdx.x, lane = tid & 63, wave = tid >> 6;
+  const int roff = rel_off[g], Rg = rel_off[g + 1] - roff;
+  const size_t n0 = (size_t)g * N;
+  for (long long i = (long long)g * NT + tid; i < zero_na; i += (long long)nq * NT) zero_a[i] = 0.f;
+  for (long long i = (long long)g * NT + tid; i < zero_nb; i += (long long)nq * NT) zero_b[i] = 0.f;
+  if (tid == 0) s_ns = 0;
+  if (g == nq - 1 && tid < 64) row_flag[(size_t)nq * N + tid] = 0;
+  for (int i = tid; i < N; i += NT) row_flag[n0 + i] = 0;
+  for (int i = tid; i < Rg; i += NT) tflag[roff + i] = 0;
+  __syncthreads();
+  constexpr int U = kFrPass / NT;
+  for (int i0 = 0; i0 < N; i0 += kFrPass) {
+    float v[U];
+#pragma unroll
+    for (int u = 0; u < U; ++u) {
+      const int i = i0 + u * NT + tid;
+      v[u] = i < N ? dist[n0 + i] : 0.f;
+    }
+#pragma unroll
+    for (int u = 0; u < U; ++u) {
+      if (v[u] != 0.f) {
+        const int k = atomicAdd(&s_ns, 1);
+        if (k < kFrSeedCap) s_seed[k] = (int)n0 + i0 + u * NT + tid;
+      }
+    }
+  }
+  __syncthreads();
+  const int ns = s_ns;
+  if (tid == 0) {
+    int cnt = -1, facts = 0;
+    if (ns <= kFrAltSeeds) {
+      cnt = ns;
+      for (int i = 1; i < ns; ++i) {
+        const int v = s_seed[i];
+        int j = i - 1;
+        for (; j >= 0 && s_seed[j] > v; --j) s_seed[j + 1] = s_seed[j];
+        s_seed[j + 1] = v;
+      }
+      for (int i = 0; i < ns; ++i) {
+        const int sn = s_seed[i];
+        seeds[g * kFrAltSeeds + i] = sn;
+        facts += (rp0[sn + 1] - rp0[sn]) + (rp1[sn + 1] - rp1[sn]);
+      }
+    }
+    seedinfo[2 * g] = cnt;
+    seedinfo[2 * g + 1] = facts;
+  }
+  __syncthreads();
+  if (ns > kFrSeedCap) {
+    for (int i = tid; i < N; i += NT) row_flag[n0 + i] = 1;
+    for (int i = tid; i < Rg; i += NT) tflag[roff + i] = 1;
+  } else {
+    for (int k = 0; k < ns; ++k) {
+      const int s = s_seed[k];
+#pragma unroll
+      for (int dd = 0; dd < 2; ++dd) {
+        const int32_t* rp = dd ? rp1 : rp0;
+        const int2* el = dd ? el1 : el0;
+        const int beg = rp[s], end = rp[s + 1];
+        for (int j = beg + tid; j < end; j += NT) {
+          const int2 e = el[j];
+          row_flag[e.x] = 1;
+          tflag[roff + e.y] = 1;
+        }
+      }
+    }
+  }
+  __syncthreads();
+  auto compact = [&](const uint8_t* flag, int n, int first, int32_t* list, int32_t* count_out) {
+    int base = 0;
+    for (int c0 = 0; c0 < n; c0 += kFrPass) {
+      uint8_t fl[U];
+#pragma unroll
+      for (int u = 0; u < U; ++u) {
+        const int i = c0 + u * NT + tid;
+        fl[u] = i < n ? flag[i] : (uint8_t)0;
+      }
+      unsigned long long mk[U];
+#pragma unroll
+      for (int u = 0; u < U; ++u) {
+        mk[u] = __ballot(fl[u] != 0);
+        if (lane == 0) s_wsum[u * (NT / 64) + wave] = __popcll(mk[u]);
+      }
+      __syncthreads();
+#pragma unroll
+      for (int u = 0; u < U; ++u) {
+        int off = base;
+        for (int w = 0; w < NT / 64; ++w) {
+          const int c = s_wsum[u * (NT / 64) + w];
+          if (w < wave) off += c;
+          base += c;
+        }
+        if (fl[u] != 0) list[off + __popcll(mk[u] & ((1ull << lane) - 1))] = first + c0 + u * NT + tid;
+      }
+      __syncthreads();
+    }
+    if (tid == 0) *count_out = base;
+  };
+  compact(row_flag + n0, N, (int)n0, rows + n0, counts + 2 * g);
+  compact(tflag + roff, Rg, roff, trows + roff, counts + 2 * g + 1);
+}
+
+struct FrontierArgs {
+  const float* dist;
+  const int32_t* rp0;
+  const int32_t* rp1;
+  const int2* el0;
+  const int2* el1;
+  const int32_t* rel_off;
+  uint8_t* row_flag;
+  int32_t* rows;
+  uint8_t* tflag;
+  int32_t* trows;
+  int32_t* counts;
+  int32_t* seeds;
+  int32_t* seedinfo;
+  float* zero_a;
+  float* zero_b;
+  long long zero_na, zero_nb;
+  int N, B;
+};
+
+}
diff --git a/gnn-rag_amd/csrc/softmax_layer.hip b/gnn-rag_amd/csrc/softmax_layer.hip
--- a/gnn-rag_amd/csrc/softmax_layer.hip
+++ b/gnn-rag_amd/csrc/softmax_layer.hip
@@ -257,14 +257,29 @@
   return gnnrag_masked_softmax(score, dist_out, csr->B, csr->N, stream);
 }
 
+static bool frontier_form_ok(const gnnrag_csr* csr, const LayerWs& w, const char* base, const float* dist, const float* ins,
+                             const float* T_fwd, const float* T_inv, const float* W_e2e, int32_t D, int32_t I, int32_t path) {
+  if (!(path & GNNRAG_PATH_SEED_PRIOR) || (path & (GNNRAG_PATH_ONLY_FWD | GNNRAG_PATH_ONLY_INV))) return false;
+  int p = path & 0xf;
+  if (p == GNNRAG_PATH_AUTO)
+    p = fused_is_cheaper(csr->B, csr->N, csr->rel_total, D, I) ? GNNRAG_PATH_FUSED : GNNRAG_PATH_UNFUSED;
+  if (p != GNNRAG_PATH_FUSED) return false;
+  const float* P = (const float*)(base + w.P);
+  const float* nbr = (const float*)(base + w.nbr);
+  return aligned16(ins, W_e2e, T_fwd, T_inv, P, nbr, dist) && csr->N > 0 && gnnrag_frontier_supported(csr, D) &&
+         csr->rel_total > 0;
+}
+
 static int layer_body(const gnnrag_csr* csr, const LayerWs& w, char* base, const float* h, const float* dist,
                       const float* ins, const float* T_fwd, const float* T_inv, const void* planes, const float* W_e2e,
                       const float* b_e2e, const float* w_score, const float* b_score, const float* mask,
                       float* h_out, float* score_out, float* dist_out, int32_t D, int32_t I, int32_t path,
-                      int32_t math, gnnrag_stream_t stream, bool pairs_ready = false, bool* pairs_for_next = nullptr) {
+                      int32_t math, gnnrag_stream_t stream, bool pairs_ready = false, bool* pairs_for_next = nullptr,
+                      bool frontier_built = false) {
   if (pairs_for_next) *pairs_for_next = false;
   const int64_t BN = (int64_t)csr->B * csr->N;
   int rc;
+  const bool frontier_form = frontier_form_ok(csr, w, base, dist, ins, T_fwd, T_inv, W_e2e, D, I, path);
   const int only = (path & GNNRAG_PATH_ONLY_FWD) ? 0 : (path & GNNRAG_PATH_ONLY_INV) ? 1 : -1;
   const bool seed_prior = (path & GNNRAG_PATH_SEED_PRIOR) != 0;
   path &= 0xf;
@@ -274,14 +289,14 @@
     float* P = (float*)(base + w.P);
     float* nbr = (float*)(base + w.nbr);
     const bool one_dir = only >= 0 && gnnrag_aggregate_fused_variant(csr, D) != GNNRAG_WALK_L2_GATHER;
-    const bool fr_aligned = aligned16(ins, W_e2e, T_fwd, T_inv, P, nbr, dist) && csr->N > 0;
-    const bool frontier_form = seed_prior && only < 0 && fr_aligned && gnnrag_frontier_supported(csr, D) && csr->rel_total > 0;
     if (frontier_form) {
       void* fws = base + w.fws;
       const bool gated = update_rows_supported(h, nbr, W_e2e, h_out, BN, D, I, math);
       if (!gated) GNNRAG_HIP(hipMemsetAsync(nbr, 0, (size_t)BN * D * sizeof(float), (hipStream_t)stream));
-      rc = frontier_build_z(csr, dist, fws, w.fws_bytes, score_out, BN, nbr + (size_t)BN * D, D, (hipStream_t)stream);
-      if (rc) return rc;
+      if (!frontier_built) {
+        rc = frontier_build_z(csr, dist, fws, w.fws_bytes, score_out, BN, nbr + (size_t)BN * D, D, (hipStream_t)stream);
+        if (rc) return rc;
+      }
       rc = gnnrag_relation_tables_frontier(csr, fws, T_fwd, T_inv, ins, W_e2e, P, D, I, stream);
       if (rc) return rc;
       rc = gnnrag_aggregate_fused_frontier(csr, fws, dist, P, nbr, D, stream);
@@ -334,6 +349,27 @@
     if (rc) return rc;
   }
   return 0;
+}
+
+static int seed_projections(const gnnrag_csr* csr, const LayerWs& w, char* base, int32_t n, const gnnrag_layer_params* layers,
+                            const float* relfeat_fwd, const float* relfeat_inv, int32_t pos_rows, float* T, void* planes,
+                            bool* planes_written, const float* dist, const float* ins, float* score0, int32_t D, int32_t I,
+                            int32_t path, int32_t math, gnnrag_stream_t stream, bool* frontier_built) {
+  *frontier_built = false;
+  const size_t RD = (size_t)csr->R1 * D;
+  const int64_t BN = (int64_t)csr->B * csr->N;
+  if (frontier_form_ok(csr, w, base, dist, ins, T, T + RD, layers[0].W_e2e, D, I, path)) {
+    float* nbr = (float*)(base + w.nbr);
+    const int rc = seed_prologue_launch(csr, dist, base + w.fws, w.fws_bytes, score0, BN, nbr + (size_t)BN * D, D, relfeat_fwd,
+                                        relfeat_inv, D, n, layers, pos_rows, T, planes, stream);
+    if (rc == 0) {
+      *planes_written = planes != nullptr;
+      *frontier_built = true;
+      return 0;
+    }
+    if (rc != GNNRAG_E_UNSUPPORTED) return rc;
+  }
+  return rel_projections(csr, n, layers, relfeat_fwd, relfeat_inv, pos_rows, T, planes, planes_written, D, math, stream);
 }
 
 extern "C" size_t gnnrag_stack_workspace_bytes(const gnnrag_csr* csr, int32_t L, int32_t D, int32_t I) {
@@ -361,13 +397,13 @@
   float* T_inv = (float*)(base + w.T_inv);
   const gnnrag_layer_params p = {W_rel, b_rel, pos_fwd, pos_inv, W_e2e, b_e2e};
   void* planes = planes_wanted(csr, D, I, path, math) ? (void*)(base + w.planes) : nullptr;
-  bool planes_written = false;
-  const int rc = rel_projections(csr, 1, &p, relfeat_fwd, relfeat_inv, pos_rows, T_fwd, planes, &planes_written, D, math,
-                                 stream);
+  bool planes_written = false, frontier_built = false;
+  const int rc = seed_projections(csr, w, base, 1, &p, relfeat_fwd, relfeat_inv, pos_rows, T_fwd, planes, &planes_written, dist,
+                                  ins, score_out, D, I, path, math, stream, &frontier_built);
   if (rc) return rc;
   if (!planes_written) planes = nullptr;
   return layer_body(csr, w, base, h, dist, ins, T_fwd, T_inv, planes, W_e2e, b_e2e, w_score, b_score, mask, h_out, score_out,
-                    dist_out, D, I, path, math, stream);
+                    dist_out, D, I, path, math, stream, false, nullptr, frontier_built);
 }
 
 extern "C" int gnnrag_reason_stack(const gnnrag_csr* csr, int32_t L, const gnnrag_layer_params* layers,
@@ -393,15 +429,16 @@
   const bool want_planes = planes_wanted(csr, D, I, path, math);
   const size_t plane_bytes = tables_vq_packed_bytes(csr->R1);
   char* planes_all = base + w.total + align_up((size_t)L * 2 * RD * sizeof(float), 256);
-  bool planes_written = false;
+  bool planes_written = false, frontier_built = false;
   const bool reuse = upfront && (path & GNNRAG_PATH_REUSE_PROJ) != 0;
   path &= ~GNNRAG_PATH_REUSE_PROJ;
   if (reuse) {
     planes_written = want_planes && rel_transform_accepts(relfeat_fwd, relfeat_inv, csr->R1, D, L, layers, pos_rows, Tall,
                                                           planes_all);
   } else if (upfront) {
-    const int rc = rel_projections(csr, L, layers, relfeat_fwd, relfeat_inv, pos_rows, Tall,
-                                   want_planes ? planes_all : nullptr, &planes_written, D, math, stream);
+    const int rc = seed_projections(csr, w, base, L, layers, relfeat_fwd, relfeat_inv, pos_rows, Tall,
+                                    want_planes ? planes_all : nullptr, &planes_written, dist0, ins, score_out, D, I, path, math,
+                                    stream, &frontier_built);
     if (rc) return rc;
   }
   const float* h = h0;
@@ -423,7 +460,7 @@
     bool pairs_next = false;
     const int rc = layer_body(csr, w, base, h, dist, ins, T, T + RD, planes, p.W_e2e, p.b_e2e, w_score, b_score, mask, hj, sj,
                               dj, D, I, j == 0 ? path : (path & ~GNNRAG_PATH_SEED_PRIOR), math, stream, pairs_ready,
-                              j + 1 < L ? &pairs_next : nullptr);
+                              j + 1 < L ? &pairs_next : nullptr, j == 0 && frontier_built);
     if (rc) return rc;
     pairs_ready = pairs_next;
     h = hj;
diff --git a/gnn-rag_amd/ops.py b/gnn-rag_amd/ops.py
--- a/gnn-rag_amd/ops.py
+++ b/gnn-rag_amd/ops.py
@@ -600,6 +600,59 @@
         return out
 
 
+FRONTIER_PARTS = ("counts", "row_flag", "rows", "tflag", "trows", "seeds", "seedinfo")
+
+
+def frontier_layout(plan: CsrPlan) -> dict:
+    off = (C.c_uint64 * 8)()
+    _lib.check(_lib.load().gnnrag_frontier_layout(C.byref(plan.c), off), "gnnrag_frontier_layout")
+    return dict(zip(FRONTIER_PARTS + ("total",), (int(x) for x in off)))
+
+
+def seed_prologue(plan: CsrPlan, dist: torch.Tensor, ws: torch.Tensor, relfeat: torch.Tensor, relfeat_inv: torch.Tensor,
+                  layers, T_out: torch.Tensor, packed_out: Optional[torch.Tensor] = None,
+                  zero_a: Optional[torch.Tensor] = None, zero_b: Optional[torch.Tensor] = None) -> bool:
+    lib = _lib.load()
+    relfeat = _chk(relfeat, "rel_features")
+    R1, D = relfeat.shape
+    relfeat_inv = _chk(relfeat_inv, "rel_features_inv", shape=(R1, D))
+    dist = _chk(dist, "dist").reshape(-1)
+    _on_plan_device(plan, dist, "dist")
+    if dist.numel() != plan.B * plan.N or R1 != plan.R1:
+        raise ValueError("dist / rel_features do not match the plan")
+    L = len(layers)
+    params = (_lib.LayerParams * max(L, 1))()
+    keep, pos_rows = [], 0
+    for j, (W, b, pos, pos_inv) in enumerate(layers):
+        W = _chk(W, "rel_linear.weight", shape=(D, D))
+        b = _chk(b, "rel_linear.bias", shape=(D,))
+        keep += [W, b]
+        params[j].W_rel, params[j].b_rel = W.data_ptr(), b.data_ptr()
+        if pos is not None:
+            pos = _chk(pos, "pos_emb.weight")
+            pos_inv = _chk(pos_inv, "pos_emb_inv.weight", shape=tuple(pos.shape))
+            pos_rows = pos.shape[0]
+            keep += [pos, pos_inv]
+            params[j].pos_fwd, params[j].pos_inv = pos.data_ptr(), pos_inv.data_ptr()
+    if T_out.dtype != torch.float32 or T_out.numel() < L * 2 * R1 * D or not T_out.is_contiguous():
+        raise ValueError("T_out must be a contiguous float32 buffer of at least L*2*R1*D elements")
+    if packed_out is not None and packed_out.numel() * packed_out.element_size() < lib.gnnrag_rel_packed_bytes(R1, D, L):
+        raise ValueError("packed_out is smaller than gnnrag_rel_packed_bytes")
+    if ws.numel() * ws.element_size() < lib.gnnrag_frontier_workspace_bytes(C.byref(plan.c)):
+        raise ValueError("ws is smaller than gnnrag_frontier_workspace_bytes")
+    for z in (zero_a, zero_b):
+        if z is not None and (z.dtype != torch.float32 or not z.is_contiguous()):
+            raise ValueError("zero_a / zero_b must be contiguous float32")
+    combined = C.c_int32(0)
+    with torch.cuda.device(dist.device):
+        _lib.check(lib.gnnrag_seed_prologue(
+            C.byref(plan.c), dist.data_ptr(), ws.data_ptr(), ws.numel() * ws.element_size(), _ptr(zero_a),
+            zero_a.numel() if zero_a is not None else 0, _ptr(zero_b), zero_b.numel() if zero_b is not None else 0,
+            relfeat.data_ptr(), relfeat_inv.data_ptr(), D, L, params, pos_rows, T_out.data_ptr(), _ptr(packed_out),
+            C.byref(combined), _stream()), "gnnrag_seed_prologue")
+    return bool(combined.value)
+
+
 def update_score_fused(h, nbr, W, b, w_s, b_s, mask, I: int, math: Optional[int] = None):
     lib = _lib.load()
     h = _chk(h, "h")
diff --git a/include/gnnrag.h b/include/gnnrag.h
--- a/include/gnnrag.h
+++ b/include/gnnrag.h
@@ -268,6 +268,11 @@
                                     float* out, int32_t D, gnnrag_stream_t stream);
 int gnnrag_frontier_read(const gnnrag_csr* csr, const void* fws, int32_t* counts2, uint8_t* row_flag_host,
                          gnnrag_stream_t stream);
+int gnnrag_frontier_layout(const gnnrag_csr* csr, uint64_t* offsets8);
+int gnnrag_seed_prologue(const gnnrag_csr* csr, const float* dist, void* fws, size_t fws_bytes, float* zero_a,
+                         int64_t zero_na, float* zero_b, int64_t zero_nb, const float* relfeat_fwd,
+                         const float* relfeat_inv, int32_t D, int32_t L, const gnnrag_layer_params* layers,
+                         int32_t pos_rows, float* T_out, void* packed_out, int32_t* combined, gnnrag_stream_t stream);
 
 int gnnrag_topp_candidates(const float* pred_dist, const uint8_t* eligible, int32_t B, int32_t N,
                            double ignore_prob, double eps, int32_t* out_slot, int32_t* out_cnt,
```
